# rabbitmq/ra

Hardware: AMD Instinct MI355X
Metric: append_entries decisions/sec across N Raft groups; achieved HBM GB/s vs peak (higher is better)
Workload: dtype u64

## Files before the change

### include/ra_gpu_batch.h

```cpp
#ifndef RA_GPU_BATCH_H
#define RA_GPU_BATCH_H

#include <stddef.h>
#include <stdint.h>

#ifdef __cplusplus
extern "C" {
#endif

#define RGB_ABI_VERSION   10u
#define RGB_UNDEF         UINT64_MAX
#define RGB_NONE          0xFFu
#define RGB_MAX_MEMBERS   8u
#define RGB_MAX_PENDING_RANGES 3u
#define RGB_MAX_RUNS      16u

#define RGB_AER_CHUNK_SIZE              128u
#define RGB_DEFAULT_MAX_PIPELINE_COUNT  4096u

enum {
  RGB_ROLE_FOLLOWER        = 0,
  RGB_ROLE_CANDIDATE       = 1,
  RGB_ROLE_LEADER          = 2,
  RGB_ROLE_PRE_VOTE        = 3,
// ... 273 lines not shown
int  rgb_collect(rgb_ctx *ctx, rgb_decision *out, uint32_t cap, uint32_t *n_out,
                 rgb_rpc *rpc_out, uint32_t rpc_cap, uint32_t *n_rpc_out, uint64_t *tick_out);
typedef struct rgb_view {
  const rgb_decision *decisions;
  const rgb_rpc *rpcs;
  uint64_t tick;
  uint32_t n;
  uint32_t n_rpcs;
  uint32_t slot;
  uint32_t _pad;
} rgb_view;
int  rgb_collect_view(rgb_ctx *ctx, rgb_view *view);
int  rgb_release(rgb_ctx *ctx, uint32_t slot);
uint32_t rgb_submit_trains(const rgb_ctx *ctx);
int      rgb_peek(rgb_ctx *ctx, uint32_t *n_out, uint32_t *n_rpc_out);
int      rgb_wait(rgb_ctx *ctx, uint32_t timeout_ms);
void     rgb_wake(rgb_ctx *ctx);
uint32_t rgb_in_flight(const rgb_ctx *ctx);

#define RGB_SUBMIT_RAW_MAX_ROUNDS 8u
typedef struct rgb_fill {
  rgb_msg *msgs;
  uint32_t cap;
  uint32_t slot;
  uint32_t max_rounds;
} rgb_fill;
uint32_t rgb_submit_raw_capacity(const rgb_ctx *ctx, uint32_t max_rounds);
int      rgb_submit_begin(rgb_ctx *ctx, uint32_t max_rounds, rgb_fill *out);
int      rgb_submit_commit(rgb_ctx *ctx, uint32_t slot, uint32_t n, uint64_t tick);
int      rgb_submit_raw(rgb_ctx *ctx, const rgb_msg *msgs, uint32_t n, uint32_t max_rounds, uint64_t tick);

uint32_t rgb_route(uint64_t group_uid, uint32_t n_contexts);

#define RGB_COMM_ID_BYTES 128u
typedef struct rgb_comm rgb_comm;
int  rgb_comm_unique_id(void *id_out );
int  rgb_comm_init_rank(rgb_ctx *ctx, const void *id, uint32_t n_ranks, uint32_t rank, rgb_comm **out);
void rgb_comm_destroy(rgb_comm *comm);
uint32_t rgb_comm_n_ranks(const rgb_comm *comm);
uint32_t rgb_comm_rank(const rgb_comm *comm);
int  rgb_leaderboard_allgather(rgb_ctx *ctx, rgb_comm *comm, const void *d_rows_local, uint32_t n_rows,
                               void *d_rows_all , void *stream);
int  rgb_leaderboard_allgather_host(rgb_ctx *ctx, rgb_comm *comm, uint32_t n_rows, rgb_leaderboard_row *rows_all);
const char *rgb_comm_last_error(void);

int  rgb_run_ticks_device(rgb_ctx *ctx, const void *d_msgs, uint32_t tick_stride,
                          const uint32_t *tick_counts, const void *d_tick_counts,
                          const uint32_t *kind_counts, uint32_t n_ticks, void *d_decisions,
                          void *d_rpcs, void *stream);

#define RGB_TRAIN_BUCKETS 256u
#define RGB_TRAIN_ERR_PLACEMENT 1u
#define RGB_TRAIN_ERR_SPIN      2u
#define RGB_TRAIN_ERR_ORDER     4u
#define RGB_TRAIN_ERR_PLAN      8u
#define RGB_TRAIN_FORM_NONE       0u
#define RGB_TRAIN_FORM_DEALT      1u
#define RGB_TRAIN_FORM_PERSISTENT 2u
typedef struct rgb_train_plan rgb_train_plan;
uint32_t rgb_train_bucket(uint32_t kind, uint32_t flags, uint32_t server, uint32_t n_members);
int  rgb_train_plan_create(rgb_ctx *ctx, const uint32_t *bucket_counts, uint32_t n_ticks, rgb_train_plan **out);
void rgb_train_plan_destroy(rgb_train_plan *plan);
uint32_t rgb_train_plan_blocks_per_tick(const rgb_train_plan *plan);
int  rgb_train_stamp_device(rgb_ctx *ctx, const void *d_msgs, void *d_stamps, uint32_t tick_stride,
                            const uint32_t *tick_counts, uint32_t n_ticks, void *stream);
int  rgb_train_run_device(rgb_ctx *ctx, const rgb_train_plan *plan, uint32_t first_tick, uint32_t n_ticks,
                          const void *d_msgs, const void *d_stamps, uint32_t tick_stride, void *d_decisions,
                          void *d_rpcs, uint32_t rpc_ring, void *stream);
int  rgb_train_plan_create_snap(rgb_ctx *ctx, const uint32_t *bucket_counts, uint32_t n_ticks, uint32_t snapshot_every,
                                rgb_train_plan **out);
int  rgb_train_run_snap_device(rgb_ctx *ctx, const rgb_train_plan *plan, uint32_t first_tick, uint32_t n_ticks,
                               const void *d_msgs, const void *d_stamps, uint32_t tick_stride, void *d_decisions,
                               void *d_rpcs, uint32_t rpc_ring, const void *d_snap_stamps, void *d_snap_rows,
                               void *stream);
int  rgb_snapshot_train_device(rgb_ctx *ctx, void *d_rows, void *stream);
int  rgb_train_plan_create_device(rgb_ctx *ctx, uint32_t n_ticks, uint32_t snapshot_every, rgb_train_plan **out);
int  rgb_train_plan_build_device(rgb_ctx *ctx, rgb_train_plan *plan, uint32_t first_tick, uint32_t n_ticks,
                                 const void *d_bucket_counts, void *stream);
int  rgb_train_plan_fit(rgb_ctx *ctx, rgb_train_plan *plan, uint32_t first_tick, uint32_t n_ticks, void *stream);
int  rgb_train_plan_download(rgb_ctx *ctx, const rgb_train_plan *plan, uint32_t tick, void *out_tick, uint32_t *out_rows,
                             uint32_t rows_cap);
uint32_t rgb_train_seq_bytes(const rgb_ctx *ctx);
int  rgb_train_status(rgb_ctx *ctx, uint32_t *flags_out, uint32_t *xcc_of_shard );
uint32_t rgb_train_form(const rgb_ctx *ctx);
uint32_t rgb_train_recoveries(const rgb_ctx *ctx);

int  rgb_snapshot(rgb_ctx *ctx, rgb_leaderboard_row *out);
int  rgb_snapshot_device(rgb_ctx *ctx, void *d_rows, void *stream);

int  rgb_state_checksum(rgb_ctx *ctx, uint32_t first, uint32_t n, uint64_t *out);

int  rgb_synchronize(rgb_ctx *ctx);

#ifdef __cplusplus
}
#endif
#endif
```

### ra_amd/csrc/rgb_api.hip

```cpp
#include <hip/hip_runtime.h>

#include <atomic>
#include <chrono>
#include <condition_variable>
#include <cstdio>
#include <cstdlib>
#include <cstring>
#include <memory>
#include <mutex>
#include <thread>
#include <new>
#include <vector>

#if defined(__x86_64__)
#include <emmintrin.h>
#endif

#include "rgb_internal.h"
#include "../../include/ra_gpu_batch_synth.h"

#define RGB_STREAM_COPY_MIN (1u << 20)
#ifndef RGB_COPY_STREAM_MIN
#define RGB_COPY_STREAM_MIN (2u << 20)
#endif
static inline void copy_msg(rgb_msg *dst, const rgb_msg *src, bool stream) {
#if defined(__x86_64__)
  if (stream) {
    const __m128i *q = reinterpret_cast<const __m128i *>(src);
    __m128i *d = reinterpret_cast<__m128i *>(dst);
    const __m128i a = _mm_loadu_si128(q), b = _mm_loadu_si128(q + 1), c = _mm_loadu_si128(q + 2), e = _mm_loadu_si128(q + 3);
    _mm_stream_si128(d, a); _mm_stream_si128(d + 1, b); _mm_stream_si128(d + 2, c); _mm_stream_si128(d + 3, e);
    return;
  }
#endif
  (void)stream;
  *dst = *src;
}
static inline void copy_out(void *dst, const void *src, size_t bytes) {
#if defined(__x86_64__)
  if (bytes >= RGB_STREAM_COPY_MIN && ((uintptr_t)dst & 15u) == 0 && (bytes & 63u) == 0) {
    const __m128i *q = reinterpret_cast<const __m128i *>(src);
    __m128i *d = reinterpret_cast<__m128i *>(dst);
    for (size_t k = 0; k < bytes / 16u; k += 4) {
      const __m128i a = _mm_loadu_si128(q + k), b = _mm_loadu_si128(q + k + 1), c = _mm_loadu_si128(q + k + 2), e = _mm_loadu_si128(q + k + 3);
      _mm_stream_si128(d + k, a); _mm_stream_si128(d + k + 1, b); _mm_stream_si128(d + k + 2, c); _mm_stream_si128(d + k + 3, e);
    }
    _mm_sfence();
    return;
  }
#endif
  memcpy(dst, src, bytes);
}

#define HIPCHK(ctx, expr)                          \
  do {                                             \
    hipError_t e__ = (expr);                       \
    if (e__ != hipSuccess) {                       \
      (ctx)->last_hip.store((int)e__, std::memory_order_relaxed); \
      return RGB_E_HIP;                            \
    }                                              \
  } while (0)
#define LAUNCHCHK(ctx, expr)                       \
  do {                                             \
    int lr__ = (expr);                             \
    if (lr__) {                                    \
      (ctx)->last_hip.store(lr__, std::memory_order_relaxed); \
      return RGB_E_HIP;                            \
    }                                              \
  } while (0)

struct rgb_slot {
  rgb_msg *h_msgs = nullptr;
  rgb_decision *h_dec = nullptr;
  rgb_msg *d_msgs = nullptr;
  rgb_decision *d_dec = nullptr;
  u32 *h_pos = nullptr, *d_pos = nullptr;
  rgb_rpc *d_rpcs = nullptr;
  rgb_rpc *h_rpcs = nullptr;
  u32 *h_nrpc = nullptr;
  u32 *d_res = nullptr;
  unsigned char *h_stamps = nullptr, *d_stamps = nullptr;
  rgb_train_tick *h_plan = nullptr, *d_plan = nullptr;
  u32 *h_rows = nullptr, *d_rows = nullptr;
  u32 rows_cap = 0;
  u32 *d_ctl = nullptr;
  u64 *h_ranges = nullptr, *d_ranges = nullptr;
  u32 ranges_cap = 0, n_ranges = 0;
  bool has_seqx = false;
  u32 *h_touched = nullptr, *d_touched = nullptr;
  u32 n_touched = 0;
  void *d_undo = nullptr;
  bool has_undo = false;
  u32 n_rounds = 0;
  std::vector<u32> round_start;
  std::vector<u32> round_cc;
// ... 109 lines not shown
    case RGB_E_NOMEM: return "out of memory";
    case RGB_E_HIP: return "HIP runtime error (see rgb_last_hip_error)";
    case RGB_E_STATE: return "call out of order";
    case RGB_E_FULL: return "staging ring full";
    case RGB_E_EMPTY: return "nothing submitted";
    case RGB_E_UNSUPPORTED: return "unsupported";
    case RGB_E_NODEVICE: return "no HIP device (there is no CPU fallback)";
    case RGB_E_COMM: return "RCCL error (see rgb_comm_last_error)";
    default: return "unknown error";
  }
}

void rgb_default_config(rgb_config *cfg) {
  if (!cfg) return;
  memset(cfg, 0, sizeof *cfg);
  cfg->abi_version = RGB_ABI_VERSION;
  cfg->device = 0;
  cfg->max_runs = 8;
  cfg->ring_slots = 4;
  cfg->ring_capacity = 65536;
  cfg->max_pipeline_count = RGB_DEFAULT_MAX_PIPELINE_COUNT;
  cfg->max_aer_batch = RGB_AER_CHUNK_SIZE;
  cfg->flags = 0;
}

int rgb_last_hip_error(const rgb_ctx *ctx) { return ctx ? ctx->last_hip.load(std::memory_order_relaxed) : 0; }

static int settle_trains(rgb_ctx *ctx);
struct rgb_stream_turn {
  std::lock_guard<std::mutex> a, c, b;
  int rc;
  explicit rgb_stream_turn(rgb_ctx *ctx) : a(ctx->state_mu), c(ctx->collect_mu), b(ctx->enqueue_mu), rc(settle_trains(ctx)) {}
};

static void free_slot(rgb_slot &s) {
  if (s.h_msgs) (void)hipHostFree(s.h_msgs);
  if (s.h_dec) (void)hipHostFree(s.h_dec);
  if (s.d_msgs) (void)hipFree(s.d_msgs);
  if (s.d_dec) (void)hipFree(s.d_dec);
  if (s.d_rpcs) (void)hipFree(s.d_rpcs);
  if (s.h_rpcs) (void)hipHostFree(s.h_rpcs);
  if (s.h_nrpc) (void)hipHostFree(s.h_nrpc);
  if (s.d_res) (void)hipFree(s.d_res);
  if (s.h_stamps) (void)hipHostFree(s.h_stamps);
  if (s.d_stamps) (void)hipFree(s.d_stamps);
  if (s.h_plan) (void)hipHostFree(s.h_plan);
  if (s.d_plan) (void)hipFree(s.d_plan);
  if (s.h_rows) (void)hipHostFree(s.h_rows);
  if (s.d_rows) (void)hipFree(s.d_rows);
  if (s.d_ctl) (void)hipFree(s.d_ctl);
  if (s.h_ranges) (void)hipHostFree(s.h_ranges);
  if (s.d_ranges) (void)hipFree(s.d_ranges);
  s.h_ranges = s.d_ranges = nullptr; s.ranges_cap = 0;
  if (s.h_touched) (void)hipHostFree(s.h_touched);
  if (s.d_touched) (void)hipFree(s.d_touched);
  if (s.d_undo) (void)hipFree(s.d_undo);
  if (s.done) (void)hipEventDestroy(s.done);
  if (s.copied) (void)hipEventDestroy(s.copied);
  s.copied = nullptr;
  if (s.d_raw) (void)hipFree(s.d_raw);
  if (s.d_key) (void)hipFree(s.d_key);
  free(s.h_stage);
  s.d_raw = nullptr; s.d_key = nullptr; s.h_stage = nullptr;
  s.h_msgs = nullptr; s.h_dec = nullptr; s.d_msgs = nullptr; s.d_dec = nullptr; s.d_rpcs = nullptr; s.h_rpcs = nullptr;
  s.h_nrpc = nullptr; s.d_res = nullptr;
  s.h_stamps = s.d_stamps = nullptr; s.h_plan = s.d_plan = nullptr; s.h_rows = s.d_rows = nullptr; s.done = nullptr;
  s.d_ctl = nullptr; s.h_touched = s.d_touched = nullptr; s.d_undo = nullptr;
  s.h_pos = s.d_pos = nullptr;
}

void rgb_close(rgb_ctx *ctx) {
  if (!ctx) return;
  if (ctx->stream) (void)hipStreamSynchronize(ctx->stream);
  rgb_wal_release(ctx);
  rgb_seg_release(ctx);
  for (u32 k = 0; k < ctx->ring_size; ++k) free_slot(ctx->ring_mem[k]);
  if (ctx->dev.dbg_buf) (void)hipFree(ctx->dev.dbg_buf);
  if (ctx->dev.hot) (void)hipFree(ctx->dev.hot);
  if (ctx->dev.peers) (void)hipFree(ctx->dev.peers);
  if (ctx->dev.runs) (void)hipFree(ctx->dev.runs);
  if (ctx->dev.cond) (void)hipFree(ctx->dev.cond);
  if (ctx->dev.qry) (void)hipFree(ctx->dev.qry);
  if (ctx->dev.seq) (void)hipFree(ctx->dev.seq);
  if (ctx->d_stage) (void)hipFree(ctx->d_stage);
  if (ctx->h_stage) (void)hipHostFree(ctx->h_stage);
  if (ctx->d_rows) (void)hipFree(ctx->d_rows);
  if (ctx->d_sums) (void)hipFree(ctx->d_sums);
  if (ctx->lb_stream) { (void)hipStreamSynchronize(ctx->lb_stream); (void)hipStreamDestroy(ctx->lb_stream); }
  if (ctx->copy_stream) { (void)hipStreamSynchronize(ctx->copy_stream); (void)hipStreamDestroy(ctx->copy_stream); }
  if (ctx->d_lb_gather) (void)hipFree(ctx->d_lb_gather);
  if (ctx->h_lb_pinned) (void)hipHostFree(ctx->h_lb_pinned);
  if (ctx->lb_event) (void)hipEventDestroy(ctx->lb_event);
  if (ctx->d_synth) (void)hipFree(ctx->d_synth);
  if (ctx->d_synth_sent) (void)hipFree(ctx->d_synth_sent);
  if (ctx->d_train_ctl) (void)hipFree(ctx->d_train_ctl);
  if (ctx->d_seq_cnt) (void)hipFree(ctx->d_seq_cnt);
  if (ctx->d_srv_cnt) (void)hipFree(ctx->d_srv_cnt);
  if (ctx->d_srv_list) (void)hipFree(ctx->d_srv_list);
  if (ctx->d_prep) (void)hipFree(ctx->d_prep);

  if (ctx->stream) (void)hipStreamDestroy(ctx->stream);
  delete ctx;
}

int rgb_open(const rgb_config *cfg_in, rgb_ctx **out) {
  if (!out) return RGB_E_INVAL;
  *out = nullptr;
  rgb_config cfg;
  if (cfg_in) cfg = *cfg_in; else rgb_default_config(&cfg);
  if (cfg.abi_version != RGB_ABI_VERSION) return RGB_E_INVAL;
  if (cfg.max_runs < 2 || cfg.max_runs > RGB_MAX_RUNS) return RGB_E_INVAL;
  if (cfg.ring_slots < 1 || cfg.ring_slots > 64 || cfg.ring_capacity < 1) return RGB_E_INVAL;
  if (cfg.max_pipeline_count == 0) cfg.max_pipeline_count = RGB_DEFAULT_MAX_PIPELINE_COUNT;
  if (cfg.max_aer_batch == 0) cfg.max_aer_batch = RGB_AER_CHUNK_SIZE;
  if (cfg.max_aer_batch > 65535) return RGB_E_INVAL;
  int ndev = 0;
  hipError_t e = hipGetDeviceCount(&ndev);
  if (e != hipSuccess || ndev <= 0) return RGB_E_NODEVICE;
  if (cfg.device < 0 || cfg.device >= ndev) return RGB_E_INVAL;
  rgb_ctx *ctx = new (std::nothrow) rgb_ctx();
  if (!ctx) return RGB_E_NOMEM;
  ctx->cfg = cfg;
  memset(&ctx->dev, 0, sizeof ctx->dev);
  e = hipSetDevice(cfg.device);
  if (e == hipSuccess) e = hipStreamCreateWithFlags(&ctx->stream, hipStreamNonBlocking);
  if (e == hipSuccess) e = hipStreamCreateWithFlags(&ctx->copy_stream, hipStreamNonBlocking);

  if (e != hipSuccess) { delete ctx; return RGB_E_HIP; }
  *out = ctx;
  return RGB_OK;
}

uint32_t rgb_n_servers(const rgb_ctx *ctx) { return ctx ? ctx->dev.n_servers : 0; }

static int alloc_slot(rgb_ctx *ctx, rgb_slot &s) {
  const u32 cap = ctx->cfg.ring_capacity;
  HIPCHK(ctx, hipHostMalloc((void **)&s.h_msgs, (size_t)cap * (sizeof(rgb_msg) + sizeof(u32)), hipHostMallocDefault));
  HIPCHK(ctx, hipHostMalloc((void **)&s.h_dec, (size_t)cap * sizeof(rgb_decision), hipHostMallocDefault));
  HIPCHK(ctx, hipMalloc((void **)&s.d_msgs, (size_t)cap * (sizeof(rgb_msg) + sizeof(u32))));
  HIPCHK(ctx, hipMalloc((void **)&s.d_dec, (size_t)cap * sizeof(rgb_decision)));
  s.h_pos = reinterpret_cast<u32 *>(s.h_msgs + cap); s.d_pos = reinterpret_cast<u32 *>(s.d_msgs + cap);
  HIPCHK(ctx, hipMalloc((void **)&s.d_rpcs, (size_t)ctx->rpc_cap * sizeof(rgb_rpc)));
  HIPCHK(ctx, hipHostMalloc((void **)&s.h_rpcs, (size_t)ctx->rpc_cap * sizeof(rgb_rpc), hipHostMallocDefault));
  HIPCHK(ctx, hipEventCreateWithFlags(&s.done, hipEventDisableTiming));
  HIPCHK(ctx, hipEventCreateWithFlags(&s.copied, hipEventDisableTiming));
  HIPCHK(ctx, hipHostMalloc((void **)&s.h_nrpc, 64, hipHostMallocDefault));
  HIPCHK(ctx, hipMalloc((void **)&s.d_res, ((size_t)rgb_results_blocks(cap) + 1u) * sizeof(u32)));
  HIPCHK(ctx, hipMemsetAsync(s.d_res, 0, ((size_t)rgb_results_blocks(cap) + 1u) * sizeof(u32), ctx->stream));
  HIPCHK(ctx, hipHostMalloc((void **)&s.h_stamps, cap, hipHostMallocDefault));
  HIPCHK(ctx, hipMalloc((void **)&s.d_stamps, cap));
  HIPCHK(ctx, hipHostMalloc((void **)&s.h_plan, RGB_SUBMIT_TRAIN_ROUNDS * sizeof(rgb_train_tick), hipHostMallocDefault));
  HIPCHK(ctx, hipMalloc((void **)&s.d_plan, RGB_SUBMIT_TRAIN_ROUNDS * sizeof(rgb_train_tick)));
  s.rows_cap = (cap / 32u + 2u * RGB_N_CLASSES * RGB_SUBMIT_TRAIN_ROUNDS + 64u);
  HIPCHK(ctx, hipHostMalloc((void **)&s.h_rows, (size_t)s.rows_cap * RGB_SUBMIT_TRAIN_ROUNDS * sizeof(u32), hipHostMallocDefault));
  HIPCHK(ctx, hipMalloc((void **)&s.d_rows, (size_t)s.rows_cap * RGB_SUBMIT_TRAIN_ROUNDS * sizeof(u32)));
  HIPCHK(ctx, hipMalloc((void **)&s.d_ctl, RGB_TRAIN_CTL_WORDS * sizeof(u32)));
  HIPCHK(ctx, hipMemsetAsync(s.d_ctl, 0, RGB_TRAIN_CTL_WORDS * sizeof(u32), ctx->stream));
  HIPCHK(ctx, hipHostMalloc((void **)&s.h_touched, (size_t)cap * sizeof(u32), hipHostMallocDefault));
  HIPCHK(ctx, hipMalloc((void **)&s.d_touched, (size_t)cap * sizeof(u32)));
  return RGB_OK;
}

int rgb_upload_state(rgb_ctx *ctx, uint32_t first, uint32_t n, const rgb_server_state *in);

int rgb_register_groups(rgb_ctx *ctx, uint32_t n_groups, uint32_t n_members) {
  if (!ctx) return RGB_E_INVAL;
  if (ctx->registered) return RGB_E_STATE;
  if (n_members < 1 || n_members > RGB_MAX_MEMBERS || n_groups < 1) return RGB_E_INVAL;
  const uint64_t S64 = (uint64_t)n_groups * n_members;
  if (S64 > 0x7FFFFFFFull) return RGB_E_INVAL;
  const u32 S = (u32)S64;
  HIPCHK(ctx, hipSetDevice(ctx->cfg.device));
  rgb_dev &d = ctx->dev;
  d.n_servers = S; d.n_members = n_members; d.max_runs = ctx->cfg.max_runs;
  d.peer_stride = rgb_peer_stride(n_members);
  d.max_pipeline_count = ctx->cfg.max_pipeline_count;
  d.max_aer_batch = ctx->cfg.max_aer_batch;
  d.dbg = 0; d.dbg_buf = nullptr;
  d.synth_hint = ctx->synth_hint;
  d.fuse_pipeline = (ctx->cfg.flags & RGB_CFG_FUSE_PIPELINE) ? 1u : 0u;
  d.seq_ranges = nullptr; d.n_seq_ranges = 0;
#ifdef RGB_PROFILE
  { const char *e = getenv("RGB_DEBUG"); d.dbg = e ? (u32)atoi(e) : 0u; }
  if (d.dbg & 16u) {
    HIPCHK(ctx, hipMalloc((void **)&d.dbg_buf, (size_t)(S / 64 + 16) * 8 * sizeof(u64)));
    HIPCHK(ctx, hipMemsetAsync(d.dbg_buf, 0, (size_t)(S / 64 + 16) * 8 * sizeof(u64), ctx->stream));
  }
#endif
#ifdef RGB_X_DECLINE_HIST
  HIPCHK(ctx, hipMalloc((void **)&d.dbg_buf, 128 * sizeof(u64)));
  HIPCHK(ctx, hipMemsetAsync(d.dbg_buf, 0, 128 * sizeof(u64), ctx->stream));
#endif
#ifdef RGB_X_TRAIN_TIMELINE
  HIPCHK(ctx, hipMalloc((void **)&d.dbg_buf, (size_t)(1u << 20) * 8 * sizeof(u64)));
  HIPCHK(ctx, hipMemsetAsync(d.dbg_buf, 0, (size_t)(1u << 20) * 8 * sizeof(u64), ctx->stream));
#endif
  HIPCHK(ctx, hipMalloc((void **)&d.hot, (size_t)S * RGB_HOT_WORDS * sizeof(u64)));
  HIPCHK(ctx, hipMalloc((void **)&d.peers, (size_t)S * d.peer_stride * sizeof(u64)));
  HIPCHK(ctx, hipMalloc((void **)&d.runs, (size_t)S * d.max_runs * 2 * sizeof(u64)));
  HIPCHK(ctx, hipMalloc((void **)&d.cond, (size_t)S * 4 * sizeof(u64)));
  HIPCHK(ctx, hipMalloc((void **)&d.qry, (size_t)S * RGB_QRY_WORDS * sizeof(u64)));
  HIPCHK(ctx, hipMemsetAsync(d.runs, 0, (size_t)S * d.max_runs * 2 * sizeof(u64), ctx->stream));
  d.seq_stride = (((n_groups + RGB_TRAIN_SHARDS - 1u) / RGB_TRAIN_SHARDS) * n_members + 255u) & ~255u;
  HIPCHK(ctx, hipMalloc((void **)&d.seq, (size_t)d.seq_stride * RGB_TRAIN_SHARDS));
  HIPCHK(ctx, hipMemsetAsync(d.seq, 0, (size_t)d.seq_stride * RGB_TRAIN_SHARDS, ctx->stream));
  ctx->stage_cap = S < 16384u ? S : 16384u;
  HIPCHK(ctx, hipMalloc((void **)&ctx->d_stage, (size_t)ctx->stage_cap * sizeof(rgb_server_state)));
  HIPCHK(ctx, hipHostMalloc((void **)&ctx->h_stage, (size_t)ctx->stage_cap * sizeof(rgb_server_state),
                            hipHostMallocDefault));
  HIPCHK(ctx, hipMalloc((void **)&ctx->d_rows, (size_t)n_groups * sizeof(rgb_leaderboard_row)));
  HIPCHK(ctx, hipMalloc((void **)&ctx->d_sums, (size_t)S * sizeof(u64)));
  ctx->rpc_stride = n_members > 1 ? n_members - 1 : 1;
  ctx->rpc_cap = ctx->cfg.ring_capacity * ctx->rpc_stride;
  ctx->ring_mem.reset(new (std::nothrow) rgb_slot[ctx->cfg.ring_slots]);
  if (!ctx->ring_mem) return RGB_E_NOMEM;
  ctx->ring_size = ctx->cfg.ring_slots;
  for (u32 k = 0; k < ctx->ring_size; ++k) {
    rgb_slot &s = ctx->ring_mem[k];
    int rc = alloc_slot(ctx, s);
    if (rc) return rc;
  }
  ctx->registered = true;
  std::vector<rgb_server_state> init(ctx->stage_cap);
  for (u32 base = 0; base < S; base += ctx->stage_cap) {
    u32 cnt = S - base < ctx->stage_cap ? S - base : ctx->stage_cap;
    for (u32 k = 0; k < cnt; ++k) {
      rgb_server_state &h = init[k];
      memset(&h, 0, sizeof h);
      h.snapshot_index = RGB_UNDEF; h.snapshot_term = RGB_UNDEF;
      h.pending_first = 1;
      for (unsigned i = 0; i < n_members; ++i) h.next_index[i] = 1;
      h.role = RGB_ROLE_FOLLOWER; h.self = (uint8_t)((base + k) % n_members);
      h.n_members = (uint8_t)n_members; h.voted_for = RGB_NONE; h.leader_id = RGB_NONE;
      h.cond_leader = RGB_NONE; h.n_runs = 1;
      h.present_mask = (uint8_t)((1u << n_members) - 1u); h.voter_mask = h.present_mask;
      h.status_mask = 0xFF;
    }
    int rc = rgb_upload_state(ctx, base, cnt, init.data());
    if (rc) return rc;
  }
  return RGB_OK;
}

static int validate_state(const rgb_ctx *ctx, const rgb_server_state &h) {
  if (h.n_members != ctx->dev.n_members) return RGB_E_INVAL;
  if (h.self >= RGB_MAX_MEMBERS) return RGB_E_INVAL;
  if (h.role > RGB_ROLE_AWAIT_CONDITION || h.cond_reason > RGB_COND_TRANSFER_LEADERSHIP) return RGB_E_INVAL;
  if (h.n_runs > RGB_MAX_RUNS || h.votes > 15) return RGB_E_INVAL;
  if (h.voted_for != RGB_NONE && h.voted_for >= RGB_MAX_MEMBERS) return RGB_E_INVAL;
  if (h.leader_id != RGB_NONE && h.leader_id >= RGB_MAX_MEMBERS) return RGB_E_INVAL;
  if (h.cond_leader != RGB_NONE && h.cond_leader >= RGB_MAX_MEMBERS) return RGB_E_INVAL;
  if (h.first_index <= h.last_index) {
    if (h.n_runs == 0 || h.run_start[0] != h.first_index) return RGB_E_INVAL;
    for (unsigned r = 1; r < h.n_runs; ++r)
      if (!(h.run_start[r] > h.run_start[r - 1] && h.run_start[r] <= h.last_index)) return RGB_E_INVAL;
    if (h.run_term[h.n_runs - 1] != h.last_term) return RGB_E_INVAL;
  }
  if (h.n_pending_old > 2) return RGB_E_INVAL;
  uint64_t above = h.pending_first;
  for (int k = (int)h.n_pending_old - 1; k >= 0; --k) {
    const uint64_t s = h.pending_old[k][0], e = h.pending_old[k][1];
    if (s > e || e == RGB_UNDEF || !(e + 1 < above)) return RGB_E_INVAL;
    above = s;
  }
  return RGB_OK;
}

int rgb_upload_state(rgb_ctx *ctx, uint32_t first, uint32_t n, const rgb_server_state *in) {
  if (!ctx || (!in && n)) return RGB_E_INVAL;
  if (!ctx->registered) return RGB_E_STATE;
  if ((uint64_t)first + n > ctx->dev.n_servers) return RGB_E_INVAL;
  for (u32 k = 0; k < n; ++k) {
    int rc = validate_state(ctx, in[k]);
    if (rc) return rc;
  }
  HIPCHK(ctx, hipSetDevice(ctx->cfg.device));
  rgb_stream_turn turn(ctx);
  if (turn.rc) return turn.rc;
  for (u32 base = 0; base < n; base += ctx->stage_cap) {
    u32 cnt = n - base < ctx->stage_cap ? n - base : ctx->stage_cap;
    memcpy(ctx->h_stage, in + base, (size_t)cnt * sizeof(rgb_server_state));
    HIPCHK(ctx, hipMemcpyAsync(ctx->d_stage, ctx->h_stage, (size_t)cnt * sizeof(rgb_server_state),
                               hipMemcpyHostToDevice, ctx->stream));
    LAUNCHCHK(ctx, rgb_launch_pack(ctx->dev, ctx->d_stage, first + base, cnt, ctx->stream));
    HIPCHK(ctx, hipStreamSynchronize(ctx->stream));
  }
  return RGB_OK;
}

int rgb_download_state(rgb_ctx *ctx, uint32_t first, uint32_t n, rgb_server_state *out) {
  if (!ctx || (!out && n)) return RGB_E_INVAL;
  if (!ctx->registered) return RGB_E_STATE;
  if ((uint64_t)first + n > ctx->dev.n_servers) return RGB_E_INVAL;
  HIPCHK(ctx, hipSetDevice(ctx->cfg.device));
  rgb_stream_turn turn(ctx);
  if (turn.rc) return turn.rc;
  for (u32 base = 0; base < n; base += ctx->stage_cap) {
    u32 cnt = n - base < ctx->stage_cap ? n - base : ctx->stage_cap;
    LAUNCHCHK(ctx, rgb_launch_unpack(ctx->dev, ctx->d_stage, first + base, cnt, ctx->stream));
    HIPCHK(ctx, hipMemcpyAsync(ctx->h_stage, ctx->d_stage, (size_t)cnt * sizeof(rgb_server_state),
                               hipMemcpyDeviceToHost, ctx->stream));
    HIPCHK(ctx, hipStreamSynchronize(ctx->stream));
    memcpy(out + base, ctx->h_stage, (size_t)cnt * sizeof(rgb_server_state));
  }
  return RGB_OK;
}

static int validate_msg(const rgb_ctx *ctx, const rgb_msg &m) {
  if (m.kind > RGB_MSG_KIND_MAX) return RGB_E_INVAL;
  if (m.kind == RGB_MSG_NOP) return RGB_OK;
  if (m.server >= ctx->dev.n_servers) return RGB_E_INVAL;
  if (m.from != RGB_NONE && m.from >= RGB_MAX_MEMBERS) return RGB_E_INVAL;
  if (m.kind == RGB_MSG_AER && m.n_run0 > m.n_entries) return RGB_E_INVAL;
  if (m.kind == RGB_MSG_WRITTEN && m.a > m.b) return RGB_E_INVAL;
  if (m.kind == RGB_MSG_WRITTEN && (m.flags & RGB_MF_SEQ2) &&
      !(m.run0_term <= m.run1_term && m.run1_term != RGB_UNDEF && m.run1_term + 1 < m.a)) return RGB_E_INVAL;
  if (m.kind == RGB_MSG_WRITTEN && (m.flags & RGB_MF_SEQX) && !(m.flags & RGB_MF_SEQ2)) return RGB_E_INVAL;
  return RGB_OK;
}
static int validate_seqx(const rgb_msg &m, const uint64_t *ranges, uint32_t n_ranges) {
  if (m.kind != RGB_MSG_WRITTEN || !(m.flags & RGB_MF_SEQX)) return RGB_OK;
  if (!ranges || m.n_entries == 0 || m.c > n_ranges || (uint64_t)m.c + m.n_entries > n_ranges) return RGB_E_INVAL;
  uint64_t prev_last = 0; bool have = false;
  for (uint32_t k = 0; k < m.n_entries; ++k) {
    const uint64_t f = ranges[2 * (m.c + k)], l = ranges[2 * (m.c + k) + 1];
    if (f > l || l == RGB_UNDEF || (have && !(prev_last + 1 < f))) return RGB_E_INVAL;
    prev_last = l; have = true;
  }
  return prev_last + 1 < m.run0_term ? RGB_OK : RGB_E_INVAL;
}

static int train_scratch(rgb_ctx *ctx);

#define RGB_FAULT_STAMP 1u
#define RGB_FAULT_SHARD 2u

static rgb_dev slot_dev(const rgb_ctx *ctx, const rgb_slot &s) {
  rgb_dev d = ctx->dev;
  d.seq_ranges = s.n_ranges ? s.d_ranges : nullptr;
  d.n_seq_ranges = s.n_ranges;
  return d;
}

static int enqueue_rounds(rgb_ctx *ctx, rgb_slot &s) {
  const rgb_dev dv = slot_dev(ctx, s);
  auto classes = [&](const u32 counts[RGB_N_CLASSES], u32 at) {
    return rgb_launch_tick_classes(dv, s.d_msgs + at, counts, nullptr, 0, s.d_dec + at, s.d_rpcs, at, at, ctx->stream);
  };
  for (u32 r = 0; r < s.n_rounds; ++r) {
    const u32 off = s.round_start[r], cnt = s.round_start[r + 1] - s.round_start[r];
    u32 cc[RGB_N_CLASSES], real = 0, before_written = 0;
    for (int c = 0; c < RGB_N_CLASSES; ++c) {
      cc[c] = s.round_cc[(size_t)r * RGB_N_CLASSES + c];
      real += cc[c];
      if (c < 2) before_written += cc[c];
    }
    if (!s.has_seqx || cc[2] == 0) {
      LAUNCHCHK(ctx, classes(cc, off));
    } else {
      u32 head[RGB_N_CLASSES] = {0}, tail[RGB_N_CLASSES] = {0};
      head[0] = cc[0]; head[1] = cc[1];
// ... 851 lines not shown
  void *st = stream ? stream : (void *)ctx->stream;
  LAUNCHCHK(ctx, rgb_launch_train_plan((const u32 *)d_bucket_counts, plan->d_ticks, plan->d_rows, plan->bpt / RGB_TRAIN_SHARDS,
                                       first_tick, n_ticks, plan->snap_every, ctx->dev.n_servers / ctx->dev.n_members,
                                       ctx->dev.n_members, ctx->d_train_ctl, st));
  for (u32 t = first_tick; t < first_tick + n_ticks; ++t) plan->rows_fit[t] = 0xFFFFFFFFu;
  return RGB_OK;
}

int rgb_train_plan_fit(rgb_ctx *ctx, rgb_train_plan *plan, uint32_t first_tick, uint32_t n_ticks, void *stream) {
  if (!ctx || !plan) return RGB_E_INVAL;
  if (!plan->on_device || (uint64_t)first_tick + n_ticks > plan->n_ticks) return RGB_E_INVAL;
  if (n_ticks == 0) return RGB_OK;
  HIPCHK(ctx, hipSetDevice(ctx->cfg.device));
  hipStream_t st = stream ? (hipStream_t)stream : ctx->stream;
  std::vector<u32> rows(n_ticks);
  HIPCHK(ctx, hipStreamSynchronize(st));
  HIPCHK(ctx, hipMemcpy2D(rows.data(), sizeof(u32), &plan->d_ticks[first_tick].n_rows, sizeof(rgb_train_tick), sizeof(u32),
                          n_ticks, hipMemcpyDeviceToHost));
  for (u32 t = 0; t < n_ticks; ++t) plan->rows_fit[first_tick + t] = rows[t];
  return RGB_OK;
}

int rgb_train_plan_download(rgb_ctx *ctx, const rgb_train_plan *plan, uint32_t tick, void *out_tick, uint32_t *out_rows,
                            uint32_t rows_cap) {
  if (!ctx || !plan || !out_tick || tick >= plan->n_ticks) return RGB_E_INVAL;
  HIPCHK(ctx, hipSetDevice(ctx->cfg.device));
  HIPCHK(ctx, hipStreamSynchronize(ctx->stream));
  rgb_train_tick h;
  HIPCHK(ctx, hipMemcpy(&h, plan->d_ticks + tick, sizeof h, hipMemcpyDeviceToHost));
  memcpy(out_tick, &h, sizeof h);
  const u32 rpt = plan->bpt / RGB_TRAIN_SHARDS;
  const u32 n = h.n_rows < rows_cap ? h.n_rows : rows_cap;
  if (out_rows && n && h.n_rows <= rpt)
    HIPCHK(ctx, hipMemcpy(out_rows, plan->d_rows + (size_t)tick * rpt, (size_t)n * sizeof(u32), hipMemcpyDeviceToHost));
  return (int)h.n_rows;
}

void rgb_train_plan_destroy(rgb_train_plan *plan) {
  if (!plan) return;
  if (plan->d_ticks) (void)hipFree(plan->d_ticks);
  if (plan->d_rows) (void)hipFree(plan->d_rows);
  delete plan;
}

uint32_t rgb_train_plan_blocks_per_tick(const rgb_train_plan *plan) {
  if (!plan) return 0;
  if (plan->on_device && !plan->rows_fit.empty()) {
    u32 mx = 0;
    for (u32 r : plan->rows_fit) { if (r == 0xFFFFFFFFu) return plan->bpt; if (r > mx) mx = r; }
    if (mx * RGB_TRAIN_SHARDS <= plan->bpt) return (mx ? mx : 1u) * RGB_TRAIN_SHARDS;
  }
  return plan->bpt;
}

int rgb_train_stamp_device(rgb_ctx *ctx, const void *d_msgs, void *d_stamps, uint32_t tick_stride,
                           const uint32_t *tick_counts, uint32_t n_ticks, void *stream) {
  if (!ctx || !d_msgs || !d_stamps || (!tick_counts && n_ticks)) return RGB_E_INVAL;
  if (!ctx->registered) return RGB_E_STATE;
  if (!ctx->d_seq_cnt || ctx->xcc_state != 1) return RGB_E_STATE;
  hipStream_t st = stream ? (hipStream_t)stream : ctx->stream;
  const rgb_msg *m = (const rgb_msg *)d_msgs;
  unsigned char *sp = (unsigned char *)d_stamps;
  HIPCHK(ctx, hipMemcpyAsync(ctx->d_seq_cnt, ctx->dev.seq, (size_t)ctx->dev.seq_stride * RGB_TRAIN_SHARDS,
                             hipMemcpyDeviceToDevice, st));
  for (u32 t = 0; t < n_ticks; ++t) {
    if (tick_counts[t] > tick_stride) return RGB_E_INVAL;
    LAUNCHCHK(ctx, rgb_launch_train_seq(ctx->dev, m + (size_t)t * tick_stride, tick_counts[t], ctx->d_seq_cnt,
                                        sp + (size_t)t * tick_stride, st));
  }
  return RGB_OK;
}

int rgb_train_run_device(rgb_ctx *ctx, const rgb_train_plan *plan, uint32_t first_tick, uint32_t n_ticks,
                         const void *d_msgs, const void *d_stamps, uint32_t tick_stride, void *d_decisions,
                         void *d_rpcs, uint32_t rpc_ring, void *stream) {
  return rgb_train_run_snap_device(ctx, plan, first_tick, n_ticks, d_msgs, d_stamps, tick_stride, d_decisions, d_rpcs,
                                   rpc_ring, nullptr, nullptr, stream);
}

uint32_t rgb_train_seq_bytes(const rgb_ctx *ctx) {
  return (ctx && ctx->registered) ? ctx->dev.seq_stride * RGB_TRAIN_SHARDS : 0u;
}

int rgb_snapshot_train_device(rgb_ctx *ctx, void *d_rows, void *stream) {
  int rc = rgb_snapshot_device(ctx, d_rows, stream);
  if (rc) return rc;
  void *st = stream ? stream : (void *)ctx->stream;
  LAUNCHCHK(ctx, rgb_launch_seq_bump(ctx->dev.seq, nullptr, ctx->dev.seq_stride * RGB_TRAIN_SHARDS, st));
  return RGB_OK;
}

int rgb_train_run_snap_device(rgb_ctx *ctx, const rgb_train_plan *plan, uint32_t first_tick, uint32_t n_ticks,
                              const void *d_msgs, const void *d_stamps, uint32_t tick_stride, void *d_decisions,
                              void *d_rpcs, uint32_t rpc_ring, const void *d_snap_stamps, void *d_snap_rows,
                              void *stream) {
  if (!ctx || !plan || !d_msgs || !d_stamps || !d_decisions) return RGB_E_INVAL;
  if (plan->snap_every && (!d_snap_stamps || !d_snap_rows)) return RGB_E_INVAL;
  if (!plan->snap_every && (d_snap_stamps || d_snap_rows)) return RGB_E_INVAL;
  if (!ctx->registered || ctx->xcc_state != 1) return RGB_E_STATE;
  if ((uint64_t)first_tick + n_ticks > plan->n_ticks) return RGB_E_INVAL;
  if (n_ticks == 0 || plan->bpt == 0) return RGB_OK;
  void *st = stream ? stream : (void *)ctx->stream;
  u32 per = RGB_TRAIN_MAX_TICKS;
  if ((uint64_t)per * plan->bpt > 0x7FFFFFFFull) per = (u32)(0x7FFFFFFFull / plan->bpt);
  if (per == 0) return RGB_E_INVAL;
  if (plan->snap_every) {
    if (n_ticks > per) return RGB_E_INVAL;
    const u32 last = first_tick + n_ticks - 1u;
    const u32 inside = last / plan->snap_every - first_tick / plan->snap_every;
    if (n_ticks + inside > RGB_TRAIN_MAX_TICKS) return RGB_E_INVAL;
  }
  for (u32 t = first_tick; t < first_tick + n_ticks; t += per) {
    const u32 n = first_tick + n_ticks - t < per ? first_tick + n_ticks - t : per;
    const size_t off = (size_t)t * tick_stride;
    u32 grid_bpt = plan->bpt;
    if (plan->on_device) {
      u32 mx = 0; bool known = true;
      for (u32 k = t; k < t + n && known; ++k) { known = plan->rows_fit[k] != 0xFFFFFFFFu; if (known && plan->rows_fit[k] > mx) mx = plan->rows_fit[k]; }
      if (known && mx * RGB_TRAIN_SHARDS <= plan->bpt) grid_bpt = (mx ? mx : 1u) * RGB_TRAIN_SHARDS;
    }
    LAUNCHCHK(ctx, rgb_launch_train(ctx->dev, (const rgb_msg *)d_msgs + off, (const unsigned char *)d_stamps + off,
                                    tick_stride, plan->d_ticks + t, plan->d_rows + (size_t)t * (plan->bpt / RGB_TRAIN_SHARDS), n,
                                    grid_bpt, (rgb_decision *)d_decisions + off,
                                    (rgb_rpc *)d_rpcs, rpc_ring, (u32)off, ctx->d_train_ctl, ctx->n_xcc,
                                    ctx->train_dealt.load(std::memory_order_relaxed) ? 0u : ctx->train_blocks, st,
                                    (const unsigned char *)d_snap_stamps, (rgb_leaderboard_row *)d_snap_rows,
                                    plan->bpt / RGB_TRAIN_SHARDS));
  }
  return RGB_OK;
}

int rgb_train_status(rgb_ctx *ctx, uint32_t *flags_out, uint32_t *xcc_of_shard) {
  if (!ctx) return RGB_E_INVAL;
  if (flags_out) *flags_out = 0;
  if (xcc_of_shard)
    for (u32 x = 0; x < RGB_TRAIN_SHARDS; ++x)
      xcc_of_shard[x] = ctx->xcc_state == 1 ? x % ctx->n_xcc : 0xFFFFFFFFu;
  if (!ctx->d_train_ctl) return RGB_OK;
  HIPCHK(ctx, hipSetDevice(ctx->cfg.device));
  HIPCHK(ctx, hipStreamSynchronize(ctx->stream));
  u32 w = 0;
  HIPCHK(ctx, hipMemcpy(&w, ctx->d_train_ctl, sizeof w, hipMemcpyDeviceToHost));
  if (flags_out) *flags_out = w;
  if (w & RGB_TRAIN_ERR_PLACEMENT) ctx->train_dealt.store(false, std::memory_order_relaxed);
  if (w) {
    HIPCHK(ctx, hipMemsetAsync(ctx->d_train_ctl, 0, sizeof(u32), ctx->stream));
    HIPCHK(ctx, hipStreamSynchronize(ctx->stream));
    return RGB_E_STATE;
  }
  return RGB_OK;
}

int rgb_synth_apply_tick_device(rgb_ctx *ctx, const void *d_msgs, uint32_t max_msgs, void *d_decisions,
                                void *d_rpcs, void *stream) {
  if (!ctx || !d_msgs || !d_decisions) return RGB_E_INVAL;
  if (!ctx->registered || !ctx->d_synth) return RGB_E_STATE;
  void *st = stream ? stream : (void *)ctx->stream;
  LAUNCHCHK(ctx, rgb_launch_tick_classes(ctx->dev, (const rgb_msg *)d_msgs, nullptr, ctx->d_synth, max_msgs,
                                         (rgb_decision *)d_decisions, (rgb_rpc *)d_rpcs, 0, 0, st));
  return RGB_OK;
}

int rgb_snapshot_device(rgb_ctx *ctx, void *d_rows, void *stream) {
  if (!ctx || !d_rows) return RGB_E_INVAL;
  if (!ctx->registered) return RGB_E_STATE;
  void *st = stream ? stream : (void *)ctx->stream;
// ... 164 lines not shown
```

### ra_amd/csrc/rgb_internal.h

```cpp
#ifndef RGB_INTERNAL_H
#define RGB_INTERNAL_H

#include <stdint.h>
#include "../../include/ra_gpu_batch.h"

typedef unsigned long long u64;
typedef uint32_t u32;

#define RGB_HOT_WORDS 16
#define RGB_QRY_WORDS 16

#define HOT_CT    0
#define HOT_PK    1
#define HOT_LRT   2
#define HOT_PRS   3
#define HOT_CI    4
#define HOT_LA    5
#define HOT_LI    6
#define HOT_LT    7
#define HOT_SI    8
#define HOT_ST    9
#define HOT_FIRST 10
#define HOT_LRS   11
#define HOT_LWI   12
// ... 11 lines not shown
#define PEER_MI(i, N) (2u * (unsigned)(i))
#define PEER_NI(i, N) (2u * (unsigned)(i) + 1u)
#define PEER_CS(i, N) (2u * (unsigned)(N) + (unsigned)(i))

#define PK_ROLE_SH      0
#define PK_COND_SH      3
#define PK_SELF_SH      5
#define PK_VOTES_SH     9
#define PK_NRUNS_SH     13
#define PK_NONVOTER_SH  18
#define PK_CONDTO_SH    19
#define PK_VOTED_SH     20
#define PK_LEADER_SH    24
#define PK_CONDLDR_SH   28
#define PK_PRESENT_SH   32
#define PK_VOTER_SH     40
#define PK_STATUS_SH    48
#define PK_QSELF_SH     56
#define PK_QPEER_SH     57
#define PK_BACKOFF_SH   58
#define PK_PENDX_SH     59
static inline __host__ __device__ unsigned pk_cond_reason(u64 pk) {
  const unsigned c = (unsigned)((pk >> PK_COND_SH) & 3ull), to = (unsigned)((pk >> PK_CONDTO_SH) & 1ull);
  return to == 0u ? c : c == RGB_COND_WAL_DOWN ? (unsigned)RGB_COND_WAL_DOWN_LEADER : (unsigned)RGB_COND_TRANSFER_LEADERSHIP;
}
static inline __host__ __device__ u64 pk_with_cond_reason(u64 pk, unsigned reason) {
  const u64 c = reason == RGB_COND_WAL_DOWN_LEADER ? (u64)RGB_COND_WAL_DOWN : reason == RGB_COND_TRANSFER_LEADERSHIP ? 0ull : (u64)reason;
  const u64 to = (reason == RGB_COND_WAL_DOWN_LEADER || reason == RGB_COND_TRANSFER_LEADERSHIP) ? 1ull : 0ull;
  return (pk & ~((3ull << PK_COND_SH) | (1ull << PK_CONDTO_SH))) | (c << PK_COND_SH) | (to << PK_CONDTO_SH);
}
#define QRY_PEND_LO     12
#define QRY_PEND_HI     14
#define QRY_BACKOFF     9
#define QRY_TOKEN       10
#define QRY_MACVER      11

#define RGB_N_CLASSES 15
static inline __host__ __device__ unsigned rgb_kind_rank(unsigned kind) {
  switch (kind) {
    case RGB_MSG_AER: return 0;
    case RGB_MSG_AER_REPLY: return 1;
    case RGB_MSG_WRITTEN: return 2;
    case RGB_MSG_APPEND: return 3;
    case RGB_MSG_PIPELINE_RPCS: return 4;
    case RGB_MSG_REQUEST_VOTE: return 5;
    case RGB_MSG_VOTE_RESULT: return 6;
    case RGB_MSG_AWAIT_TIMEOUT: return 7;
    case RGB_MSG_ELECTION_TIMEOUT: return 8;
    case RGB_MSG_PRE_VOTE_RPC: return 9;
    case RGB_MSG_PRE_VOTE_RESULT: return 10;
    case RGB_MSG_SNAPSHOT_WRITTEN: return 11;
    case RGB_MSG_HEARTBEAT_RPC: return 12;
    case RGB_MSG_HEARTBEAT_REPLY: return 13;
    case RGB_MSG_CONSISTENT_QUERY: return 14;
    case RGB_MSG_TRANSFER_LEADERSHIP: return 14;
    default: return 15;
  }
}
#define RGB_N_FAMILIES 32
static inline __host__ __device__ unsigned rgb_family(unsigned kind, unsigned flags) {
  return 2u * rgb_kind_rank(kind) + ((flags & RGB_MF_SUCCESS) ? 1u : 0u);
}
static inline unsigned rgb_class_of_kind(unsigned kind) { return rgb_kind_rank(kind); }

#define RGB_TRAIN_SHARDS 8u
#define RGB_N_BUCKETS ((RGB_N_CLASSES + 1u) * RGB_TRAIN_SHARDS * 2u)
#define RGB_TRAIN_CTL_WORDS (320u + 32u * 64u)
static inline __host__ __device__ unsigned rgb_shard_of_server(unsigned server, unsigned n_members) {
  return (server / n_members) & (RGB_TRAIN_SHARDS - 1u);
}
static inline __host__ __device__ unsigned rgb_bucket(unsigned kind, unsigned flags, unsigned server, unsigned n_members) {
  return (rgb_kind_rank(kind) * RGB_TRAIN_SHARDS + rgb_shard_of_server(server, n_members)) * 2u +
         ((flags & RGB_MF_SUCCESS) ? 1u : 0u);
}
static inline __host__ __device__ unsigned rgb_bucket_hinted(unsigned kind, unsigned flags, unsigned server,
                                                             unsigned n_members, bool off_steady) {
  const bool hinted_kind = kind == RGB_MSG_WRITTEN || kind == RGB_MSG_AER;
  return rgb_bucket(kind, flags, server, n_members) | ((hinted_kind && off_steady) ? 1u : 0u);
}
static inline __host__ __device__ unsigned rgb_seq_index(unsigned server, unsigned n_members, unsigned seq_stride) {
  const unsigned g = server / n_members, m = server - g * n_members;
  return (g & (RGB_TRAIN_SHARDS - 1u)) * seq_stride + (g / RGB_TRAIN_SHARDS) * n_members + m;
}
#define RGB_TRAIN_MAX_TICKS 255u
#define RGB_N_PCLASSES (2u * RGB_N_CLASSES)
#define RGB_PC_SNAP RGB_N_PCLASSES
#define RGB_SNAP_LEAD 0.5f
struct rgb_train_tick {
  u32 n_rows;
  u32 msg_base;
  u32 snap;
  u32 pad[13];
  u32 off[RGB_N_PCLASSES][RGB_TRAIN_SHARDS];
  u32 cnt[RGB_N_PCLASSES][RGB_TRAIN_SHARDS];
};
#define RGB_SYNTH_FIXED_WORDS (RGB_N_FAMILIES + 2u * RGB_N_BUCKETS)
u32 rgb_synth_scratch_words(u32 n_groups);

static inline __host__ __device__ unsigned rgb_peer_stride(unsigned n_members) {
  return (3u * n_members + 7u) & ~7u;
}

struct rgb_dev {
  u64 *hot;
  u64 *peers;
  u64 *runs;
  u64 *cond;
  u64 *qry;
  u32 n_servers;
  u32 n_members;
  u32 max_runs;
  u32 peer_stride;
  u32 max_pipeline_count;
  u32 max_aer_batch;
  unsigned char *seq;
  u32 seq_stride;
  const u64 *seq_ranges;
  u32 n_seq_ranges;
  u32 fuse_pipeline;
  u32 synth_hint;
  u32 dbg;
  u64 *dbg_buf;
};

#define RGB_TICK_CLS_WRITTEN_SEQX 32
#define RGB_TICK_CLS_NOP 33
int rgb_launch_tick(const rgb_dev &dev, int cls, const rgb_msg *d_msgs, u32 n, const u32 *d_n,
                    rgb_decision *d_dec, rgb_rpc *d_rpcs, u32 rpc_slot_base, u32 msg_index_base, void *stream);
int rgb_launch_tick_classes(const rgb_dev &dev, const rgb_msg *d_msgs, const u32 counts[RGB_N_CLASSES],
                            const u32 *d_family_totals, u32 max_msgs, rgb_decision *d_dec, rgb_rpc *d_rpcs,
                            u32 rpc_slot_base, u32 msg_index_base, void *stream);
int rgb_launch_synth(const rgb_dev &dev, u64 seed, u64 tick, rgb_msg *d_msgs, u32 *d_scratch,
                     u32 *d_kind_counts, u32 *d_n, u32 *d_bucket_counts, unsigned char *d_stamps, unsigned char *d_sent,
                     void *stream);
int rgb_launch_train(const rgb_dev &dev, const rgb_msg *d_msgs, const unsigned char *d_stamps, u32 tick_stride,
                     const rgb_train_tick *d_plan, const u32 *d_row_tab, u32 n_ticks, u32 bpt, rgb_decision *d_dec,
                     rgb_rpc *d_rpcs, u32 rpc_ring, u32 index_base, u32 *d_ctl, u32 n_xcc, u32 n_blocks, void *stream,
                     const unsigned char *d_snap_stamps = nullptr, rgb_leaderboard_row *d_snap_rows = nullptr,
                     u32 tab_rpt = 0 );
u32 rgb_train_resident_blocks(unsigned n_members);
int rgb_launch_train_verify(u32 *d_ctl, void *stream);
int rgb_launch_train_seq(const rgb_dev &dev, const rgb_msg *d_msgs, u32 n, unsigned char *d_seq_cnt,
                         unsigned char *d_stamps, void *stream);
int rgb_launch_train_calibrate(u32 *d_out, void *stream);
u32 rgb_train_make_tick(const u32 *bucket_counts, unsigned n_members, rgb_train_tick *out, u32 *row_tab, u32 row_cap,
                        u32 snap_rows = 0);
int rgb_launch_train_plan(const u32 *d_bucket_counts, rgb_train_tick *d_ticks, u32 *d_rows, u32 rpt, u32 first_tick,
                          u32 n_ticks, u32 snapshot_every, u32 n_groups, u32 n_members, u32 *d_err, void *stream);
u32 rgb_train_rows_bound(u32 n_servers, u32 n_members, bool with_snapshot);
static inline u32 rgb_train_snap_rows(u32 n_groups) {
  return ((n_groups + RGB_TRAIN_SHARDS - 1u) / RGB_TRAIN_SHARDS + 63u) / 64u;
}
int rgb_launch_seq_bump(unsigned char *d_seq, unsigned char *d_out, u32 n_bytes, void *stream);
int rgb_launch_pack(const rgb_dev &dev, const rgb_server_state *d_in, u32 first, u32 n, void *stream);
int rgb_launch_unpack(const rgb_dev &dev, rgb_server_state *d_out, u32 first, u32 n, void *stream);
int rgb_launch_leaderboard(const rgb_dev &dev, rgb_leaderboard_row *d_rows, void *stream);
int rgb_launch_checksum(const rgb_dev &dev, u32 first, u32 n, u64 *d_out, void *stream);
int rgb_launch_stamp_rounds(const rgb_dev &dev, const rgb_msg *d_msgs, u32 n, unsigned char *d_stamps, void *stream);
u32 rgb_results_blocks(u32 n);
int rgb_launch_results(const rgb_decision *d_dec, const u32 *d_pos, u32 n, u32 cap, const rgb_rpc *d_rpcs, u32 rpc_stride, u32 *d_scratch,
                       const u32 *d_ctl, rgb_decision *out_dec, rgb_rpc *out_rpcs, u32 *out_hdr, void *stream);
u32 rgb_undo_pieces(const rgb_dev &dev);
int rgb_launch_undo(const rgb_dev &dev, const u32 *d_ids, u32 n, void *d_undo, u32 restore, void *stream);

#define RGB_PREP_MAX_ROUNDS 8u
static_assert(RGB_PREP_MAX_ROUNDS == RGB_SUBMIT_RAW_MAX_ROUNDS, "a server's message list holds the public bound");
static inline __host__ __device__ u32 rgb_raw_round_base(u32 n, u32 r) {
  u32 b = 0;
  for (u32 q = 0; q < r; ++q) b += n / (q + 1u);
  return b;
}
#define RGB_PREP_ERR        0u
#define RGB_PREP_ERR_INVAL  1u
#define RGB_PREP_ERR_ROUNDS 2u
#define RGB_PREP_COUNTS     32u
#define RGB_PREP_CURSORS    (RGB_PREP_COUNTS + RGB_PREP_MAX_ROUNDS * RGB_N_FAMILIES)
#define RGB_PREP_WORDS      (RGB_PREP_CURSORS + RGB_PREP_MAX_ROUNDS * RGB_N_FAMILIES)
int rgb_launch_prepare(const rgb_dev &dev, const rgb_msg *d_raw, u32 n, u32 max_rounds, u32 *d_srv_cnt, u32 *d_srv_list,
                       u32 *d_prep, unsigned char *d_key, rgb_msg *d_msgs, rgb_decision *d_dec, u32 *d_pos,
                       u32 *code_out, void *stream);

#endif
```

### ra_amd/csrc/rgb_kernels.hip

```cpp
#include <hip/hip_runtime.h>
#include "rgb_internal.h"

#define UNDEF 0xFFFFFFFFFFFFFFFFull
#define SLOT_NONE4 0xFu

#ifdef RGB_PROFILE
#define RGB_KNOB(dev, bit) (((dev).dbg & (bit)) != 0)
#else
#define RGB_KNOB(dev, bit) false
#endif

#ifndef RGB_TICK_BLOCK
#define RGB_TICK_BLOCK 64
#endif
#ifndef RGB_CLASS_MIN_WAVES
#define RGB_CLASS_MIN_WAVES(N) ((N) <= 5 ? 4 : 3)
#endif
#ifndef RGB_MIN_WAVES
#define RGB_MIN_WAVES(N) 2
#endif

namespace {

__host__ __device__ constexpr bool rgb_lead_class(int c) { return c == 1 || c == 3 || c == 4; }
// ... 52 lines not shown

enum { GLDS_DEFAULT = 0, GLDS_NT = 2, GLDS_SC1 = 16 };
template <int POLICY>
__device__ __forceinline__ void glds16(const void *g, void *lds_base) {
#ifdef RGB_HOST_EMULATION
  memcpy(static_cast<char *>(lds_base) + 16 * emu::lane(), g, 16);
#else
  __builtin_amdgcn_global_load_lds((const __attribute__((address_space(1))) void *)g,
                                   (__attribute__((address_space(3))) void *)lds_base, 16, 0, POLICY);
#endif
}
__device__ __forceinline__ void glds_wait() {
#ifndef RGB_HOST_EMULATION
  __builtin_amdgcn_s_waitcnt(0x0F70);
  asm volatile("" ::: "memory");
#endif
}

__device__ __forceinline__ void lds_barrier() {
#ifdef RGB_HOST_EMULATION
  __syncthreads();
#else
  __builtin_amdgcn_fence(__ATOMIC_RELEASE, "workgroup", "local");
  __builtin_amdgcn_s_barrier();
  __builtin_amdgcn_fence(__ATOMIC_ACQUIRE, "workgroup", "local");
#endif
}

typedef unsigned long long v2u64 __attribute__((ext_vector_type(2)));
template <bool NT>
__device__ __forceinline__ ulonglong2 ld16(const ulonglong2 *p) {
  if (NT) {
    v2u64 v = __builtin_nontemporal_load(reinterpret_cast<const v2u64 *>(p));
    return make_ulonglong2(v.x, v.y);
  }
  return *p;
}

__device__ __forceinline__ u64 ldg8(bool coh, const u64 *p) {
#ifndef RGB_HOST_EMULATION
  if (coh) return __hip_atomic_load(p, __ATOMIC_RELAXED, __HIP_MEMORY_SCOPE_AGENT);
#endif
  return *p;
}
__device__ __forceinline__ ulonglong2 ldg16(bool coh, const ulonglong2 *p) {
#ifndef RGB_HOST_EMULATION
  if (coh) {
    const u64 *q = reinterpret_cast<const u64 *>(p);
    const u64 x = __hip_atomic_load(q, __ATOMIC_RELAXED, __HIP_MEMORY_SCOPE_AGENT);
    const u64 y = __hip_atomic_load(q + 1, __ATOMIC_RELAXED, __HIP_MEMORY_SCOPE_AGENT);
    return make_ulonglong2(x, y);
  }
#endif
  return *p;
}

__device__ __forceinline__ u64 pk_get(u64 pk, int sh, int w) { return (pk >> sh) & ((1ull << w) - 1ull); }
__device__ __forceinline__ u64 pk_set(u64 pk, int sh, int w, u64 v) {
  const u64 m = ((1ull << w) - 1ull) << sh;
  return (pk & ~m) | ((v << sh) & m);
}
__device__ __forceinline__ unsigned slot8to4(unsigned s) { return s >= 8u ? SLOT_NONE4 : s; }
__device__ __forceinline__ unsigned slot4to8(unsigned s) { return s >= 8u ? (unsigned)RGB_NONE : s; }

template <bool COH, bool WC = false, bool SEQX = false>
struct LaneT {
  static constexpr bool coh = COH;
  static constexpr bool seqx_ok = SEQX;
  static constexpr bool walk_cache = WC;
  int wc_k;
  u64 wc_start, wc_term, wc_next;
  u64 ct, ci, la, li, lt, lwi, lwt, pk, si, st, first, lrs, lrt, prs, prt, pend;
  u64 token, macver;
  u32 server, n_entries, n_run0;
  unsigned kind, from, mflags, gap;
  u64 term, a, b, c, run0_term, run1_term;
  const u64 *seqx;
  u32 n_seqx;
  const u64 *runs;
  u64 *peers;
  const ulonglong2 *peers_lds;
  unsigned peers_swz;
  const ulonglong2 *runs_lds;
  ulonglong2 *rpc_stash;
  u32 max_runs;
  u32 flags;
  u32 inv;
  bool has_reply;
  unsigned reply_to;
  u64 r_term, r_next, r_last, r_lterm;
  u64 w_first, w_last;
  bool vote_reqs;
  unsigned n_runs;
  unsigned push_cnt;
  bool cond_dirty;
  u64 cr0, cr1, cr2, cr3;
  u64 po_floor, po_cut;
  u64 pmi[8], pni[8], pcs[8];
  unsigned dmi, dni, dcs;
  unsigned pdirty;
  unsigned dcs_ci;
  bool peers_loaded;
  u64 *qry_base;
  u64 qself, qp[8];
  bool q_loaded;
  unsigned q_dirty;
  unsigned hb_mask;
  unsigned cancel_mask;
#ifdef RGB_X_DECLINE_HIST
  const u64 *dbg_hist;
#endif
#ifdef RGB_PROFILE
  unsigned prof_nloads;
  bool prof_noprobe;
#endif
  u64 hb_term, hb_qi, q_consensus;
};

template <int N, class Lane>
__device__ __forceinline__ void load_peers(Lane &L) {
  if (L.peers_loaded) return;
  constexpr int PS = (3 * N + 7) & ~7;
  u64 w[PS];
  if ((PS == 16 || PS == 24) && L.peers_lds != nullptr) {
    const unsigned sw = PS == 24 ? L.peers_swz << 1 : L.peers_swz;
#pragma unroll
    for (int k = 0; k < PS / 2; ++k) {
      if (2 * k < 3 * N) { ulonglong2 v = L.peers_lds[(unsigned)k ^ sw]; w[2 * k] = v.x; w[2 * k + 1] = v.y; }
    }
  } else {
    const ulonglong2 *pp = reinterpret_cast<const ulonglong2 *>(L.peers);
#pragma unroll
    for (int k = 0; k < PS / 2; ++k) {
      if (2 * k < 3 * N) { ulonglong2 v = ldg16(L.coh, pp + k); w[2 * k] = v.x; w[2 * k + 1] = v.y; }
    }
  }
#pragma unroll
  for (int i = 0; i < N; ++i) { L.pmi[i] = w[PEER_MI(i, N)]; L.pni[i] = w[PEER_NI(i, N)]; L.pcs[i] = w[PEER_CS(i, N)]; }
  L.peers_loaded = true;
}

template <int N>
__device__ __forceinline__ u64 peer_get(const u64 (&a)[8], unsigned p) {
  u64 r = 0;
#pragma unroll
  for (int i = 0; i < N; ++i) r = ((unsigned)i == p) ? a[i] : r;
  return r;
}
template <int N>
__device__ __forceinline__ void peer_set(u64 (&a)[8], unsigned &dirty, unsigned p, u64 v) {
#pragma unroll
  for (int i = 0; i < N; ++i)
    if ((unsigned)i == p) { a[i] = v; dirty |= 1u << i; }
}

template <class Lane>
__device__ __forceinline__ unsigned prow_at(const Lane &L, unsigned w) { return (((w >> 1) ^ L.peers_swz) << 1) | (w & 1u); }
template <class Lane>
__device__ __forceinline__ u64 prow_get(const Lane &L, unsigned w) {
  return reinterpret_cast<const u64 *>(L.peers_lds)[prow_at(L, w)];
}
template <class Lane>
__device__ __forceinline__ void prow_set(Lane &L, unsigned w, u64 v) {
  const_cast<u64 *>(reinterpret_cast<const u64 *>(L.peers_lds))[prow_at(L, w)] = v;
  L.pdirty |= 1u << w;
}
template <int N, bool PL, class Lane> __device__ __forceinline__ u64 mi_get(const Lane &L, int i) { return PL ? prow_get(L, PEER_MI(i, N)) : L.pmi[i]; }
template <int N, bool PL, class Lane> __device__ __forceinline__ u64 ni_get(const Lane &L, int i) { return PL ? prow_get(L, PEER_NI(i, N)) : L.pni[i]; }
template <int N, bool PL, class Lane> __device__ __forceinline__ u64 cs_get(const Lane &L, int i) { return PL ? prow_get(L, PEER_CS(i, N)) : L.pcs[i]; }
template <int N, bool PL, class Lane> __device__ __forceinline__ void ni_set(Lane &L, int i, u64 v) {
  if (PL) prow_set(L, PEER_NI(i, N), v); else { L.pni[i] = v; L.dni |= 1u << i; }
}
template <int N, bool PL, class Lane> __device__ __forceinline__ u64 mi_of(const Lane &L, unsigned p) { return PL ? (p < (unsigned)N ? prow_get(L, PEER_MI(p, N)) : 0) : peer_get<N>(L.pmi, p); }
template <int N, bool PL, class Lane> __device__ __forceinline__ u64 ni_of(const Lane &L, unsigned p) { return PL ? (p < (unsigned)N ? prow_get(L, PEER_NI(p, N)) : 0) : peer_get<N>(L.pni, p); }
template <int N, bool PL, class Lane> __device__ __forceinline__ void mi_put(Lane &L, unsigned p, u64 v) {
  if (PL) { if (p < (unsigned)N) prow_set(L, PEER_MI(p, N), v); } else peer_set<N>(L.pmi, L.dmi, p, v);
}
template <int N, bool PL, class Lane> __device__ __forceinline__ void ni_put(Lane &L, unsigned p, u64 v) {
  if (PL) { if (p < (unsigned)N) prow_set(L, PEER_NI(p, N), v); } else peer_set<N>(L.pni, L.dni, p, v);
}

template <class Lane>
__device__ __forceinline__ bool range_nonempty(const Lane &L) { return L.first <= L.li; }

#define RGB_RUNS_LDS 8
template <class Lane>
__device__ __forceinline__ ulonglong2 run_pair(const Lane &L, int k) {
  if (L.runs_lds != nullptr && k < RGB_RUNS_LDS) return L.runs_lds[(unsigned)k ^ L.peers_swz];
  return ldg16(L.coh, reinterpret_cast<const ulonglong2 *>(L.runs) + k);
}
template <class Lane>
__device__ __forceinline__ u64 run_word(const Lane &L, int i) {
#ifdef RGB_PROFILE
  const_cast<Lane &>(L).prof_nloads += 1;
#endif
  if (L.runs_lds != nullptr && i < 2 * RGB_RUNS_LDS) {
    const ulonglong2 v = L.runs_lds[(unsigned)(i >> 1) ^ L.peers_swz];
    return (i & 1) ? v.y : v.x;
  }
  return ldg8(L.coh, L.runs + i);
}

template <class Lane>
__device__ __forceinline__ int run_search(const Lane &L, u64 idx, u64 &term) {
  int k = (int)L.n_runs - 3;
  if (k < 0) return -1;
  if (Lane::walk_cache && L.wc_k >= 0 && L.wc_k <= k && idx >= L.wc_start && idx < L.wc_next) {
    term = L.wc_term;
    return L.wc_k;
  }
  ulonglong2 cur = run_pair(L, k);
  u64 upper = L.prs;
#pragma unroll 1
  for (; k >= 0; --k) {
    const ulonglong2 nxt = run_pair(L, k > 0 ? k - 1 : 0);
#ifdef RGB_PROFILE
    const_cast<Lane &>(L).prof_nloads += 2u;
#endif
    if (idx >= cur.x) {
      term = cur.y;
      if (Lane::walk_cache) {
        Lane &M = const_cast<Lane &>(L);
        M.wc_k = k; M.wc_start = cur.x; M.wc_term = cur.y; M.wc_next = upper;
      }
      return k;
    }
    upper = cur.x;
    cur = nxt;
  }
  return -1;
}

template <class Lane>
__device__ __forceinline__ u64 fetch_term(const Lane &L, u64 idx) {
  if (!(range_nonempty(L) && idx >= L.first && idx <= L.li)) return UNDEF;
  if (idx >= L.lrs) return L.lrt;
#ifdef RGB_PROFILE
  if (L.prof_noprobe) return L.lrt;
#endif
  if (L.n_runs >= 2 && idx >= L.prs) return L.prt;
  u64 term = UNDEF;
  run_search(L, idx, term);
  return term;
}

template <class Lane>
__device__ __forceinline__ u64 srv_fetch_term(const Lane &L, u64 idx) {
  u64 t = fetch_term(L, idx);
  if (t == UNDEF && L.si != UNDEF && L.si == idx) return L.st;
  return t;
}

template <class Lane>
__device__ __forceinline__ int find_run(const Lane &L, u64 idx) {
  if (L.n_runs == 0) return -1;
  if (idx >= L.lrs) return (int)L.n_runs - 1;
#ifdef RGB_PROFILE
  if (L.prof_noprobe) return (int)L.n_runs - 1;
#endif
  if (L.n_runs >= 2 && idx >= L.prs) return (int)L.n_runs - 2;
  u64 term;
  return run_search(L, idx, term);
}


template <class Lane>
__device__ __forceinline__ u64 next_log_index(const Lane &L) {
  if (range_nonempty(L)) return L.li + 1;
  if (L.si != UNDEF) return L.si + 1;
  return 0;
}

enum { HLE_OK = 0, HLE_MISMATCH = 1, HLE_MISSING = 2 };
template <class Lane>
__device__ __forceinline__ int has_log_entry_or_snapshot(const Lane &L, u64 idx, u64 term) {
  u64 t = fetch_term(L, idx);
  if (t == UNDEF) {
    if (L.si != UNDEF && L.si == idx) return L.st == term ? HLE_OK : HLE_MISMATCH;
    return HLE_MISSING;
// ... 267 lines not shown
  u64 lwt;
  if (lwi == L.lwi) lwt = L.lwt;
  else if (L.si != UNDEF && L.si == lwi) lwt = L.st;
  else if (lwi == 0) lwt = 0;
  else {
    lwt = fetch_term(L, lwi);
    if (lwt == UNDEF) return RGB_INV_LAST_WRITTEN_TERM;
  }
  if (!had_range) {
    L.first = fst; L.n_runs = 0;
  } else if (fst <= L.li) {
    if (fst == 0 || fst <= L.first) L.n_runs = 0;
    else truncate_runs_to(L, fst - 1);
  }
  const u64 lo = (had_range && L.first > fst) ? L.first : fst;
  if (range_lost) {
    L.n_runs = 0; L.push_cnt = 0;
    L.li = L.si; L.lt = L.st; L.first = L.si + 1;
  } else {
    if (k0 < L.n_run0) {
      const u64 s1 = base + L.n_run0;
      if (L.n_run0 == L.n_entries || lo < s1) push_segment(L, lo, L.run0_term);
      if (L.n_run0 < L.n_entries) push_segment(L, s1 > lo ? s1 : lo, L.run1_term);
    } else {
      push_segment(L, lo, L.run1_term);
    }
    L.li = lst;
    L.lt = (L.n_entries - 1) < L.n_run0 ? L.run0_term : L.run1_term;
  }
  L.lwi = lwi; L.lwt = lwt;
  if (fst < L.pend) L.pend = fst;
  pend_old_limit(L, fst);
  return 0;
}

template <class Lane>
__device__ __forceinline__ int log_set_last_index(Lane &L, u64 idx) {
  u64 t = fetch_term(L, idx);
  bool snap_is_idx = (L.si != UNDEF && L.si == idx);
  if (t == UNDEF && !snap_is_idx) return RGB_INV_SET_LAST_INDEX_NOT_FOUND;
  if (snap_is_idx) {
    if (range_nonempty(L)) {
      if (idx + 1 <= L.first) { L.n_runs = 0; L.li = idx; L.first = idx + 1; }
      else if (idx + 1 <= L.li) { truncate_runs_to(L, idx); L.li = idx; }
    }
    if (!range_nonempty(L)) L.li = L.si;
    L.lt = L.st;
    L.lwi = L.si; L.lwt = L.st;
    if (idx + 1 < L.pend) L.pend = idx + 1;
    pend_old_limit(L, idx + 1);
    pend_canon(L);
    return 0;
  }
  u64 lwi = idx < L.lwi ? idx : L.lwi;
  u64 lwt;
  if (L.si != UNDEF && L.si == lwi) lwt = L.st;
  else lwt = fetch_term(L, lwi);
  if (lwt == UNDEF) return RGB_INV_LAST_WRITTEN_TERM;
  if (idx + 1 <= L.li) { truncate_runs_to(L, idx); L.li = idx; }
  L.lt = t;
  L.lwi = lwi; L.lwt = lwt;
  if (idx + 1 < L.pend) L.pend = idx + 1;
  pend_old_limit(L, idx + 1);
  pend_canon(L);
  return 0;
}


template <class Lane>
__device__ __forceinline__ bool written_c1(const Lane &L, u64 term, u64 from, u64 to, u64 &c1) {
  const u64 hi = to < L.li ? to : L.li;
  const u64 lo = from > L.first ? from : L.first;
  if (hi < lo) return false;
  u64 end = L.li;
  for (int k = (int)L.n_runs - 1; k >= 0; --k) {
    u64 s, t;
    if ((unsigned)k == L.n_runs - 1) { s = L.lrs; t = L.lrt; }
    else if ((unsigned)k == L.n_runs - 2) { s = L.prs; t = L.prt; }
    else {
#ifdef RGB_PROFILE
      if (L.prof_noprobe) break;
#endif
      const ulonglong2 r = ldg16(L.coh, reinterpret_cast<const ulonglong2 *>(L.runs) + k);
#ifdef RGB_PROFILE
      const_cast<Lane &>(L).prof_nloads += 2;
#endif
      s = r.x; t = r.y;
    }
    const u64 rs = s < L.first ? L.first : s;
    if (rs <= hi && end >= lo && t == term) {
      const u64 idx = end < hi ? end : hi;
      if (idx >= lo && idx >= rs) { c1 = idx; return true; }
    }
    if (s <= lo) break;
    end = s - 1;
  }
  return false;
}
template <class Lane>
__device__ __forceinline__ bool written_c2(const Lane &L, bool in_range, u64 from, u64 to, u64 &c2) {
  if (L.si == UNDEF) return false;
  u64 u = to < L.si ? to : L.si;
  bool ok = u >= from;
  if (ok && in_range && u >= L.first && u <= L.li) {
    ok = L.first > 0 && L.first - 1 >= from;
    u = L.first - 1;
  }
  if (ok) c2 = u;
  return ok;
}
template <class Lane>
__device__ __forceinline__ void written_range(const Lane &L, u32 r, u64 from, u64 to, u64 &f, u64 &t) {
  if (r == 0) { f = from; t = to; }
  else if (r == 1) { f = L.run0_term; t = L.run1_term; }
  else {
    const u64 *e = L.seqx + 2u * ((u64)L.c + (u64)(L.n_entries - 1u - (r - 2u)));
    f = e[0]; t = e[1];
  }
}
template <class Lane>
__device__ __forceinline__ bool pend_range_written_many(const Lane &L, u64 ps, u64 pe, u64 c, u32 n_w, u64 from, u64 to) {
  if (ps > pe || ps > c) return true;
  const u64 e = pe < c ? pe : c;
#pragma unroll 1
  for (u32 r = 0; r < n_w; ++r) {
    u64 f, t;
    written_range(L, r, from, to, f, t);
    const u64 te = t < c ? t : c;
    if (f <= c && ps >= f && e <= te) return true;
  }
  return false;
}

template <class Lane>
__device__ __forceinline__ int log_written_many(Lane &L, u64 term, u64 from, u64 to, bool &changed) {
  changed = false;
  const bool in_range = range_nonempty(L);
  const bool two = (L.mflags & (RGB_MF_SEQ2 | RGB_MF_SEQX)) != 0;
  u32 n_w = two ? 2u : 1u;
  if (L.mflags & RGB_MF_SEQX) {
    if (L.seqx == nullptr || L.n_entries == 0u || (u64)L.c + (u64)L.n_entries > (u64)L.n_seqx) return RGB_INV_WRITTEN_SEQ_LIST;
    n_w += L.n_entries;
  }
  bool have1 = false; u64 c1 = 0;
  bool have2 = false; u64 c2 = 0;
#pragma unroll 1
  for (u32 r = 0; r < n_w; ++r) {
    u64 f, t;
    written_range(L, r, from, to, f, t);
    if (in_range && !have1) have1 = written_c1(L, term, f, t, c1);
    if (!have2) have2 = written_c2(L, in_range, f, t, c2);
  }
  const bool first_clause = have1 && (!have2 || c1 > c2);
  if (!first_clause && !have2) return 0;
  const u64 c = first_clause ? c1 : c2;
  bool prefix = true;
  const bool sparse = pk_get(L.pk, PK_PENDX_SH, 1) != 0;
  if (pend_nonempty(L)) prefix = pend_range_written_many(L, L.pend, L.li, c, n_w, from, to);
  if (sparse && prefix) {
    const u64 *q = qry_row(L);
#pragma unroll 1
    for (int k = 0; k < 2 && prefix; ++k) {
      u64 ps = ldg8(L.coh, q + QRY_PEND_LO + 2 * k), pe = ldg8(L.coh, q + QRY_PEND_LO + 2 * k + 1);
      if (ps < L.po_floor) ps = L.po_floor;
      if (L.po_cut != UNDEF && pe >= L.po_cut) pe = L.po_cut - 1;
      if (L.po_cut == 0) continue;
// ... 882 lines not shown
      return 0;
    }
    case RGB_MSG_WRITTEN:
      { bool changed; return log_written(L, L.term, L.a, L.b, changed); }
    case RGB_MSG_SNAPSHOT_WRITTEN:
      log_snapshot_written(L, L.a, L.b);
      return 0;
    case RGB_MSG_PRE_VOTE_RPC: return process_pre_vote(L);
    case RGB_MSG_ELECTION_TIMEOUT:
      if (pk_get(L.pk, PK_NONVOTER_SH, 1)) return 0;
      call_for_election_pre_vote<N>(L, L.c);
      return 0;
    case RGB_MSG_AER: {
      bool pred = false;
      if (wal_down) {
        pred = can_write;
      } else if (transfer) {
        pred = L.term > L.ct;
      } else if (L.term >= L.ct) {
        int h = has_log_entry_or_snapshot(L, L.a, L.b);
        if (h == HLE_OK) pred = true;
        else if (h == HLE_MISMATCH) pred = pk_get(L.pk, PK_COND_SH, 2) == RGB_COND_MISSING;
      }
      if (pred) { set_role(L, wal_down ? back : (unsigned)RGB_ROLE_FOLLOWER); reprocess = true; }
      return 0;
    }
    default:
      if (wal_down && can_write) { set_role(L, back); reprocess = true; }
      return 0;
  }
}

struct Dec { u64 w[8]; };

__device__ __forceinline__ void make_decision(Dec &d, u32 server, unsigned role, unsigned reply_to,
                                              unsigned n_rpcs, unsigned kind, u32 flags, u32 inv, u64 w2,
                                              u64 w3, u64 w4, u64 w5, u64 ci, u64 la, unsigned hb_mask = 0,
                                              unsigned cancel_mask = 0) {
  d.w[0] = (u64)server | ((u64)(role & 0xFF) << 32) | ((u64)(reply_to & 0xFF) << 40) |
           ((u64)(n_rpcs & 0xFF) << 48) | ((u64)(kind & 0xFF) << 56);
  d.w[1] = (u64)flags | ((u64)(inv & 0xFFFFu) << 32) | ((u64)(hb_mask & 0xFFu) << 48) |
           ((u64)(cancel_mask & 0xFFu) << 56);
  d.w[2] = w2; d.w[3] = w3; d.w[4] = w4; d.w[5] = w5; d.w[6] = ci; d.w[7] = la;
}

__device__ __forceinline__ bool compact_decision(Dec &d) {
  const u32 flags = (u32)d.w[1];
  const unsigned kind = (unsigned)(d.w[0] >> 56);
  if ((d.w[1] >> 32) != 0ull || (flags & RGB_F_COMPACT)) return false;
  const u32 plain = RGB_F_LEADER_MSG | RGB_F_APPLIED | RGB_F_AUX_EVAL | RGB_F_PIPELINE;
  u64 A, B; u32 aux = 0;
  if ((flags & ~plain) == 0u && (kind == RGB_MSG_AER_REPLY || kind == RGB_MSG_WRITTEN)) {
    if ((d.w[2] | d.w[3] | d.w[4] | d.w[5]) != 0ull) return false;
    A = d.w[6]; B = d.w[7];
  } else if ((flags & ~plain) == RGB_F_WROTE && kind == RGB_MSG_AER) {
    const u64 fst = d.w[3], lst = d.w[4], la = d.w[7];
    if ((d.w[2] | d.w[5]) != 0ull || fst > lst || lst - fst > 0xFFFFull || la > lst || lst - la > 0xFFFFull) return false;
    A = lst; B = d.w[6];
    aux = (u32)(lst - fst) | ((u32)(lst - la) << 16);
  } else if ((flags & ~plain) == (RGB_F_REPLY | RGB_F_REPLY_SUCCESS) && (kind == RGB_MSG_AER || kind == RGB_MSG_WRITTEN)) {
    const u64 term = d.w[2], next = d.w[3], last = d.w[4], lterm = d.w[5], ci = d.w[6], la = d.w[7];
    if (next == 0ull) return false;
    A = next - 1ull; B = term;
    const u64 d1 = A - last, d2 = term - lterm, d3 = ci + 512ull - A, d4 = A + 1ull - la;
    if (last > A || d1 > 0xFFull || lterm > term || d2 > 0xFull || ci + 512ull < A || d3 > 0x3FFull || la > A + 1ull ||
        d4 > 0x3FFull)
      return false;
    aux = (u32)d1 | ((u32)d2 << 8) | ((u32)d3 << 12) | ((u32)d4 << 22);
  } else {
    return false;
  }
  d.w[1] = (u64)(flags | RGB_F_COMPACT) | ((u64)aux << 32);
  d.w[2] = A; d.w[3] = B;
  return true;
}

template <int N, int KIND, bool PRE = false, bool TR = false, bool SEQXP = (KIND < 0)>
__device__ __forceinline__ void process_message(const rgb_dev &dev, const ulonglong2 m0, const ulonglong2 m1,
                                                const ulonglong2 m2, const ulonglong2 m3, u32 i,
                                                rgb_rpc *__restrict__ rpcs, u32 rpc_slot_base,
                                                u32 msg_index_base, Dec &out, u64 *t_loaded = nullptr,
                                                const ulonglong2 *pre = nullptr, unsigned swz = 0,
                                                const ulonglong2 *prepeers = nullptr,
                                                const ulonglong2 *preruns = nullptr, ulonglong2 *rpc_stash = nullptr) {
  LaneT<TR, (N >= 6 && KIND == RGB_MSG_AER), SEQXP> L;
  L.rpc_stash = rpc_stash;
  L.wc_k = -1; L.wc_start = L.wc_term = L.wc_next = 0;
  L.server = (u32)(m0.x & 0xFFFFFFFFull);
  const unsigned wire_kind = (unsigned)((m0.x >> 32) & 0xFF);
  L.kind = KIND >= 0 ? (unsigned)KIND : wire_kind;
  L.from = (unsigned)((m0.x >> 40) & 0xFF);
  L.mflags = (unsigned)((m0.x >> 48) & 0xFF);
  L.gap = (unsigned)((m0.x >> 56) & 0xFF);
  L.term = m0.y; L.a = m1.x; L.b = m1.y; L.c = m2.x;
  L.n_entries = (u32)(m2.y & 0xFFFFFFFFull);
  L.n_run0 = (u32)(m2.y >> 32);
  L.run0_term = m3.x; L.run1_term = m3.y;
  if (L.n_run0 > L.n_entries) L.n_run0 = L.n_entries;

  if (L.kind == RGB_MSG_NOP) {
    make_decision(out, L.server, 0, RGB_NONE, 0, 0, 0, 0, 0, 0, 0, 0, 0, 0);
    return;
  }
  if (L.server >= dev.n_servers || wire_kind != L.kind) {
    make_decision(out, L.server, 0xFF, RGB_NONE, 0, wire_kind, RGB_F_UNHANDLED, 0, 0, 0, 0, 0, 0, 0);
    return;
  }
  u64 *hot = dev.hot + (size_t)L.server * RGB_HOT_WORDS;
  const ulonglong2 *hp = reinterpret_cast<const ulonglong2 *>(hot);
  ulonglong2 h0, h1, h2, h3, h4, h5, h6, h7;
  if (RGB_KNOB(dev, 8u)) { h0 = h1 = h2 = h3 = h4 = h5 = h6 = h7 = make_ulonglong2(0, 0); h0.y = 0x1Full << PK_PRESENT_SH; }
  else if (PRE) {
    h0 = pre[HOT_P_TERM ^ swz]; h1 = pre[HOT_P_CI ^ swz]; h2 = pre[HOT_P_LI ^ swz]; h3 = pre[HOT_P_LW ^ swz];
    h4 = pre[HOT_P_SI ^ swz]; h5 = pre[HOT_P_FIRST ^ swz]; h6 = pre[HOT_P_LRT ^ swz]; h7 = pre[HOT_P_PEND ^ swz];
  } else {
    h0 = ldg16(TR, hp + HOT_P_TERM); h1 = ldg16(TR, hp + HOT_P_CI); h2 = ldg16(TR, hp + HOT_P_LI); h3 = ldg16(TR, hp + HOT_P_LW);
    h4 = ldg16(TR, hp + HOT_P_SI); h5 = ldg16(TR, hp + HOT_P_FIRST); h6 = ldg16(TR, hp + HOT_P_LRT); h7 = ldg16(TR, hp + HOT_P_PEND);
  }
#ifdef RGB_PROFILE
  L.prof_noprobe = RGB_KNOB(dev, 32u); L.prof_nloads = 0;
#endif
#ifdef RGB_X_DECLINE_HIST
  L.dbg_hist = dev.dbg_buf;
#endif
  if (decltype(L)::seqx_ok) { L.seqx = dev.seq_ranges; L.n_seqx = dev.n_seq_ranges; } else { L.seqx = nullptr; L.n_seqx = 0; }
  L.qry_base = dev.qry;
  L.q_loaded = false; L.q_dirty = 0; L.hb_mask = 0;
  L.qself = 0; L.hb_term = L.hb_qi = L.q_consensus = 0; L.cancel_mask = 0;
#pragma unroll
  for (int i = 0; i < 8; ++i) L.qp[i] = 0;
  L.runs = dev.runs + (size_t)L.server * dev.max_runs * 2;
  L.peers = dev.peers + (size_t)L.server * dev.peer_stride;
  L.max_runs = dev.max_runs;
  L.peers_loaded = false; L.dmi = L.dni = L.dcs = 0; L.dcs_ci = 0;
  L.peers_lds = prepeers; L.peers_swz = swz; L.pdirty = 0;
  L.runs_lds = preruns;
  constexpr bool PL = !TR && PRE && rgb_class_slice(1, (unsigned)N) == 32u &&
                      (KIND == RGB_MSG_AER_REPLY || KIND == RGB_MSG_APPEND || KIND == RGB_MSG_PIPELINE_RPCS);
  if (!PL && (L.kind == RGB_MSG_AER_REPLY || L.kind == RGB_MSG_APPEND || L.kind == RGB_MSG_PIPELINE_RPCS ||
              L.kind == RGB_MSG_TRANSFER_LEADERSHIP) &&
      !RGB_KNOB(dev, 64u)) {
    load_peers<N>(L);
  }
#ifdef RGB_PROFILE
  if (RGB_KNOB(dev, 64u)) {
#pragma unroll
    for (int i = 0; i < 8; ++i) { L.pmi[i] = 0; L.pni[i] = 1; L.pcs[i] = 0; }
    L.peers_loaded = true;
  }
#endif
  if (t_loaded && RGB_KNOB(dev, 16u)) {
#ifndef RGB_HOST_EMULATION
    asm volatile("s_waitcnt vmcnt(0)" ::"v"(h0.x), "v"(h6.y) : "memory");
#endif
    *t_loaded = wall_clock64();
  }
  L.ct = h0.x; L.pk = h0.y; L.ci = h1.x; L.la = h1.y; L.li = h2.x; L.lt = h2.y; L.lwi = h3.x;
  L.lwt = h3.y; L.si = h4.x; L.st = h4.y; L.first = h5.x; L.lrs = h5.y; L.lrt = h6.x;
  L.prs = h6.y; L.prt = h7.x; L.pend = h7.y; L.vote_reqs = false;
  constexpr bool TM = KIND < 0 || KIND == RGB_MSG_ELECTION_TIMEOUT || KIND == RGB_MSG_PRE_VOTE_RPC ||
                      KIND == RGB_MSG_PRE_VOTE_RESULT;
  u64 token0 = 0;
  L.token = 0; L.macver = 0;
  if (TM && (L.kind == RGB_MSG_ELECTION_TIMEOUT || L.kind == RGB_MSG_PRE_VOTE_RPC || L.kind == RGB_MSG_PRE_VOTE_RESULT)) {
    const ulonglong2 tm = ldg16(TR, reinterpret_cast<const ulonglong2 *>(qry_row(L) + QRY_TOKEN));
    L.token = token0 = tm.x; L.macver = tm.y;
  }
  L.flags = 0; L.inv = 0; L.has_reply = false; L.reply_to = RGB_NONE;
  L.r_term = L.r_next = L.r_last = L.r_lterm = 0; L.w_first = L.w_last = 0;
  L.n_runs = (unsigned)pk_get(L.pk, PK_NRUNS_SH, 5);
  L.push_cnt = 0;
  L.cond_dirty = false; L.cr0 = L.cr1 = L.cr2 = L.cr3 = 0;
  L.po_floor = 0; L.po_cut = UNDEF;

  const unsigned role0 = role_of(L);
  const unsigned pkhi0 = (unsigned)(L.pk >> 56);
  const u64 ci0 = L.ci, la0 = L.la;
  const unsigned n_runs0 = L.n_runs;
  unsigned n_rpcs = 0;
  int rc = 0;
  unsigned role1 = role0;
  bool go = true;
  if (role0 == RGB_ROLE_AWAIT_CONDITION) {
    bool reprocess = false;
    rc = handle_await_condition<N>(L, reprocess, dev.cond + (size_t)L.server * 4);
    go = !rc && reprocess;
    if (go) { L.flags |= RGB_F_REPROCESSED; role1 = role_of(L); }
  }
  if (go && role1 != RGB_ROLE_FOLLOWER) {
    bool reprocess = false;
    switch (role1) {
      case RGB_ROLE_LEADER:          rc = handle_leader<N, PL>(L, reprocess, dev, rpcs,
                                                           (rpc_slot_base + i) * (N > 1 ? N - 1 : 1),
                                                           msg_index_base + i, n_rpcs); break;
      case RGB_ROLE_CANDIDATE:       rc = handle_candidate<N>(L, reprocess); break;
      case RGB_ROLE_PRE_VOTE:        rc = handle_pre_vote<N>(L, reprocess); break;
      default: L.flags |= RGB_F_UNHANDLED; break;
    }
    go = !rc && reprocess;
    if (go) L.flags |= RGB_F_REPROCESSED;
  }
  if (go) rc = handle_follower<N>(L);
#ifdef RGB_PROFILE
  if (t_loaded && RGB_KNOB(dev, 16u)) t_loaded[2] = wall_clock64();
#endif
  if (rc) {
    make_decision(out, L.server, role0, RGB_NONE, 0, L.kind, RGB_F_INVARIANT, (u32)rc, 0, 0, 0, 0, ci0, la0);
    return;
  }

#ifndef RGB_HOST_EMULATION
  __builtin_amdgcn_s_waitcnt(0x0F70);
#endif
  if (RGB_KNOB(dev, 1u)) { L.n_runs = n_runs0; L.push_cnt = 0; L.cond_dirty = false; L.dmi = L.dni = L.dcs = 0; L.dcs_ci = 0; L.pdirty = 0; }
  if (L.n_runs != n_runs0 || L.push_cnt) {
    u64 *runs = const_cast<u64 *>(L.runs);
    unsigned nr = L.n_runs;
    if (nr > L.max_runs) {
      unsigned shift = nr - L.max_runs;
      unsigned in_mem = nr - L.push_cnt;
      for (unsigned k = shift; k < in_mem; ++k) {
        const u64 rs = ldg8(TR, runs + 2 * k), rt = ldg8(TR, runs + 2 * k + 1);
        runs[2 * (k - shift)] = rs;
        runs[2 * (k - shift) + 1] = rt;
      }
      nr = L.max_runs;
      L.flags |= RGB_F_RUNS_OVERFLOW;
      u64 nf;
      if (L.push_cnt >= nr) nf = (L.push_cnt == 2 && nr == 2) ? L.prs : L.lrs;
      else nf = ldg8(TR, runs);
      L.first = nf;
      L.n_runs = nr;
    }
    if (L.push_cnt == 2) { runs[2 * (nr - 2)] = L.prs; runs[2 * (nr - 2) + 1] = L.prt; }
    if (L.push_cnt >= 1) { runs[2 * (nr - 1)] = L.lrs; runs[2 * (nr - 1) + 1] = L.lrt; }
  }
  L.pk = pk_set(L.pk, PK_NRUNS_SH, 5, L.n_runs);
  if (L.cond_dirty) {
    ulonglong2 *cp = reinterpret_cast<ulonglong2 *>(dev.cond + (size_t)L.server * 4);
    ST16(cp, make_ulonglong2(L.cr0, L.cr1));
    ST16(cp + 1, make_ulonglong2(L.cr2, L.cr3));
  }
  const bool q_reset = ((pkhi0 >> (PK_QPEER_SH - 56)) & 1u) && !pk_get(L.pk, PK_QPEER_SH, 1);
  if ((L.q_dirty || q_reset) && !RGB_KNOB(dev, 1u)) {
    u64 *q = qry_row(L);
    if (L.q_dirty & 1u) q[0] = L.qself;
#pragma unroll
    for (int i = 0; i < N; ++i)
      if (q_reset || (L.q_dirty & (2u << i))) q[1 + i] = L.qp[i];
  }
  if (PL) {
    if (L.pdirty | L.dcs_ci) {
#pragma unroll
      for (int w = 0; w < 2 * N; ++w)
        if (L.pdirty & (1u << w)) ST8(L.peers + w, prow_get(L, (unsigned)w));
#pragma unroll
      for (int k = 0; k < N; ++k)
        if (L.dcs_ci & (1u << k)) ST8(L.peers + PEER_CS(k, N), L.ci);
    }
  } else if (L.dmi | L.dni | L.dcs | L.dcs_ci) {
#pragma unroll
    for (int k = 0; k < N; ++k) {
      if (L.dmi & (1u << k)) ST8(L.peers + PEER_MI(k, N), L.pmi[k]);
      if (L.dni & (1u << k)) ST8(L.peers + PEER_NI(k, N), L.pni[k]);
      if (L.dcs & (1u << k)) ST8(L.peers + PEER_CS(k, N), L.pcs[k]);
      else if (L.dcs_ci & (1u << k)) ST8(L.peers + PEER_CS(k, N), L.ci);
    }
  }
  if (((pkhi0 >> (PK_PENDX_SH - 56)) & 1u) && !RGB_KNOB(dev, 1u)) {
    u64 *q = qry_row(L);
    u64 s0 = ldg8(TR, q + QRY_PEND_LO), e0 = ldg8(TR, q + QRY_PEND_LO + 1), s1 = ldg8(TR, q + QRY_PEND_HI),
        e1 = ldg8(TR, q + QRY_PEND_HI + 1);
    if (s0 < L.po_floor) s0 = L.po_floor;
    if (s1 < L.po_floor) s1 = L.po_floor;
    if (L.po_cut != UNDEF) {
      if (L.po_cut == 0) { s0 = 1; e0 = 0; s1 = 1; e1 = 0; }
      else { if (e0 >= L.po_cut) e0 = L.po_cut - 1; if (e1 >= L.po_cut) e1 = L.po_cut - 1; }
    }
    bool v0 = s0 <= e0, v1 = s1 <= e1;
    const bool newest = range_nonempty(L) && L.pend <= L.li;
    if (v1 && newest && e1 + 1 == L.pend) { L.pend = s1; v1 = false; }
    else if (v1 && !newest && range_nonempty(L) && e1 == L.li) { L.pend = s1; v1 = false; }
    else if (!v1 && v0 && newest && e0 + 1 == L.pend) { L.pend = s0; v0 = false; }
    else if (!v1 && v0 && !newest && range_nonempty(L) && e0 == L.li) { L.pend = s0; v0 = false; }
    if (!v1 && v0) { s1 = s0; e1 = e0; v1 = true; v0 = false; }
    q[QRY_PEND_LO] = v0 ? s0 : 1; q[QRY_PEND_LO + 1] = v0 ? e0 : 0;
    q[QRY_PEND_HI] = v1 ? s1 : 1; q[QRY_PEND_HI + 1] = v1 ? e1 : 0;
    L.pk = pk_set(L.pk, PK_PENDX_SH, 1, v1 ? 1 : 0);
  }
  ulonglong2 *ho = reinterpret_cast<ulonglong2 *>(hot);
  if (!RGB_KNOB(dev, 1u)) {
  if (L.n_runs < 2) { L.prs = 0; L.prt = 0; }
  if (!TR && PRE) {
#pragma unroll
    for (int k = 0; k < 8; ++k) {
      const ulonglong2 o = pre[(unsigned)k ^ swz];
      ulonglong2 n;
      switch (k) {
        case HOT_P_TERM: n = make_ulonglong2(L.ct, L.pk); break;
        case HOT_P_CI: n = make_ulonglong2(L.ci, L.la); break;
        case HOT_P_LI: n = make_ulonglong2(L.li, L.lt); break;
        case HOT_P_LW: n = make_ulonglong2(L.lwi, L.lwt); break;
        case HOT_P_SI: n = make_ulonglong2(L.si, L.st); break;
        case HOT_P_FIRST: n = make_ulonglong2(L.first, L.lrs); break;
        case HOT_P_LRT: n = make_ulonglong2(L.lrt, L.prs); break;
        default: n = make_ulonglong2(L.prt, L.pend); break;
      }
      if (n.x != o.x || n.y != o.y) ST16(ho + k, n);
    }
  } else {
  if (L.ct != h0.x || L.pk != h0.y) ST16(ho + HOT_P_TERM, make_ulonglong2(L.ct, L.pk));
  if (L.ci != h1.x || L.la != h1.y) ST16(ho + HOT_P_CI, make_ulonglong2(L.ci, L.la));
  if (L.li != h2.x || L.lt != h2.y) ST16(ho + HOT_P_LI, make_ulonglong2(L.li, L.lt));
  if (L.lwi != h3.x || L.lwt != h3.y) ST16(ho + HOT_P_LW, make_ulonglong2(L.lwi, L.lwt));
  if (L.si != h4.x || L.st != h4.y) ST16(ho + HOT_P_SI, make_ulonglong2(L.si, L.st));
  if (L.first != h5.x || L.lrs != h5.y) ST16(ho + HOT_P_FIRST, make_ulonglong2(L.first, L.lrs));
  if (L.lrt != h6.x || L.prs != h6.y) ST16(ho + HOT_P_LRT, make_ulonglong2(L.lrt, L.prs));
  if (L.prt != h7.x || L.pend != h7.y) ST16(ho + HOT_P_PEND, make_ulonglong2(L.prt, L.pend));
  }
  if (TM && L.token != token0) ST8(qry_row(L) + QRY_TOKEN, L.token);
  }

  u64 w2 = 0, w3 = 0, w4 = 0, w5 = 0;
  if (L.has_reply || L.vote_reqs) { w2 = L.r_term; w3 = L.r_next; w4 = L.r_last; w5 = L.r_lterm; }
  else if (L.flags & RGB_F_WROTE) { w3 = L.w_first; w4 = L.w_last; }
  if ((L.flags & RGB_F_SEND_HEARTBEATS) || L.kind == RGB_MSG_CONSISTENT_QUERY) { w2 = L.hb_term; w5 = L.hb_qi; }
  if (L.flags & RGB_F_QUERY_QUORUM) w3 = L.q_consensus;
  make_decision(out, L.server, role_of(L), L.has_reply ? L.reply_to : (unsigned)RGB_NONE, n_rpcs, L.kind,
                L.flags, 0, w2, w3, w4, w5, L.ci, L.la, L.hb_mask, L.cancel_mask);
#ifdef RGB_PROFILE
  if (t_loaded) { t_loaded[1] = L.prof_nloads; if (RGB_KNOB(dev, 16u)) t_loaded[3] = wall_clock64(); }
#endif
}

template <int N, bool TR>
__device__ __forceinline__ void fuse_pipeline_step(const rgb_dev &dev, Dec &d, u32 i, rgb_rpc *__restrict__ rpcs,
                                                   u32 rpc_slot_base, u32 msg_index_base) {
#ifndef RGB_HOST_EMULATION
  __builtin_amdgcn_s_waitcnt(0x0F70);
  asm volatile("" ::: "memory");
#endif
  const u64 m0x = (d.w[0] & 0xFFFFFFFFull) | ((u64)RGB_MSG_PIPELINE_RPCS << 32) | ((u64)RGB_NONE << 40);
  Dec e;
  process_message<N, RGB_MSG_PIPELINE_RPCS, false, TR>(dev, make_ulonglong2(m0x, 0), make_ulonglong2(0, 0), make_ulonglong2(0, 0),
                                                        make_ulonglong2(0, 0), i, rpcs, rpc_slot_base, msg_index_base, e);
  const u32 ef = (u32)e.w[1];
  if (ef & (RGB_F_INVARIANT | RGB_F_UNHANDLED)) return;
  d.w[0] = (d.w[0] & ~(0xFFull << 48)) | (e.w[0] & (0xFFull << 48));
  d.w[1] = (d.w[1] & ~(u64)RGB_F_PIPELINE) | (u64)ef;
}
__device__ __forceinline__ bool fuse_wanted(const rgb_dev &dev, const Dec &d) {
  const unsigned kind = (unsigned)(d.w[0] >> 56), role = (unsigned)((d.w[0] >> 32) & 0xFF);
  return dev.fuse_pipeline && ((u32)d.w[1] & RGB_F_PIPELINE) && !((u32)d.w[1] & RGB_F_INVARIANT) && role == RGB_ROLE_LEADER &&
         (kind == RGB_MSG_AER_REPLY || kind == RGB_MSG_WRITTEN);
}

#if defined(RGB_X_DECLINE_HIST) && !defined(RGB_HOST_EMULATION)
#define FP_DECLINE(cls, code) do { atomicAdd(dev.dbg_buf + (cls) * 32 + (code), 1ull); return false; } while (0)
#define FP_TAKEN(cls) atomicAdd(dev.dbg_buf + (cls) * 32, 1ull)
#else
#define FP_DECLINE(cls, code) return false
#define FP_TAKEN(cls) do { } while (0)
#endif

struct PairSt {
  ulonglong2 *p;
  ulonglong2 a, b;
  unsigned m;
};
__device__ __forceinline__ void pair_record(PairSt *ps, ulonglong2 *p, bool sa, const ulonglong2 a, bool sb, const ulonglong2 b) {
  if (ps != nullptr) {
    ps->p = p; ps->a = a; ps->b = b; ps->m = (sa ? 1u : 0u) | (sb ? 2u : 0u);
  }
}
__device__ __forceinline__ u64 shfl64(u64 v, int src) {
  return (u64)(u32)__shfl((int)(u32)v, src, 64) | ((u64)(u32)__shfl((int)(u32)(v >> 32), src, 64) << 32);
}
__device__ __forceinline__ void pair_store(const PairSt &st, u32 lane) {
  const int t = (int)(threadIdx.x & ~63u) + (int)(lane & ~1u);
#pragma unroll
  for (int k = 0; k < 2; ++k) {
    const int src = t + k;
    const u64 pp = shfl64((u64)(uintptr_t)st.p, src);
    const unsigned m = (unsigned)__shfl((int)st.m, src, 64);
    const bool second = (lane & 1u) != 0u;
    const u64 ax = shfl64(st.a.x, src), ay = shfl64(st.a.y, src), bx = shfl64(st.b.x, src), by = shfl64(st.b.y, src);
    if (m & (second ? 2u : 1u))
      ST16(reinterpret_cast<ulonglong2 *>((uintptr_t)pp) + (second ? 1 : 0), second ? make_ulonglong2(bx, by) : make_ulonglong2(ax, ay));
  }
}

__device__ __forceinline__ bool fast_aer(const rgb_dev &dev, const ulonglong2 m0, const ulonglong2 m1, const ulonglong2 m2,
                                         const ulonglong2 m3, const ulonglong2 *pre, unsigned swz, Dec &out,
                                         PairSt *pst) {
  const u32 server = (u32)(m0.x & 0xFFFFFFFFull);
  const unsigned wire_kind = (unsigned)((m0.x >> 32) & 0xFF), from = (unsigned)((m0.x >> 40) & 0xFF);
  const unsigned mflags = (unsigned)((m0.x >> 48) & 0xFF), gap = (unsigned)((m0.x >> 56) & 0xFF);
  const u32 n_entries = (u32)(m2.y & 0xFFFFFFFFull), n_run0 = (u32)(m2.y >> 32);
  if (wire_kind != RGB_MSG_AER || server >= dev.n_servers || from >= 8u || mflags != 0) FP_DECLINE(0, 1);
  if (gap != 0) FP_DECLINE(0, 2);
  if (n_run0 < n_entries) FP_DECLINE(0, 4);
  const ulonglong2 h0 = pre[HOT_P_TERM ^ swz], h1 = pre[HOT_P_CI ^ swz], h2 = pre[HOT_P_LI ^ swz], h3 = pre[HOT_P_LW ^ swz],
                   h5 = pre[HOT_P_FIRST ^ swz], h6 = pre[HOT_P_LRT ^ swz], h7 = pre[HOT_P_PEND ^ swz];
  const u64 ct = h0.x, pk = h0.y, la = h1.y, li = h2.x, lt = h2.y, lwi = h3.x, first = h5.x, lrs = h5.y, lrt = h6.x,
            pend = h7.y;
  if (pk_get(pk, PK_ROLE_SH, 3) != RGB_ROLE_FOLLOWER) FP_DECLINE(0, 5);
  if (pk_get(pk, PK_LEADER_SH, 4) != from) FP_DECLINE(0, 6);
  if (pk_get(pk, PK_PENDX_SH, 1) || pk_get(pk, PK_NRUNS_SH, 5) == 0) FP_DECLINE(0, 7);
  const u64 term = m0.y, pli = m1.x, plt = m1.y, leader_commit = m2.x, eterm = m3.x;
  if (term != ct) FP_DECLINE(0, 8);
  if (!(first <= li) || li == UNDEF) FP_DECLINE(0, 9);
  if (pli != li) FP_DECLINE(0, 10);
  if (li < lrs) FP_DECLINE(0, 11);
  if (plt != lrt) FP_DECLINE(0, 12);
  if (lt != lrt) FP_DECLINE(0, 13);
  if (n_entries != 0 && eterm != lrt) FP_DECLINE(0, 14);
  if (la > li + 1 || lwi > li || pend > li + 1) FP_DECLINE(0, 15);
  if (pk_get(pk, PK_NRUNS_SH, 5) < 2 && (h6.y | h7.x) != 0) FP_DECLINE(0, 16);
  FP_TAKEN(0);
  const u64 fst = li + 1, lst = li + n_entries;
  u32 flags = RGB_F_LEADER_MSG;
  const u64 ci = leader_commit;
  u64 nla = la;
  const u64 at = lst < ci ? lst : ci;
  if (at > la) { nla = at; flags |= RGB_F_APPLIED | RGB_F_AUX_EVAL; }
  ulonglong2 *ho = reinterpret_cast<ulonglong2 *>(dev.hot + (size_t)server * RGB_HOT_WORDS);
  static_assert(HOT_P_LI == HOT_P_CI + 1 && (HOT_P_CI & 1) == 0, "commit and last_index pieces: one aligned 32-byte unit");
  pair_record(pst, ho + HOT_P_CI, ci != h1.x || nla != la, make_ulonglong2(ci, nla), n_entries != 0, make_ulonglong2(li + n_entries, lt));
  if (n_entries == 0) {
    make_decision(out, server, RGB_ROLE_FOLLOWER, from, 0, RGB_MSG_AER, flags | RGB_F_REPLY | RGB_F_REPLY_SUCCESS, 0, term,
                  li + 1, lwi, h3.y, ci, nla);
    return true;
  }
  flags |= RGB_F_WROTE;
  make_decision(out, server, RGB_ROLE_FOLLOWER, RGB_NONE, 0, RGB_MSG_AER, flags, 0, 0, fst, lst, 0, ci, nla);
  return true;
}

__device__ __forceinline__ bool fast_written(const rgb_dev &dev, const ulonglong2 m0, const ulonglong2 m1,
                                             const ulonglong2 *pre, unsigned swz, Dec &out, PairSt *pst) {
  const u32 server = (u32)(m0.x & 0xFFFFFFFFull);
  const unsigned wire_kind = (unsigned)((m0.x >> 32) & 0xFF), mflags = (unsigned)((m0.x >> 48) & 0xFF);
  if (wire_kind != RGB_MSG_WRITTEN || server >= dev.n_servers || mflags != 0) FP_DECLINE(2, 1);
  const ulonglong2 h0 = pre[HOT_P_TERM ^ swz], h1 = pre[HOT_P_CI ^ swz], h2 = pre[HOT_P_LI ^ swz], h3 = pre[HOT_P_LW ^ swz],
                   h4 = pre[HOT_P_SI ^ swz], h5 = pre[HOT_P_FIRST ^ swz], h6 = pre[HOT_P_LRT ^ swz], h7 = pre[HOT_P_PEND ^ swz];
  const u64 ct = h0.x, pk = h0.y, li = h2.x, si = h4.x, first = h5.x, lrs = h5.y, lrt = h6.x, pend = h7.y;
  const unsigned l4 = (unsigned)pk_get(pk, PK_LEADER_SH, 4);
  if (pk_get(pk, PK_ROLE_SH, 3) != RGB_ROLE_FOLLOWER) FP_DECLINE(2, 2);
  if (l4 == SLOT_NONE4) FP_DECLINE(2, 3);
  if (pk_get(pk, PK_PENDX_SH, 1) || pk_get(pk, PK_NRUNS_SH, 5) == 0) FP_DECLINE(2, 4);
  const u64 term = m0.y, from = m1.x, to = m1.y;
  if (!(first <= li) || li == UNDEF || from > to) FP_DECLINE(2, 5);
  if (to > li) FP_DECLINE(2, 6);
  if (to < lrs) FP_DECLINE(2, 7);
  if (to < first) FP_DECLINE(2, 8);
  if (lrt != term) FP_DECLINE(2, 9);
  if (si != UNDEF && si >= first) FP_DECLINE(2, 10);
  if (pend > li + 1) FP_DECLINE(2, 11);
  if (pk_get(pk, PK_NRUNS_SH, 5) < 2 && (h6.y | h7.x) != 0) FP_DECLINE(2, 12);
  if (pend <= li && pend <= to && pend < from) FP_DECLINE(2, 13);
  FP_TAKEN(2);
  u64 npend = pend;
  if (pend <= li && to + 1 > pend) npend = to + 1;
  const bool changed = !(h3.x == to && h3.y == term);
  ulonglong2 *ho = reinterpret_cast<ulonglong2 *>(dev.hot + (size_t)server * RGB_HOT_WORDS);
  static_assert(HOT_P_PEND == HOT_P_LW + 1 && (HOT_P_LW & 1) == 0, "last_written and pending pieces: one aligned 32-byte unit");
  pair_record(pst, ho + HOT_P_LW, changed, make_ulonglong2(to, term), npend != pend, make_ulonglong2(h7.x, npend));
  u32 flags = 0;
  u64 w2 = 0, w3 = 0, w4 = 0, w5 = 0;
  unsigned reply_to = RGB_NONE;
  if (changed) {
    flags = RGB_F_REPLY | RGB_F_REPLY_SUCCESS;
    w2 = ct; w3 = li + 1; w4 = to; w5 = term; reply_to = slot4to8(l4);
  }
  make_decision(out, server, RGB_ROLE_FOLLOWER, reply_to, 0, RGB_MSG_WRITTEN, flags, 0, w2, w3, w4, w5, h1.x, h1.y);
  return true;
}

template <int N, bool TR = false, bool PROW = false>
__device__ __forceinline__ bool fast_aer_reply(const rgb_dev &dev, const ulonglong2 m0, const ulonglong2 m1,
                                               const ulonglong2 *pre, unsigned swz, Dec &out,
                                               const ulonglong2 *prow = nullptr,
                                               const ulonglong2 *rrow = nullptr) {
  const u32 server = (u32)(m0.x & 0xFFFFFFFFull);
  const unsigned wire_kind = (unsigned)((m0.x >> 32) & 0xFF), peer = (unsigned)((m0.x >> 40) & 0xFF);
  const unsigned mflags = (unsigned)((m0.x >> 48) & 0xFF);
  const ulonglong2 h0 = pre[HOT_P_TERM ^ swz], h1 = pre[HOT_P_CI ^ swz], h2 = pre[HOT_P_LI ^ swz], h3 = pre[HOT_P_LW ^ swz],
                   h4 = pre[HOT_P_SI ^ swz], h5 = pre[HOT_P_FIRST ^ swz], h6 = pre[HOT_P_LRT ^ swz], h7 = pre[HOT_P_PEND ^ swz];
  const u64 ct = h0.x, pk = h0.y, ci0 = h1.x, la = h1.y, li = h2.x, lwi = h3.x, si = h4.x, st = h4.y, first = h5.x,
            lrs = h5.y, lrt = h6.x, prs = h6.y, prt = h7.x;
  const unsigned present = (unsigned)pk_get(pk, PK_PRESENT_SH, 8), voters = (unsigned)pk_get(pk, PK_VOTER_SH, 8);
  const unsigned self = (unsigned)pk_get(pk, PK_SELF_SH, 4), n_runs = (unsigned)pk_get(pk, PK_NRUNS_SH, 5);
#if defined(RGB_X_DECLINE_HIST) && !defined(RGB_HOST_EMULATION)
  if (wire_kind != RGB_MSG_AER_REPLY || server >= dev.n_servers || peer >= (unsigned)N) FP_DECLINE(1, 1);
  if (mflags != RGB_MF_SUCCESS) FP_DECLINE(1, 2);
  if (dev.fuse_pipeline) FP_DECLINE(1, 9);
  if (pk_get(pk, PK_ROLE_SH, 3) != RGB_ROLE_LEADER) FP_DECLINE(1, 3);
  if (m0.y != ct) FP_DECLINE(1, 4);
  if (!((present >> peer) & 1u)) FP_DECLINE(1, 5);
  if (n_runs < 2 && (h6.y | h7.x) != 0) FP_DECLINE(1, 6);
#else
  const bool ok = (wire_kind == RGB_MSG_AER_REPLY) & (server < dev.n_servers) & (peer < (unsigned)N) &
                  (mflags == RGB_MF_SUCCESS) & (dev.fuse_pipeline == 0u) &
                  (pk_get(pk, PK_ROLE_SH, 3) == RGB_ROLE_LEADER) & (m0.y == ct) & (((present >> (peer & 7u)) & 1u) != 0u) &
                  !((n_runs < 2) & ((h6.y | h7.x) != 0));
  if (!ok) return false;
#endif
  u64 *peers = dev.peers + (size_t)server * dev.peer_stride;
  u64 wm[N], wn[N];
  if (PROW || prow != nullptr) {
    const unsigned psw = rgb_wide_peers((unsigned)N) ? swz << 1 : swz;
#pragma unroll
    for (int k = 0; k < N; ++k) { const ulonglong2 v = prow[(unsigned)k ^ psw]; wm[k] = v.x; wn[k] = v.y; }
  } else {
    const ulonglong2 *pp = reinterpret_cast<const ulonglong2 *>(peers);
#pragma unroll
    for (int k = 0; k < N; ++k) { const ulonglong2 v = ldg16(TR, pp + k); wm[k] = v.x; wn[k] = v.y; }
  }
  u64 mi_new = 0, ni_new = 0; bool mi_dirty = false, ni_dirty = false;
  if (PROW) {
    const unsigned psw = rgb_wide_peers((unsigned)N) ? swz << 1 : swz;
    const ulonglong2 pv = prow[peer ^ psw];
    mi_dirty = m1.y > pv.x; ni_dirty = m1.x > pv.y;
    mi_new = mi_dirty ? m1.y : pv.x; ni_new = ni_dirty ? m1.x : pv.y;
#pragma unroll
    for (int i = 0; i < N; ++i) wm[i] = ((unsigned)i == peer) ? mi_new : wm[i];
  } else {
#pragma unroll
    for (int i = 0; i < N; ++i) {
      if ((unsigned)i != peer) continue;
      mi_new = wm[i]; ni_new = wn[i];
      if (m1.y > wm[i]) { mi_new = m1.y; mi_dirty = true; wm[i] = m1.y; }
      if (m1.x > wn[i]) { ni_new = m1.x; ni_dirty = true; }
    }
  }
  u64 v[N + 1]; bool use[N + 1]; int n = 1;
  v[N] = lwi; use[N] = true;
#pragma unroll
  for (int i = 0; i < N; ++i) {
    const bool u = ((unsigned)i != self) && ((present >> i) & 1u) && ((voters >> i) & 1u);
    v[i] = wm[i]; use[i] = u; n += u ? 1 : 0;
  }
  const u64 p = agreed_commit<N + 1>(v, use, n);
  u64 t = UNDEF;
  if (first <= li && p >= first && p <= li) {
    if (p >= lrs) t = lrt;
    else if (n_runs >= 2 && p >= prs) t = prt;
    else {
      bool found = false;
      const ulonglong2 *rt = reinterpret_cast<const ulonglong2 *>(dev.runs + (size_t)server * dev.max_runs * 2u);
      const int lds_runs = rrow != nullptr ? RGB_RUNS_LDS : 0;
#pragma unroll 1
      for (int k = (int)n_runs - 3; k >= lds_runs && !found; --k) {
        const ulonglong2 r = ldg16(TR, rt + k);
        if (p >= r.x) { t = r.y; found = true; }
      }
      if (rrow != nullptr) {
#pragma unroll
        for (int k = RGB_RUNS_LDS - 1; k >= 0; --k) {
          if (!found && (unsigned)k + 3u <= n_runs) {
            const ulonglong2 r = rrow[(unsigned)k ^ swz];
            if (p >= r.x) { t = r.y; found = true; }
          }
        }
      }
      if (!found) FP_DECLINE(1, 8);
    }
  }
  FP_TAKEN(1);
  if (t == UNDEF && si != UNDEF && si == p) t = st;
  u64 ci = ci0, nla = la;
  u32 flags = RGB_F_PIPELINE;
  if (t != UNDEF && t == ct) ci = p;
  if (ci > ci0) flags |= RGB_F_AUX_EVAL;
  if (ci > la) { const u64 to = li < ci ? li : ci; if (to >= la + 1) { nla = to; flags |= RGB_F_APPLIED; } }
  if (mi_dirty | ni_dirty) ST16(reinterpret_cast<ulonglong2 *>(peers) + peer, make_ulonglong2(mi_new, ni_new));
  if (ci != ci0 || nla != la)
    ST16(reinterpret_cast<ulonglong2 *>(dev.hot + (size_t)server * RGB_HOT_WORDS) + HOT_P_CI, make_ulonglong2(ci, nla));
  make_decision(out, server, RGB_ROLE_LEADER, RGB_NONE, 0, RGB_MSG_AER_REPLY, flags, 0, 0, 0, 0, 0, ci, nla);
  return true;
}

#define RGB_IO_SLOT 5
#define RGB_HOT_SLOT 9

template <int N, int KIND, bool SEQXP = (KIND < 0)>
__global__ __launch_bounds__(RGB_TICK_BLOCK, RGB_MIN_WAVES(N)) void rgb_tick_kernel(rgb_dev dev, const rgb_msg *__restrict__ msgs,
                                                                  u32 n, const u32 *__restrict__ n_dev,
                                                                  rgb_decision *__restrict__ dec,
                                                                  rgb_rpc *__restrict__ rpcs, u32 rpc_slot_base,
                                                                  u32 msg_index_base) {
  __shared__ ulonglong2 io[RGB_TICK_BLOCK * RGB_IO_SLOT];
  const u32 lane = threadIdx.x;
  const u32 base = blockIdx.x * RGB_TICK_BLOCK;
  if (n_dev != nullptr) {
    const u32 nd = *n_dev;
    n = nd < n ? nd : n;
    if (base >= n) return;
  }
  const u32 cnt = n - base < RGB_TICK_BLOCK ? n - base : RGB_TICK_BLOCK;
  const ulonglong2 *src = reinterpret_cast<const ulonglong2 *>(msgs + base);
  {
    const u32 last = cnt * 4u - 1u;
    ulonglong2 v[4];
#pragma unroll
    for (int k = 0; k < 4; ++k) {
      const u32 piece = k * RGB_TICK_BLOCK + lane;
      v[k] = ld16<true>(src + (piece < last ? piece : last));
    }
#pragma unroll
    for (int k = 0; k < 4; ++k) {
      const u32 piece = k * RGB_TICK_BLOCK + lane;
      io[(piece >> 2) * RGB_IO_SLOT + (piece & 3u)] = v[k];
    }
  }
  lds_barrier();
  const bool active = lane < cnt;
  Dec d;
  if (active) {
    const ulonglong2 m0 = io[lane * RGB_IO_SLOT + 0], m1 = io[lane * RGB_IO_SLOT + 1],
                     m2 = io[lane * RGB_IO_SLOT + 2], m3 = io[lane * RGB_IO_SLOT + 3];
    process_message<N, KIND, false, false, SEQXP>(dev, m0, m1, m2, m3, base + lane, rpcs, rpc_slot_base, msg_index_base, d);
    if (fuse_wanted(dev, d)) fuse_pipeline_step<N, false>(dev, d, base + lane, rpcs, rpc_slot_base, msg_index_base);
    (void)compact_decision(d);
    io[lane * RGB_IO_SLOT + 0] = make_ulonglong2(d.w[0], d.w[1]);
    io[lane * RGB_IO_SLOT + 1] = make_ulonglong2(d.w[2], d.w[3]);
    io[lane * RGB_IO_SLOT + 2] = make_ulonglong2(d.w[4], d.w[5]);
    io[lane * RGB_IO_SLOT + 3] = make_ulonglong2(d.w[6], d.w[7]);
  }
  lds_barrier();
  if (RGB_KNOB(dev, 2u)) return;
  ulonglong2 *dst = reinterpret_cast<ulonglong2 *>(dec + base);
// ... 1 lines not shown
  for (int k = 0; k < 4; ++k) {
    const u32 piece = k * RGB_TICK_BLOCK + lane;
    const u32 j = piece >> 2, part = piece & 3u;
    if (j < cnt && (part < 2u || !((u32)io[j * RGB_IO_SLOT].y & RGB_F_COMPACT)))
      store16_nt((void *)(dst + piece), io[j * RGB_IO_SLOT + part]);
  }
}


struct rgb_tick_plan {
  u32 blk_end[RGB_N_CLASSES];
  u32 off[RGB_N_CLASSES];
  u32 cnt[RGB_N_CLASSES];
};

#define RGB_CLASS_ORDER 0x201CDEB756A8943ull
__host__ __device__ constexpr int rgb_class_at(unsigned q) { return (int)((RGB_CLASS_ORDER >> (4u * q)) & 0xFu); }
static_assert(rgb_class_at(0) == 3 && rgb_class_at(1) == 4 && rgb_class_at(2) == 9 && rgb_class_at(3) == 8 &&
              rgb_class_at(4) == 10 && rgb_class_at(5) == 6 && rgb_class_at(6) == 5 && rgb_class_at(7) == 7 &&
              rgb_class_at(8) == 11 && rgb_class_at(9) == 14 && rgb_class_at(10) == 13 && rgb_class_at(11) == 12 &&
              rgb_class_at(12) == 1 && rgb_class_at(13) == 0 && rgb_class_at(14) == 2, "class order");

__host__ __device__ __forceinline__ void rgb_make_plan(const u32 (&n)[RGB_N_CLASSES], rgb_tick_plan &p, unsigned n_members) {
  u32 blocks = 0;
#pragma unroll
  for (int q = 0; q < RGB_N_CLASSES; ++q) {
    const int c = rgb_class_at((unsigned)q);
    u32 off = 0, cnt = 0;
#pragma unroll
    for (int k = 0; k < RGB_N_CLASSES; ++k) { off += k < c ? n[k] : 0u; cnt = k == c ? n[k] : cnt; }
    const u32 sl = rgb_class_slice(c, n_members);
    blocks += (cnt + sl - 1) / sl;
    p.blk_end[q] = blocks; p.off[q] = off; p.cnt[q] = cnt;
  }
}

__device__ __forceinline__ u32 rgb_xcc_id() {
#ifdef RGB_HOST_EMULATION
  return 0;
#else
  u32 xcc;
  asm volatile("s_getreg_b32 %0, hwreg(HW_REG_XCC_ID, 0, 4)" : "=s"(xcc));
  return xcc;
#endif
}

#ifndef RGB_TRAIN_SPIN_LIMIT
#ifdef RGB_HOST_EMULATION
#define RGB_TRAIN_SPIN_LIMIT 16u
#else
#define RGB_TRAIN_SPIN_LIMIT 20000u
#endif
#endif
#ifndef RGB_TRAIN_SLEEP
#define RGB_TRAIN_SLEEP 4
#endif

__device__ __forceinline__ u32 rgb_take_ticket(u32 *ctr, const u32 *err) {
  u32 v = 0;
#ifdef RGB_HOST_EMULATION
  if (threadIdx.x == 0) v = atomicAdd(ctr, 1u);
  if (threadIdx.x == 1) v = *err;
#else
  if (threadIdx.x == 0) v = __hip_atomic_fetch_add(ctr, 1u, __ATOMIC_RELAXED, __HIP_MEMORY_SCOPE_AGENT);
  if (threadIdx.x == 1) v = __hip_atomic_load(err, __ATOMIC_RELAXED, __HIP_MEMORY_SCOPE_AGENT);
#endif
  return v;
}
__device__ __forceinline__ u32 rgb_ticket_value(u32 raw) {
#ifdef RGB_HOST_EMULATION
  return __shfl(raw, 0, 64);
#else
  return (u32)__builtin_amdgcn_readfirstlane((int)raw);
#endif
}
__device__ __forceinline__ u32 rgb_ticket_err(u32 raw) {
#ifdef RGB_HOST_EMULATION
  return __shfl(raw, 1, 64);
#else
  return (u32)__builtin_amdgcn_readlane((int)raw, 1);
#endif
}

template <int N, bool TR>
__device__ __forceinline__ bool rgb_tick_slice(const rgb_dev &dev, ulonglong2 *io, const int cls, const u32 base,
                                               const u32 cnt, const u32 SL, const rgb_msg *__restrict__ msgs,
                                               rgb_decision *__restrict__ dec, rgb_rpc *__restrict__ rpcs,
                                               u32 rpc_slot_base, u32 msg_index_base, u32 *__restrict__ ctl,
                                               const unsigned char *__restrict__ stamps,
                                               u32 *__restrict__ ticket_ctr = nullptr, u32 *next_ticket = nullptr,
                                               u32 shard = 0, u32 lane_in = 0, const u32 *place_word = nullptr,
                                               u32 place_bit = 0) {
  const u32 lane = TR ? lane_in : (u32)threadIdx.x;
#ifdef RGB_PROFILE
  u64 t0 = 0, t1 = 0, t2 = 0, t2b = 0, tl[4] = {0, 0, 0, 0};
  if (!TR && RGB_KNOB(dev, 16u)) t0 = wall_clock64();
#endif
  const bool lead_cls = rgb_lead_class(cls);
  constexpr bool PEERS_LDS = rgb_class_slice(1, (unsigned)N) == 32u;
  constexpr bool PEERS_WIDE = TR && rgb_train_class_slice(1, (unsigned)N) == 32u && !PEERS_LDS;
  const bool RUNS_LDS = TR && (PEERS_LDS || PEERS_WIDE) && dev.max_runs >= (u32)RGB_RUNS_LDS;
  bool AER_RUNS = false;
#if defined(RGB_X_TRAIN_TIMELINE) && !defined(RGB_HOST_EMULATION)
  u64 tt[7] = {0, 0, 0, 0, 0, 0, 0};
  unsigned tt_spins = 0;
#define RGB_TT(k) do { if (TR) tt[k] = wall_clock64(); } while (0)
#else
#define RGB_TT(k) do { } while (0)
#endif
  RGB_TT(0);
  const ulonglong2 *src = reinterpret_cast<const ulonglong2 *>(msgs + base);
  unsigned need_raw = 0;
  if (TR && lane < cnt) need_raw = (unsigned)stamps[base + lane];
  {
    const u32 last = cnt * 4u - 1u;
    const bool half = rgb_half_msg_class(cls);
#pragma unroll
    for (int k = 0; k < 4; ++k) {
      if ((u32)k * 16u >= SL) break;
      const u32 piece = k * RGB_TICK_BLOCK + lane;
      const u32 r = piece >> 2;
      const u32 sp = (r << 2) | ((piece & 3u) ^ ((r >> 2) & 3u));
      if (!half || (sp & 2u) == 0u) glds16<GLDS_NT>(src + (sp < last ? sp : last), io + k * RGB_TICK_BLOCK);
    }
    glds_wait();
  }
  lds_barrier();
#ifdef RGB_PROFILE
  if (!TR && RGB_KNOB(dev, 16u)) t1 = wall_clock64();
#endif
  const bool active = lane < cnt;
  const u32 mswz = (lane >> 2) & 3u;
  const ulonglong2 m0 = io[lane * 4 + (0 ^ mswz)], m1 = io[lane * 4 + (1 ^ mswz)];
  ulonglong2 m2 = io[lane * 4 + (2 ^ mswz)], m3 = io[lane * 4 + (3 ^ mswz)];
  if (rgb_half_msg_class(cls)) {
    m2 = make_ulonglong2(0, 0); m3 = make_ulonglong2(0, 0);
    if (cls == 2 && active && (((m0.x >> 48) & 0xFFull) & RGB_MF_SEQ2)) m3 = ld16<true>(src + lane * 4u + 3u);
  }
  RGB_TT(1);
  if (TR && !PEERS_LDS && cls == 0 && dev.max_runs >= (u32)RGB_RUNS_LDS)
    AER_RUNS = __ballot(active && m1.y != m0.y) != 0ull;
  const u32 sv = (u32)(m0.x & 0xFFFFFFFFull);
  const bool has_srv = TR && active && sv < dev.n_servers && ((m0.x >> 32) & 0xFFull) != RGB_MSG_NOP;
  unsigned char *seqp = nullptr;
  unsigned need = 0;
  if (TR) {
    if (__ballot(has_srv && rgb_shard_of_server(sv, (unsigned)N) != shard) != 0ull) {
      if (lane == 0) atomicOr(ctl, (u32)RGB_TRAIN_ERR_ORDER);
      return false;
    }
    seqp = dev.seq + rgb_seq_index(has_srv ? sv : 0u, dev.n_members, dev.seq_stride);
    need = has_srv ? need_raw : 0u;
    unsigned spins = 0;
    bool late = has_srv;
    for (;;) {
      if (late) {
#ifdef RGB_HOST_EMULATION
        const unsigned cur = *seqp;
#else
        const unsigned cur = __hip_atomic_load(seqp, __ATOMIC_RELAXED, __HIP_MEMORY_SCOPE_AGENT);
#endif
        late = cur != need;
      }
      if (__ballot(late) == 0ull) break;
      spins += 1;
#if defined(RGB_X_TRAIN_TIMELINE) && !defined(RGB_HOST_EMULATION)
      tt_spins = spins;
#endif
      bool give_up = spins > RGB_TRAIN_SPIN_LIMIT;
#ifndef RGB_HOST_EMULATION
      if ((spins & 15u) == 0u && __hip_atomic_load(ctl, __ATOMIC_RELAXED, __HIP_MEMORY_SCOPE_AGENT) != 0u) give_up = true;
      __builtin_amdgcn_s_sleep(RGB_TRAIN_SLEEP);
      if (spins > 64u) __builtin_amdgcn_s_sleep(127);
#endif
      if (give_up) {
        if (lane == 0) atomicOr(ctl, (u32)RGB_TRAIN_ERR_SPIN);
        return false;
      }
    }
  }
  RGB_TT(2);
  constexpr bool PRE = true;
  constexpr int ROWS = TR ? GLDS_SC1 : GLDS_DEFAULT;
  u64 pf0 = 0, pf1 = 0;
  lds_barrier();
  {
    const u32 srv = (active && sv < dev.n_servers) ? sv : 0u;
    if (lead_cls && !PEERS_LDS && !PEERS_WIDE) {
      const u64 *pp = dev.peers + (size_t)srv * dev.peer_stride;
      pf0 = ldg8(TR, pp);
      if (3 * N > 16) pf1 = ldg8(TR, pp + 16);
    }
#pragma unroll
    for (int k = 0; k < 8; ++k) {
      if ((u32)k * 8u >= SL) break;
      const u32 r = 8 * k + (lane >> 3);
      const u32 sj = __shfl(srv, (int)r, 64);
      glds16<ROWS>(reinterpret_cast<const ulonglong2 *>(dev.hot + (size_t)sj * RGB_HOT_WORDS) + ((lane & 7u) ^ ((r >> 1) & 7u)),
                   io + k * RGB_TICK_BLOCK);
    }
    if (!PEERS_LDS && AER_RUNS) {
#pragma unroll
      for (int k = 0; k < 8; ++k) {
        const u32 r = 8 * k + (lane >> 3);
        const u32 sj = __shfl(srv, (int)r, 64);
        glds16<ROWS>(reinterpret_cast<const ulonglong2 *>(dev.runs + (size_t)sj * dev.max_runs * 2u) + ((lane & 7u) ^ ((r >> 1) & 7u)),
                     io + (8 + k) * RGB_TICK_BLOCK);
      }
    }
    if (PEERS_WIDE && lead_cls) {
#pragma unroll
      for (int k = 0; k < 8; ++k) {
        const u32 r = 4 * k + (lane >> 4);
        const u32 sj = __shfl(srv, (int)r, 64);
        const u32 pcx = (lane & 15u) ^ (((r >> 1) & 7u) << 1);
        if (pcx < 12u)
          glds16<ROWS>(reinterpret_cast<const ulonglong2 *>(dev.peers + (size_t)sj * 24u) + pcx, io + (4 + k) * RGB_TICK_BLOCK);
      }
      if (RUNS_LDS) {
#pragma unroll
        for (int k = 0; k < 4; ++k) {
          const u32 r = 8 * k + (lane >> 3);
          const u32 sj = __shfl(srv, (int)r, 64);
          glds16<ROWS>(reinterpret_cast<const ulonglong2 *>(dev.runs + (size_t)sj * dev.max_runs * 2u) + ((lane & 7u) ^ ((r >> 1) & 7u)),
                       io + (12 + k) * RGB_TICK_BLOCK);
        }
      }
    }
    if (PEERS_LDS && lead_cls) {
#pragma unroll
      for (int k = 0; k < 4; ++k) {
        const u32 r = 8 * k + (lane >> 3);
        const u32 sj = __shfl(srv, (int)r, 64);
        glds16<ROWS>(reinterpret_cast<const ulonglong2 *>(dev.peers + (size_t)sj * 16u) + ((lane & 7u) ^ ((r >> 1) & 7u)),
                     io + (4 + k) * RGB_TICK_BLOCK);
      }
      if (RUNS_LDS) {
#pragma unroll
        for (int k = 0; k < 4; ++k) {
          const u32 r = 8 * k + (lane >> 3);
          const u32 sj = __shfl(srv, (int)r, 64);
          glds16<ROWS>(reinterpret_cast<const ulonglong2 *>(dev.runs + (size_t)sj * dev.max_runs * 2u) + ((lane & 7u) ^ ((r >> 1) & 7u)),
                       io + (8 + k) * RGB_TICK_BLOCK);
        }
      }
    }
    glds_wait();
  }
  lds_barrier();
  RGB_TT(3);
  const ulonglong2 *hrow = io + lane * 8;
  const unsigned hswz = (lane >> 1) & 7u;
  const ulonglong2 *prow = (PEERS_LDS && lead_cls) ? io + 4 * RGB_TICK_BLOCK + lane * 8
                           : (PEERS_WIDE && lead_cls) ? io + 4 * RGB_TICK_BLOCK + lane * 16 : nullptr;
  const ulonglong2 *rrow = (RUNS_LDS && PEERS_WIDE && lead_cls) ? io + 12 * RGB_TICK_BLOCK + lane * 8
                           : ((RUNS_LDS && PEERS_LDS && lead_cls) || (!PEERS_LDS && AER_RUNS)) ? io + 8 * RGB_TICK_BLOCK + lane * 8 : nullptr;
#ifndef RGB_HOST_EMULATION
  asm volatile("" ::"v"(pf0), "v"(pf1));
#endif
  Dec d;
  u64 *tlp = nullptr;
#ifdef RGB_PROFILE
  if (!TR) tlp = tl;
#endif
  const bool STASH = TR && (PEERS_LDS || PEERS_WIDE) && lead_cls && rpcs != nullptr;
  ulonglong2 *stash = STASH ? io + lane * 8 : nullptr;
  u64 ct0 = 0;
  if (STASH) ct0 = hrow[HOT_P_TERM ^ hswz].x;
  bool done = false;
  PairSt pst;
  pst.p = nullptr; pst.a = pst.b = make_ulonglong2(0, 0); pst.m = 0;
  if (active) {
    if (cls == 0) done = fast_aer(dev, m0, m1, m2, m3, hrow, hswz, d, &pst);
    else if (cls == 1) done = fast_aer_reply<N, TR, (PEERS_LDS || PEERS_WIDE)>(dev, m0, m1, hrow, hswz, d, prow, rrow);
    else if (cls == 2) done = fast_written(dev, m0, m1, hrow, hswz, d, &pst);
  }
  if (cls == 0 || cls == 2) pair_store(pst, lane);
#if defined(RGB_PROFILE) && !defined(RGB_HOST_EMULATION)
  u64 tf = 0; unsigned n_fast = 0;
  if (!TR && RGB_KNOB(dev, 16u)) { tf = wall_clock64(); n_fast = (unsigned)__popcll(__ballot(done)); }
#endif
  if (active && !done) {
#define RGB_CASE(RANK, KIND)                                                                            \
  case RANK:                                                                                            \
    RGB_MARK("begin", RANK)                                                                             \
    process_message<N, KIND, PRE, TR>(dev, m0, m1, m2, m3, base + lane, rpcs, rpc_slot_base, msg_index_base, d, tlp, \
                                      hrow, hswz, prow, rrow, stash);                                   \
    RGB_MARK("end", RANK)                                                                               \
    break;
    switch (cls) {
      RGB_CASE(0, RGB_MSG_AER) RGB_CASE(1, RGB_MSG_AER_REPLY) RGB_CASE(2, RGB_MSG_WRITTEN)
      RGB_CASE(3, RGB_MSG_APPEND) RGB_CASE(4, RGB_MSG_PIPELINE_RPCS) RGB_CASE(5, RGB_MSG_REQUEST_VOTE)
      RGB_CASE(6, RGB_MSG_VOTE_RESULT) RGB_CASE(7, RGB_MSG_AWAIT_TIMEOUT)
      RGB_CASE(8, RGB_MSG_ELECTION_TIMEOUT) RGB_CASE(9, RGB_MSG_PRE_VOTE_RPC)
      RGB_CASE(10, RGB_MSG_PRE_VOTE_RESULT) RGB_CASE(11, RGB_MSG_SNAPSHOT_WRITTEN)
      RGB_CASE(12, RGB_MSG_HEARTBEAT_RPC) RGB_CASE(13, RGB_MSG_HEARTBEAT_REPLY)
      default:
        if (((m0.x >> 32) & 0xFFull) == RGB_MSG_TRANSFER_LEADERSHIP)
          process_message<N, RGB_MSG_TRANSFER_LEADERSHIP, PRE, TR>(dev, m0, m1, m2, m3, base + lane, rpcs, rpc_slot_base,
                                                                   msg_index_base, d, tlp, hrow, hswz, prow);
        else
          process_message<N, RGB_MSG_CONSISTENT_QUERY, PRE, TR>(dev, m0, m1, m2, m3, base + lane, rpcs, rpc_slot_base,
                                                                msg_index_base, d, tlp, hrow, hswz, prow);
        break;
    }
#undef RGB_CASE
#if defined(RGB_PROFILE) && !defined(RGB_HOST_EMULATION)
    if (!TR && RGB_KNOB(dev, 16u)) { t2 = wall_clock64(); asm volatile("s_waitcnt vmcnt(0)" ::: "memory"); t2b = wall_clock64(); }
#endif
  }
  const unsigned n_parked = (STASH && active) ? (unsigned)((d.w[0] >> 48) & 0xFFull) : 0u;
  if (dev.fuse_pipeline && (cls == 1 || cls == 2)) {
    const bool want = active && fuse_wanted(dev, d);
    if (__ballot(want) != 0ull && want) fuse_pipeline_step<N, TR>(dev, d, base + lane, rpcs, rpc_slot_base, msg_index_base);
  }
  const bool is_compact = active && compact_decision(d);
  const u64 cmask = __ballot(is_compact);
  RGB_TT(4);
  if (TR) {
#ifndef RGB_HOST_EMULATION
    __builtin_amdgcn_s_waitcnt(0x0F70);
    asm volatile("" ::: "memory");
#endif
    if (has_srv && seqp != nullptr) *seqp = (unsigned char)(need + 1u);
    if (ticket_ctr != nullptr) *next_ticket = rgb_take_ticket(ticket_ctr, ctl);
    if (place_word != nullptr && lane == 0) {
#ifdef RGB_HOST_EMULATION
      *const_cast<u32 *>(place_word) |= place_bit;
#else
      (void)__hip_atomic_fetch_or(const_cast<u32 *>(place_word), place_bit, __ATOMIC_RELAXED, __HIP_MEMORY_SCOPE_AGENT);
#endif
    }
  }
  if (STASH) {
    const unsigned n_rp = n_parked;
    if (__ballot(n_rp != 0u) != 0ull) {
      rgb_rpc *slot0 = rpcs + (size_t)(rpc_slot_base + base + lane) * (N > 1 ? N - 1 : 1);
      const u64 w0 = (u64)(msg_index_base + base + lane) | ((d.w[0] & 0xFFFFFFFFull) << 32);
#pragma unroll
      for (unsigned j = 0; j < (N > 1 ? (unsigned)N - 1u : 1u) && j < 4u; ++j) {
        if (j < n_rp) {
          const ulonglong2 a = stash[2u * j], b = stash[2u * j + 1u];
          store_rpc(slot0 + j, w0, a.x, ct0, a.y, b.x, d.w[6], b.y);
        }
      }
    }
  }
  RGB_TT(5);
  lds_barrier();
  if (active) {
    io[lane * RGB_IO_SLOT + 0] = make_ulonglong2(d.w[0], d.w[1]);
    io[lane * RGB_IO_SLOT + 1] = make_ulonglong2(d.w[2], d.w[3]);
    if (!is_compact) {
      io[lane * RGB_IO_SLOT + 2] = make_ulonglong2(d.w[4], d.w[5]);
      io[lane * RGB_IO_SLOT + 3] = make_ulonglong2(d.w[6], d.w[7]);
    }
  }
  lds_barrier();
  if (!TR && RGB_KNOB(dev, 2u)) return true;
  ulonglong2 *dst = reinterpret_cast<ulonglong2 *>(dec + base);
#pragma unroll
  for (int k = 0; k < 4; ++k) {
    const u32 piece = k * RGB_TICK_BLOCK + lane;
    const u32 j = piece >> 2, part = piece & 3u;
    if (j < cnt && (part < 2u || !((cmask >> j) & 1ull)))
      store16_nt((void *)(dst + piece), io[j * RGB_IO_SLOT + part]);
  }
#if defined(RGB_X_TRAIN_TIMELINE) && !defined(RGB_HOST_EMULATION)
  if (TR && dev.dbg_buf != nullptr && lane == 0 && blockIdx.x < (1u << 20)) {
    u64 *o = dev.dbg_buf + (size_t)blockIdx.x * 8;
    tt[6] = wall_clock64();
    for (int k = 0; k < 7; ++k) o[k] = tt[k];
    o[7] = (u64)(unsigned)cls | ((u64)cnt << 8) | ((u64)tt_spins << 32) | ((u64)rgb_xcc_id() << 56);
  }
#endif
#ifdef RGB_PROFILE
  if (!TR && RGB_KNOB(dev, 16u)) {
    unsigned mx = (unsigned)tl[1], sm = (unsigned)tl[1], nz = tl[1] ? 1u : 0u;
#pragma unroll
    for (int o = 32; o >= 1; o >>= 1) {
      const unsigned a = __shfl_xor(mx, o, 64), b = __shfl_xor(sm, o, 64), c = __shfl_xor(nz, o, 64);
      mx = a > mx ? a : mx; sm += b; nz += c;
    }
    if (lane == 0) {
      u64 *o = dev.dbg_buf + (size_t)blockIdx.x * 8;
      o[0] = t0; o[1] = t1 | ((tl[0] > t1 ? tl[0] - t1 : 0) << 40);
      o[2] = t2 | ((t2b > t2 ? t2b - t2 : 0) << 40) | ((u64)cls << 60); o[3] = wall_clock64();
      o[4] = mx; o[5] = sm | ((tl[2] > t1 ? tl[2] - t1 : 0) << 24); o[6] = nz | ((tl[3] > t1 ? tl[3] - t1 : 0) << 24);
      o[7] = cnt | ((u64)n_fast << 8) | ((tf > t1 ? tf - t1 : 0) << 24);
    }
  }
#endif
  return true;
}

template <int N>
__global__ __launch_bounds__(RGB_TICK_BLOCK, RGB_CLASS_MIN_WAVES(N)) void rgb_tick_classes_kernel(
    rgb_dev dev, const rgb_msg *__restrict__ msgs, rgb_tick_plan plan, const u32 *__restrict__ fam_dev,
    rgb_decision *__restrict__ dec, rgb_rpc *__restrict__ rpcs, u32 rpc_slot_base, u32 msg_index_base) {
  __shared__ ulonglong2 io[RGB_TICK_BLOCK * RGB_HOT_SLOT];
  const u32 blk_id = blockIdx.x;
  u32 q = 0, off, ncls, blk;
  if (fam_dev != nullptr) {
    u32 n[RGB_N_CLASSES];
#pragma unroll
    for (int c = 0; c < RGB_N_CLASSES; ++c) n[c] = fam_dev[2 * c] + fam_dev[2 * c + 1];
    rgb_tick_plan p;
// ... 150 lines not shown
  (void)rgb_tick_slice<N, true>(args.dev, io, cls, off + lbase, cnt, SL, args.msgs + toff, args.dec + toff, rp, 0,
                                args.index_base + (u32)toff, args.ctl, args.stamps + toff, nullptr, &unused, x,
                                threadIdx.x, args.ctl + RGB_TRAIN_CTL_MARK + 32u * (k & (RGB_TRAIN_MARK_WORDS - 1u)),
                                1u << ((rgb_xcc_id() - x) & (RGB_TRAIN_SHARDS - 1u)));
}

__global__ void rgb_train_prolog_kernel(u32 *__restrict__ ctl, u32 clear) {
  if (threadIdx.x < RGB_TRAIN_MARK_WORDS) {
    u32 v = ctl[RGB_TRAIN_CTL_MARK + 32u * threadIdx.x];
#pragma unroll
    for (int o = 32; o >= 1; o >>= 1) v |= __shfl_xor(v, o, 64);
    if (threadIdx.x == 0 && (v & (v - 1u)) != 0u) atomicOr(ctl, (u32)RGB_TRAIN_ERR_PLACEMENT);
  }
  __syncthreads();
  if (clear)
    for (u32 w = 1u + threadIdx.x; w < RGB_TRAIN_CTL_WORDS; w += blockDim.x) ctl[w] = 0u;
}

template <int N>
__global__ __launch_bounds__(RGB_TICK_BLOCK, RGB_TRAIN_PERSIST_MIN_WAVES(N)) void rgb_train_kernel(rgb_train_args args) {
  __shared__ ulonglong2 io[rgb_class_slice(1, (unsigned)N) == 32u ? 12 * RGB_TICK_BLOCK : 16 * RGB_TICK_BLOCK];
  u32 x;
  {
    const u32 n_xcc = args.n_xcc;
    const u32 xcc = rgb_xcc_id() & (RGB_TRAIN_SHARDS - 1u);
    if (n_xcc >= RGB_TRAIN_SHARDS) x = xcc;
    else {
      u32 a = 0;
      if (threadIdx.x == 0) a = atomicAdd(args.ctl + RGB_TRAIN_CTL_ARRIVE + (xcc & (n_xcc - 1u)), 1u);
      a = rgb_ticket_value(a);
      x = (xcc & (n_xcc - 1u)) + n_xcc * (a % (RGB_TRAIN_SHARDS / n_xcc));
    }
  }
  u32 raw = rgb_take_ticket(args.ctl + RGB_TRAIN_CTL_TICKET * (1u + x), args.ctl);
  u32 t = 0, cum = 0;
  for (;;) {
#if defined(RGB_HOST_EMULATION) || !defined(__HIP_DEVICE_COMPILE__)
    const rgb_train_args *A = &args;
    u32 lane = threadIdx.x;
#else
    typedef const __attribute__((address_space(4))) rgb_train_args *args_ptr;
    args_ptr A = (args_ptr)__builtin_amdgcn_kernarg_segment_ptr();
    asm volatile("" : "+s"(A));
    u32 lane = threadIdx.x;
    asm volatile("" : "+v"(lane));
#endif
    const rgb_dev dev = A->dev;
    const u32 k = rgb_ticket_value(raw);
    if (rgb_ticket_err(raw) != 0u) break;
    const rgb_train_tick *plan = A->plan;
    const u32 n_ticks = A->n_ticks;
    u32 nr = 0;
    while (t < n_ticks) {
      nr = plan[t].n_rows;
      if (k - cum < nr) break;
      cum += nr; ++t;
    }
    if (t >= n_ticks) break;
    const rgb_train_tick *p = plan + t;
    const u32 e = A->row_tab[(size_t)t * A->tab_rpt + (k - cum)];
    const u32 pc = e >> 24;
    u32 *const tk = A->ctl + RGB_TRAIN_CTL_TICKET * (1u + x);
    if (pc == RGB_PC_SNAP) {
      if (t != 0u && p->snap != 0u && A->snap_rows != nullptr) {
        if (!rgb_train_snap_slice<N>(dev, x, e & 0xFFFFFFu, lane,
                                     A->snap_stamps + (size_t)(p->snap - 1u) * dev.seq_stride * RGB_TRAIN_SHARDS,
                                     A->snap_rows + (size_t)(p->snap - 1u) * (dev.n_servers / (u32)N), A->ctl))
          break;
      }
      raw = rgb_take_ticket(tk, A->ctl);
      continue;
    }
    const int cls = (int)(pc >> 1);
    const u32 off = p->off[pc][x], ncls = p->cnt[pc][x];
    const u32 SL = rgb_train_class_slice(cls, (unsigned)N);
    const u32 lbase = (e & 0xFFFFFFu) * SL;
    if (lbase >= ncls) { raw = rgb_take_ticket(tk, A->ctl); continue; }
    const u32 cnt = ncls - lbase < SL ? ncls - lbase : SL;
    const u32 tick_stride = A->tick_stride;
    const size_t toff = tick_stride ? (size_t)t * tick_stride : (size_t)p->msg_base;
    rgb_rpc *rp = A->rpcs ? A->rpcs + (tick_stride ? (size_t)(t % A->rpc_ring) * tick_stride : toff) * (N > 1 ? N - 1 : 1) : nullptr;
    lds_barrier();
    raw = 0;
    if (!rgb_tick_slice<N, true>(dev, io, cls, off + lbase, cnt, SL, A->msgs + toff, A->dec + toff, rp, 0,
                                 A->index_base + (u32)toff, A->ctl, A->stamps + toff, tk, &raw, x, lane))
      break;
  }
}

__global__ void rgb_train_calibrate_kernel(u32 *__restrict__ out) {
  if (threadIdx.x == 0) {
    const u32 xcc = rgb_xcc_id();
    atomicOr(out, 1u << xcc);
    atomicOr(out + 1, 1u << ((xcc - blockIdx.x) & (RGB_TRAIN_SHARDS - 1u)));
  }
}

__global__ void rgb_train_seq_kernel(rgb_dev dev, const rgb_msg *__restrict__ msgs, u32 n, unsigned char *__restrict__ seq_cnt,
                                     unsigned char *__restrict__ stamps) {
  const u32 i = blockIdx.x * blockDim.x + threadIdx.x;
  if (i >= n) return;
  const u64 w = *reinterpret_cast<const u64 *>(msgs + i);
  const u32 sv = (u32)(w & 0xFFFFFFFFull);
  if (((w >> 32) & 0xFFull) == RGB_MSG_NOP || sv >= dev.n_servers) { stamps[i] = 0; return; }
  const u32 k = rgb_seq_index(sv, dev.n_members, dev.seq_stride);
  const unsigned char c = seq_cnt[k];
  seq_cnt[k] = (unsigned char)(c + 1u);
  stamps[i] = c;
}


#define SYN_FAMILIES RGB_N_FAMILIES

__device__ __forceinline__ u64 sm64(u64 &x) {
  x += 0x9E3779B97F4A7C15ull;
  u64 z = x;
  z = (z ^ (z >> 30)) * 0xBF58476D1CE4E5B9ull;
  z = (z ^ (z >> 27)) * 0x94D049BB133111EBull;
  return z ^ (z >> 31);
}

struct SynMember { u64 ct, ci, la, li, lt, lwi, lwt, pk, first, lrs, lrt, prs, prt; };

template <class Lane>
__device__ __forceinline__ void syn_lane(Lane &T, const SynMember &x, const u64 *runs) {
  T.first = x.first; T.li = x.li; T.lrs = x.lrs; T.lrt = x.lrt; T.prs = x.prs; T.prt = x.prt;
  T.push_cnt = 0; T.n_runs = (unsigned)pk_get(x.pk, PK_NRUNS_SH, 5);
  T.runs = runs; T.runs_lds = nullptr;
#ifdef RGB_PROFILE
  T.prof_noprobe = false; T.prof_nloads = 0;
#endif
}

struct SynMsg {
  u32 server; unsigned kind, from, flags, gap; u64 term, a, b, c; u32 n_entries, n_run0; u64 run0, run1;
  bool off_steady;
};

__device__ __forceinline__ void syn_store(rgb_msg *slot, const SynMsg &m) {
  ulonglong2 *o = reinterpret_cast<ulonglong2 *>(slot);
  u64 w0 = (u64)m.server | ((u64)(m.kind & 0xFF) << 32) | ((u64)(m.from & 0xFF) << 40) |
           ((u64)(m.flags & 0xFF) << 48) | ((u64)(m.gap & 0xFF) << 56);
  o[0] = make_ulonglong2(w0, m.term);
  o[1] = make_ulonglong2(m.a, m.b);
  o[2] = make_ulonglong2(m.c, (u64)m.n_entries | ((u64)m.n_run0 << 32));
  o[3] = make_ulonglong2(m.run0, m.run1);
}

__device__ __forceinline__ SynMsg syn_msg(u32 server, unsigned kind, unsigned from, unsigned flags, u64 term,
                                          u64 a, u64 b, u64 c, u32 n_entries = 0, u32 n_run0 = 0, u64 run0 = 0) {
  SynMsg m;
  m.server = server; m.kind = kind; m.from = from; m.flags = flags; m.gap = 0; m.term = term;
  m.a = a; m.b = b; m.c = c; m.n_entries = n_entries; m.n_run0 = n_run0; m.run0 = run0; m.run1 = 0;
  m.off_steady = false;
  return m;
}

template <int N, class Emit>
__device__ __forceinline__ void synth_group(const rgb_dev &dev, u64 seed, u64 tick, u32 g, Emit &&emit) {
  u64 rs = seed ^ (tick * 0xD1B54A32D192ED03ull) ^ ((u64)g * 0x9E3779B97F4A7C15ull);
  SynMember mb[N];
  int leader = -1, cand = -1, prev = -1, hi = 0;
  u64 lead_ct = 0, maxct = 0;
#pragma unroll
  for (int m = 0; m < N; ++m) {
    const ulonglong2 *hp = reinterpret_cast<const ulonglong2 *>(dev.hot + ((size_t)g * N + m) * RGB_HOT_WORDS);
    const ulonglong2 h0 = hp[HOT_P_TERM], h1 = hp[HOT_P_CI], h2 = hp[HOT_P_LI], h3 = hp[HOT_P_LW], h5 = hp[HOT_P_FIRST],
                     h6 = hp[HOT_P_LRT], h7 = hp[HOT_P_PEND];
    mb[m].ct = h0.x; mb[m].pk = h0.y; mb[m].ci = h1.x; mb[m].la = h1.y; mb[m].li = h2.x;
    mb[m].lt = h2.y; mb[m].lwi = h3.x; mb[m].lwt = h3.y; mb[m].first = h5.x; mb[m].lrs = h5.y;
    mb[m].lrt = h6.x; mb[m].prs = h6.y; mb[m].prt = h7.x;
  }
#pragma unroll
  for (int m = 0; m < N; ++m) {
    const unsigned role = (unsigned)pk_get(mb[m].pk, PK_ROLE_SH, 3);
    if (mb[m].ct > maxct) maxct = mb[m].ct;
    if (role == RGB_ROLE_LEADER && (leader < 0 || mb[m].ct > lead_ct)) { leader = m; lead_ct = mb[m].ct; }
  }
#pragma unroll
  for (int m = 0; m < N; ++m) {
    const unsigned role = (unsigned)pk_get(mb[m].pk, PK_ROLE_SH, 3);
    if (role == RGB_ROLE_CANDIDATE && mb[m].ct == maxct && cand < 0) cand = m;
    if (role == RGB_ROLE_PRE_VOTE && mb[m].ct == maxct && prev < 0) prev = m;
    const bool better = mb[m].ct > mb[hi].ct ||
                        (mb[m].ct == mb[hi].ct && (mb[m].lt > mb[hi].lt ||
                                                   (mb[m].lt == mb[hi].lt && mb[m].li > mb[hi].li)));
    if (better) hi = m;
  }
  auto sid = [&](int m) -> u32 { return g * N + (u32)m; };
  auto other = [&](int m, u64 r) -> int { return N > 1 ? (int)((m + 1 + r % (N - 1)) % N) : m; };

  const bool healthy = leader >= 0 && lead_ct == maxct;
  if (!healthy) {
    const u64 r = sm64(rs);
    if (leader >= 0) {
      int mh = hi == leader ? other(leader, r) : hi;
      emit(syn_msg(sid(leader), RGB_MSG_AER_REPLY, mh, 0, mb[mh].ct, mb[mh].li + 1, mb[mh].lwi, mb[mh].lwt));
    } else if (cand >= 0) {
      emit(syn_msg(sid(cand), RGB_MSG_VOTE_RESULT, other(cand, r), RGB_MF_SUCCESS, mb[cand].ct, 0, 0, 0));
    } else if (prev >= 0) {
      emit(syn_msg(sid(prev), RGB_MSG_PRE_VOTE_RESULT, other(prev, r), RGB_MF_SUCCESS, mb[prev].ct, 0, 0,
                   (dev.qry + (size_t)sid(prev) * RGB_QRY_WORDS)[QRY_TOKEN]));
    } else {
      emit(syn_msg(sid(hi), RGB_MSG_ELECTION_TIMEOUT, RGB_NONE, 0, 0, 0, 0, (r | 1ull) & 0xFFFFFFFFFFFFull));
    }
    return;
  }
  const int l = leader;
  const SynMember &ld = mb[l];
  bool used[N];
#pragma unroll
// ... 993 lines not shown
```

### ra_amd/engine.py

```python
from __future__ import annotations

import ctypes as C
import os
import subprocess

import numpy as np

from . import abi

_CSRC = os.path.join(os.path.dirname(os.path.abspath(__file__)), "csrc")
LIB_PATH = os.environ.get("RGB_LIB") or os.path.join(_CSRC, "libra_gpu_batch.so")

EXPORTS = [
    "rgb_abi_version", "rgb_struct_size", "rgb_strerror", "rgb_default_config", "rgb_open",
    "rgb_close", "rgb_last_hip_error", "rgb_register_groups", "rgb_n_servers", "rgb_upload_state",
    "rgb_download_state", "rgb_submit", "rgb_collect", "rgb_run_ticks_device", "rgb_snapshot",
    "rgb_snapshot_device", "rgb_state_checksum", "rgb_synchronize", "rgb_wait", "rgb_wake", "rgb_in_flight",
    "rgb_route", "rgb_submit_trains", "rgb_peek",
    "rgb_train_bucket", "rgb_train_plan_create", "rgb_train_plan_destroy", "rgb_train_plan_blocks_per_tick",
    "rgb_train_stamp_device", "rgb_train_run_device", "rgb_train_status", "rgb_train_form", "rgb_train_recoveries",
    "rgb_train_plan_create_snap", "rgb_train_run_snap_device", "rgb_snapshot_train_device", "rgb_train_seq_bytes",
    "rgb_train_plan_create_device", "rgb_train_plan_build_device", "rgb_train_plan_download", "rgb_train_plan_fit",
    "rgb_submit_seq", "rgb_set_seq_ranges_device", "rgb_collect_view", "rgb_release",
    "rgb_submit_raw_capacity", "rgb_submit_begin", "rgb_submit_commit", "rgb_submit_raw",
]
COMM_EXPORTS = ["rgb_comm_unique_id", "rgb_comm_init_rank", "rgb_comm_destroy", "rgb_comm_n_ranks", "rgb_comm_rank",
                "rgb_leaderboard_allgather", "rgb_leaderboard_allgather_host", "rgb_comm_last_error"]
EXPORTS += COMM_EXPORTS
SYNTH_EXPORTS = ["rgb_synth_tick_device", "rgb_synth_tick_buckets_device", "rgb_synth_apply_tick_device",
                 "rgb_synth_tick_stamped_device", "rgb_synth_stamps_resync_device",
                 "rgb_synth_snapshot_mark_device", "rgb_synth_set_hint"]
OPTIONAL_IN_OLD_BUILDS = {"rgb_synth_tick_stamped_device", "rgb_synth_stamps_resync_device", "rgb_train_form",
                          "rgb_train_recoveries", "rgb_train_plan_create_snap", "rgb_train_run_snap_device",
                          "rgb_snapshot_train_device", "rgb_train_seq_bytes", "rgb_synth_snapshot_mark_device",
                          "rgb_synth_set_hint", "rgb_train_plan_create_device", "rgb_train_plan_build_device",
                          "rgb_train_plan_download", "rgb_train_plan_fit", "rgb_submit_seq", "rgb_set_seq_ranges_device",
                          "rgb_collect_view", "rgb_release", "rgb_submit_raw_capacity", "rgb_submit_begin",
                          "rgb_submit_commit", "rgb_submit_raw"} | set(COMM_EXPORTS)
WAL_EXPORTS = ["rgb_wal_adler32_device", "rgb_wal_adler32", "rgb_wal_layout", "rgb_wal_frame_device",
               "rgb_wal_frame", "rgb_wal_scan", "rgb_wal_validate",
               "rgb_crc32_device", "rgb_crc32", "rgb_crc32_stream_device", "rgb_crc32_stream", "rgb_segment_layout",
               "rgb_segment_build_device", "rgb_segment_build", "rgb_segment_scan", "rgb_segment_validate"]


class RgbError(RuntimeError):
    def __init__(self, code: int, what: str, hip: int = 0):
        self.code, self.hip = code, hip
        super().__init__(f"{what}: rc={code} ({_strerror(code)})" + (f" hipError={hip}" if hip else ""))


def build(force: bool = False) -> str:
    srcs = [os.path.join(_CSRC, f) for f in ("rgb_kernels.hip", "rgb_api.hip", "rgb_prepare.hip", "rgb_wal.hip", "rgb_wal_host.cpp", "rgb_segment.hip",
                                              "rgb_segment_host.cpp", "rgb_comm.cpp", "rgb_internal.h")]
    srcs.append(os.path.join(_CSRC, "..", "..", "include", "ra_gpu_wal.h"))
    srcs.append(os.path.join(_CSRC, "..", "..", "include", "ra_gpu_batch.h"))
    stale = (not os.path.exists(LIB_PATH)) or any(
        os.path.getmtime(s) > os.path.getmtime(LIB_PATH) for s in srcs)
    if force or stale:
        subprocess.check_call(["make", "-C", _CSRC, "libra_gpu_batch.so"])
    return LIB_PATH


_lib = None


def lib():
    global _lib
    if _lib is not None:
        return _lib
    if not os.path.exists(LIB_PATH):
        raise RuntimeError(
            f"{LIB_PATH} is missing: build it (python -c 'import __graft_entry__ as g; g.build()' "
            "or make -C ra_amd/csrc).  ra_gpu_batch has no CPU fallback.")
    try:
        import torch
    except Exception:
        pass
    L = C.CDLL(LIB_PATH)
    for name in EXPORTS + SYNTH_EXPORTS + WAL_EXPORTS:
        if not hasattr(L, name):
            if os.environ.get("RGB_LIB") and name in OPTIONAL_IN_OLD_BUILDS:
                continue
            raise RuntimeError(f"libra_gpu_batch.so does not export {name}")
    vp, u32, u64p = C.c_void_p, C.c_uint32, C.POINTER(C.c_uint64)
    L.rgb_abi_version.restype = C.c_uint32
    L.rgb_struct_size.restype = C.c_size_t
    L.rgb_struct_size.argtypes = [C.c_int]
    L.rgb_strerror.restype = C.c_char_p
    L.rgb_strerror.argtypes = [C.c_int]
    L.rgb_default_config.argtypes = [vp]
    L.rgb_open.argtypes = [vp, C.POINTER(vp)]
    L.rgb_close.argtypes = [vp]
    L.rgb_last_hip_error.argtypes = [vp]
    L.rgb_register_groups.argtypes = [vp, u32, u32]
    L.rgb_n_servers.restype = C.c_uint32
    L.rgb_n_servers.argtypes = [vp]
    L.rgb_upload_state.argtypes = [vp, u32, u32, vp]
    L.rgb_download_state.argtypes = [vp, u32, u32, vp]
    L.rgb_submit.argtypes = [vp, vp, u32, C.c_uint64]
    if hasattr(L, "rgb_submit_seq"):
        L.rgb_submit_seq.argtypes = [vp, vp, u32, C.c_uint64, vp, u32]
        L.rgb_set_seq_ranges_device.argtypes = [vp, vp, u32]
    L.rgb_collect.argtypes = [vp, vp, u32, C.POINTER(u32), vp, u32, C.POINTER(u32), u64p]
    if hasattr(L, "rgb_collect_view"):
        L.rgb_collect_view.argtypes = [vp, vp]
        L.rgb_release.argtypes = [vp, u32]
    if hasattr(L, "rgb_submit_raw"):
        L.rgb_submit_raw_capacity.restype = C.c_uint32
        L.rgb_submit_raw_capacity.argtypes = [vp, u32]
        L.rgb_submit_begin.argtypes = [vp, u32, vp]
        L.rgb_submit_commit.argtypes = [vp, u32, u32, C.c_uint64]
        L.rgb_submit_raw.argtypes = [vp, vp, u32, u32, C.c_uint64]
    L.rgb_run_ticks_device.argtypes = [vp, vp, u32, vp, vp, vp, u32, vp, vp, vp]
    L.rgb_snapshot.argtypes = [vp, vp]
    L.rgb_snapshot_device.argtypes = [vp, vp, vp]
    L.rgb_state_checksum.argtypes = [vp, u32, u32, u64p]
    L.rgb_synchronize.argtypes = [vp]
    L.rgb_wait.argtypes = [vp, u32]
    L.rgb_wake.argtypes = [vp]
    L.rgb_wake.restype = None
    L.rgb_in_flight.argtypes = [vp]
    L.rgb_peek.argtypes = [vp, C.POINTER(u32), C.POINTER(u32)]
    L.rgb_submit_trains.restype = C.c_uint32
    L.rgb_submit_trains.argtypes = [vp]
    L.rgb_in_flight.restype = C.c_uint32
    L.rgb_route.argtypes = [C.c_uint64, u32]
    L.rgb_route.restype = C.c_uint32
    L.rgb_synth_tick_device.argtypes = [vp, C.c_uint64, C.c_uint64, vp, vp, vp, vp]
    L.rgb_synth_tick_buckets_device.argtypes = [vp, C.c_uint64, C.c_uint64, vp, vp, vp, vp, vp]
    if hasattr(L, "rgb_synth_tick_stamped_device"):
        L.rgb_synth_tick_stamped_device.argtypes = [vp, C.c_uint64, C.c_uint64, vp, vp, vp, vp, vp, vp]
        L.rgb_synth_stamps_resync_device.argtypes = [vp, vp]
    if hasattr(L, "rgb_comm_init_rank"):
        L.rgb_comm_unique_id.argtypes = [vp]
        L.rgb_comm_init_rank.argtypes = [vp, vp, u32, u32, C.POINTER(vp)]
        L.rgb_comm_destroy.argtypes = [vp]
        L.rgb_comm_destroy.restype = None
        L.rgb_comm_n_ranks.argtypes = [vp]
        L.rgb_comm_n_ranks.restype = C.c_uint32
        L.rgb_comm_rank.argtypes = [vp]
        L.rgb_comm_rank.restype = C.c_uint32
        L.rgb_leaderboard_allgather.argtypes = [vp, vp, vp, u32, vp, vp]
        L.rgb_comm_last_error.restype = C.c_char_p
    if hasattr(L, "rgb_debug_inject_train_fault"):
        L.rgb_debug_inject_train_fault.argtypes = [vp, u32]
        L.rgb_debug_inject_train_fault.restype = None
        L.rgb_train_recoveries.argtypes = [vp]
        L.rgb_train_recoveries.restype = C.c_uint32
        L.rgb_train_form.argtypes = [vp]
        L.rgb_train_form.restype = C.c_uint32
    L.rgb_train_bucket.restype = C.c_uint32
    L.rgb_train_bucket.argtypes = [u32, u32, u32, u32]
    L.rgb_train_plan_create.argtypes = [vp, vp, u32, C.POINTER(vp)]
    L.rgb_train_plan_destroy.argtypes = [vp]
    L.rgb_train_plan_destroy.restype = None
    L.rgb_train_plan_blocks_per_tick.restype = C.c_uint32
    L.rgb_train_plan_blocks_per_tick.argtypes = [vp]
    L.rgb_train_stamp_device.argtypes = [vp, vp, vp, u32, vp, u32, vp]
    L.rgb_train_run_device.argtypes = [vp, vp, u32, u32, vp, vp, u32, vp, vp, u32, vp]
    if hasattr(L, "rgb_train_run_snap_device"):
        L.rgb_train_plan_create_snap.argtypes = [vp, vp, u32, u32, C.POINTER(vp)]
        L.rgb_train_run_snap_device.argtypes = [vp, vp, u32, u32, vp, vp, u32, vp, vp, u32, vp, vp, vp]
        L.rgb_snapshot_train_device.argtypes = [vp, vp, vp]
        L.rgb_train_seq_bytes.restype = C.c_uint32
        L.rgb_train_seq_bytes.argtypes = [vp]
        L.rgb_synth_snapshot_mark_device.argtypes = [vp, vp, vp]
    if hasattr(L, "rgb_train_plan_create_device"):
        L.rgb_train_plan_create_device.argtypes = [vp, u32, u32, C.POINTER(vp)]
        L.rgb_train_plan_build_device.argtypes = [vp, vp, u32, u32, vp, vp]
        L.rgb_train_plan_download.argtypes = [vp, vp, u32, vp, vp, u32]
    if hasattr(L, "rgb_train_plan_fit"):
        L.rgb_train_plan_fit.argtypes = [vp, vp, u32, u32, vp]
    L.rgb_train_status.argtypes = [vp, C.POINTER(u32), vp]
    L.rgb_synth_apply_tick_device.argtypes = [vp, vp, u32, vp, vp, vp]
    if hasattr(L, "rgb_synth_set_hint"):
        L.rgb_synth_set_hint.argtypes = [vp, u32]
    L.rgb_wal_adler32_device.argtypes = [vp, vp, u32, vp, C.c_uint64, vp, vp]
    L.rgb_wal_adler32.argtypes = [vp, vp, u32, vp, C.c_uint64, vp]
    L.rgb_wal_layout.restype = C.c_uint64
    L.rgb_wal_layout.argtypes = [vp, u32, C.c_uint64]
    L.rgb_wal_frame_device.argtypes = [vp, vp, u32, vp, C.c_uint64, vp, C.c_uint64, vp, u32, vp]
    L.rgb_wal_frame.argtypes = [vp, vp, u32, vp, C.c_uint64, vp, C.c_uint64, u32]
    L.rgb_wal_scan.argtypes = [vp, C.c_uint64, vp, u32, C.POINTER(C.c_uint32), u64p, C.POINTER(C.c_uint32)]
    L.rgb_wal_validate.argtypes = [vp, vp, C.c_uint64, vp, u32, C.POINTER(C.c_uint32), C.POINTER(C.c_uint32)]
    u32p = C.POINTER(C.c_uint32)
    L.rgb_crc32_device.argtypes = [vp, vp, u32, vp, C.c_uint64, vp, vp]
    L.rgb_crc32.argtypes = [vp, vp, u32, vp, C.c_uint64, vp]
    L.rgb_crc32_stream_device.argtypes = [vp, vp, C.c_uint64, u32, vp, vp]
    L.rgb_crc32_stream.argtypes = [vp, vp, C.c_uint64, u32, u32p]
    L.rgb_segment_layout.restype = C.c_uint64
    L.rgb_segment_layout.argtypes = [vp, u32, u32, vp]
    L.rgb_segment_build_device.argtypes = [vp, vp, u32, u32, vp, vp, C.c_uint64, vp, C.c_uint64, u32, vp]
    L.rgb_segment_build.argtypes = [vp, vp, u32, u32, vp, C.c_uint64, vp, C.c_uint64, u32]
    L.rgb_segment_scan.argtypes = [vp, C.c_uint64, vp, u32, u32p, u32p, u32p, u32p]
    L.rgb_segment_validate.argtypes = [vp, vp, C.c_uint64, vp, u32, u32p]
    if L.rgb_abi_version() != abi.ABI_VERSION and not (os.environ.get("RGB_LIB") and L.rgb_abi_version() == abi.ABI_VERSION - 1):
        raise RuntimeError("ABI version mismatch")
    for i, dt in enumerate(abi.STRUCT_DTYPES):
        if os.environ.get("RGB_LIB") and i >= 6 and L.rgb_abi_version() < abi.ABI_VERSION:
            continue
        if os.environ.get("RGB_LIB") and i >= 7 and not hasattr(L, "rgb_submit_raw"):
            continue
        if L.rgb_struct_size(i) != dt.itemsize:
            raise RuntimeError(f"struct {i}: C size {L.rgb_struct_size(i)} != numpy {dt.itemsize}")
    _lib = L
    return L


def _strerror(code: int) -> str:
    try:
        return lib().rgb_strerror(code).decode()
    except Exception:
        return "?"


def default_config() -> np.ndarray:
    cfg = np.zeros(1, dtype=abi.CONFIG_DTYPE)
    lib().rgb_default_config(cfg.ctypes.data)
    return cfg


class RaGpuBatch:

    def __init__(self, n_groups: int, n_members: int, device: int = 0, max_runs: int = 8,
                 ring_slots: int = 4, ring_capacity: int = 65536, max_pipeline_count: int = 0,
                 max_aer_batch: int = 0, flags: int = 0):
        self._L = lib()
        cfg = default_config()
        cfg["device"] = device
        cfg["max_runs"] = max_runs
        cfg["ring_slots"] = ring_slots
        cfg["ring_capacity"] = ring_capacity
        if max_pipeline_count:
            cfg["max_pipeline_count"] = max_pipeline_count
        if max_aer_batch:
            cfg["max_aer_batch"] = max_aer_batch
        cfg["flags"] = flags
        h = C.c_void_p()
        rc = self._L.rgb_open(cfg.ctypes.data, C.byref(h))
        if rc:
            raise RgbError(rc, "rgb_open")
        self._h = h
        self.n_groups, self.n_members = n_groups, n_members
        self.n_servers = n_groups * n_members
        self.ring_capacity = ring_capacity
        self._check(self._L.rgb_register_groups(self._h, n_groups, n_members), "rgb_register_groups")

    def _check(self, rc: int, what: str):
        if rc:
            raise RgbError(rc, what, self._L.rgb_last_hip_error(self._h) if self._h else 0)

    def close(self):
        if getattr(self, "_h", None):
# ... 105 lines not shown

    def submit_trains(self) -> int:
        return int(self._L.rgb_submit_trains(self._h))

    @property
    def in_flight(self) -> int:
        return int(self._L.rgb_in_flight(self._h))

    def step(self, msgs: np.ndarray, seq_ranges: np.ndarray | None = None):
        m = np.ascontiguousarray(msgs, dtype=abi.MSG_DTYPE)
        out_d, out_r = [], []
        for off in range(0, max(len(m), 1), self.ring_capacity):
            chunk = m[off:off + self.ring_capacity]
            self.submit(chunk, seq_ranges=seq_ranges)
            d, r, _ = self.collect(cap=max(len(chunk), 1))
            r = r.copy()
            r["msg_index"] += off
            out_d.append(d)
            out_r.append(r)
        return np.concatenate(out_d), np.concatenate(out_r)

    def run_ticks_device(self, d_msgs: int, tick_stride: int, n_ticks: int, d_decisions: int,
                         d_rpcs: int = 0, stream: int = 0, tick_counts: np.ndarray | None = None,
                         d_tick_counts: int = 0, kind_counts: np.ndarray | None = None):
        cp = None
        if tick_counts is not None:
            tc = np.ascontiguousarray(tick_counts, dtype=np.uint32)
            assert len(tc) >= n_ticks
            cp = tc.ctypes.data
        kp = None
        if kind_counts is not None:
            kcs = np.ascontiguousarray(kind_counts, dtype=np.uint32)
            assert kcs.shape == (n_ticks, abi.N_KINDS), kcs.shape
            kp = kcs.ctypes.data
        self._check(self._L.rgb_run_ticks_device(self._h, d_msgs, tick_stride, cp, d_tick_counts or None, kp,
                                                 n_ticks, d_decisions, d_rpcs or None, stream or None),
                    "rgb_run_ticks_device")

    def synth_tick_device(self, seed: int, tick: int, d_msgs: int, d_kind_counts: int = 0, d_n: int = 0,
                          stream: int = 0):
        self._check(self._L.rgb_synth_tick_device(self._h, seed, tick, d_msgs, d_kind_counts or None,
                                                  d_n or None, stream or None), "rgb_synth_tick_device")

    def synth_tick_buckets_device(self, seed: int, tick: int, d_msgs: int, d_kind_counts: int = 0, d_n: int = 0,
                                  d_bucket_counts: int = 0, stream: int = 0):
        self._check(self._L.rgb_synth_tick_buckets_device(self._h, seed & (2**64 - 1), tick, d_msgs, d_kind_counts,
                                                         d_n, d_bucket_counts, stream), "rgb_synth_tick_buckets_device")

    def synth_tick_stamped_device(self, seed: int, tick: int, d_msgs: int, d_kind_counts: int = 0, d_n: int = 0,
                                  d_bucket_counts: int = 0, d_stamps: int = 0, stream: int = 0):
        self._check(self._L.rgb_synth_tick_stamped_device(self._h, seed & (2**64 - 1), tick, d_msgs, d_kind_counts,
                                                         d_n, d_bucket_counts, d_stamps, stream),
                    "rgb_synth_tick_stamped_device")

    def synth_stamps_resync_device(self, stream: int = 0):
        self._check(self._L.rgb_synth_stamps_resync_device(self._h, stream), "rgb_synth_stamps_resync_device")

    def train_plan(self, bucket_counts: np.ndarray) -> "TrainPlan":
        return TrainPlan(self, bucket_counts)

    def train_stamp_device(self, d_msgs: int, d_stamps: int, tick_stride: int, tick_counts: np.ndarray, stream: int = 0):
        tc = np.ascontiguousarray(tick_counts, dtype=np.uint32)
        self._check(self._L.rgb_train_stamp_device(self._h, d_msgs, d_stamps, tick_stride, tc.ctypes.data, len(tc),
                                                   stream), "rgb_train_stamp_device")

    def train_run_device(self, plan: "TrainPlan", first_tick: int, n_ticks: int, d_msgs: int, d_stamps: int,
                         tick_stride: int, d_decisions: int, d_rpcs: int = 0, rpc_ring: int = 1, stream: int = 0):
        self._check(self._L.rgb_train_run_device(self._h, plan.h, first_tick, n_ticks, d_msgs, d_stamps, tick_stride,
                                                 d_decisions, d_rpcs, rpc_ring, stream), "rgb_train_run_device")

    def train_plan_snap(self, bucket_counts: np.ndarray, snapshot_every: int) -> "TrainPlan":
        return TrainPlan(self, bucket_counts, snapshot_every)

    def train_run_snap_device(self, plan: "TrainPlan", first_tick: int, n_ticks: int, d_msgs: int, d_stamps: int,
                              tick_stride: int, d_decisions: int, d_rpcs: int, rpc_ring: int, d_snap_stamps: int,
                              d_snap_rows: int, stream: int = 0):
        self._check(self._L.rgb_train_run_snap_device(self._h, plan.h, first_tick, n_ticks, d_msgs, d_stamps, tick_stride,
                                                      d_decisions, d_rpcs, rpc_ring, d_snap_stamps, d_snap_rows, stream),
                    "rgb_train_run_snap_device")

    def snapshot_train_device(self, d_rows: int, stream: int = 0):
        self._check(self._L.rgb_snapshot_train_device(self._h, d_rows, stream or None), "rgb_snapshot_train_device")

    def train_seq_bytes(self) -> int:
        return int(self._L.rgb_train_seq_bytes(self._h))

    def synth_snapshot_mark_device(self, d_snap_stamps: int = 0, stream: int = 0):
        self._check(self._L.rgb_synth_snapshot_mark_device(self._h, d_snap_stamps or None, stream or None),
                    "rgb_synth_snapshot_mark_device")

    def train_status(self, check: bool = True):
        flags = C.c_uint32(0)
        xcc = np.zeros(8, dtype=np.uint32)
        rc = self._L.rgb_train_status(self._h, C.byref(flags), xcc.ctypes.data)
        if check and rc:
            raise RgbError(rc, f"train launch failed (flags={flags.value}: 1 = placement, 2 = spin bound)")
        return int(flags.value), xcc

    def inject_train_fault(self, fault: int):
        self._L.rgb_debug_inject_train_fault(self._h, fault)

    def train_form(self) -> str:
        return {0: "none", 1: "dealt", 2: "persistent"}[int(self._L.rgb_train_form(self._h))] if hasattr(self._L, "rgb_train_form") else "round-3 build"

    def train_recoveries(self) -> int:
        return int(self._L.rgb_train_recoveries(self._h))

    def synth_set_hint(self, level: int):
        self._check(self._L.rgb_synth_set_hint(self._h, level), "rgb_synth_set_hint")

    def synth_apply_tick_device(self, d_msgs: int, max_msgs: int, d_decisions: int, d_rpcs: int = 0,
                                stream: int = 0):
        self._check(self._L.rgb_synth_apply_tick_device(self._h, d_msgs, max_msgs, d_decisions, d_rpcs or None,
                                                        stream or None), "rgb_synth_apply_tick_device")

    def wal_adler32_device(self, d_entries: int, n: int, d_data: int, data_bytes: int, d_checksums: int,
                           stream: int = 0):
        self._check(self._L.rgb_wal_adler32_device(self._h, d_entries, n, d_data, data_bytes, d_checksums,
                                                   stream or None), "rgb_wal_adler32_device")

    def wal_adler32(self, entries: np.ndarray, data: np.ndarray) -> np.ndarray:
        entries = np.ascontiguousarray(entries, dtype=abi.WAL_ENTRY_DTYPE)
        data = np.ascontiguousarray(data, dtype=np.uint8)
        out = np.zeros(len(entries), dtype=np.uint32)
        self._check(self._L.rgb_wal_adler32(self._h, entries.ctypes.data, len(entries),
                                            data.ctypes.data if len(data) else None, len(data),
                                            out.ctypes.data), "rgb_wal_adler32")
        return out

    def wal_frame_device(self, d_records: int, n: int, d_data: int, data_bytes: int, d_out: int, out_bytes: int,
                         d_checksums: int = 0, flags: int = 0, stream: int = 0):
        self._check(self._L.rgb_wal_frame_device(self._h, d_records, n, d_data, data_bytes, d_out, out_bytes,
                                                 d_checksums or None, flags, stream or None), "rgb_wal_frame_device")

    def wal_frame(self, records: np.ndarray, data: np.ndarray, out_bytes: int, flags: int = 0) -> np.ndarray:
        records = np.ascontiguousarray(records, dtype=abi.WAL_RECORD_DTYPE)
        data = np.ascontiguousarray(data, dtype=np.uint8)
        out = np.zeros(out_bytes, dtype=np.uint8)
        self._check(self._L.rgb_wal_frame(self._h, records.ctypes.data, len(records),
                                          data.ctypes.data if len(data) else None, len(data),
                                          out.ctypes.data if out_bytes else None, out_bytes, flags), "rgb_wal_frame")
        return out

    def wal_validate(self, file_bytes: np.ndarray, scanned: np.ndarray):
        file_bytes = np.ascontiguousarray(file_bytes, dtype=np.uint8)
        scanned = np.ascontiguousarray(scanned, dtype=abi.WAL_SCANNED_DTYPE)
        n_ok, status = C.c_uint32(0), C.c_uint32(0)
        self._check(self._L.rgb_wal_validate(self._h, file_bytes.ctypes.data, len(file_bytes),
                                             scanned.ctypes.data if len(scanned) else None, len(scanned),
                                             C.byref(n_ok), C.byref(status)), "rgb_wal_validate")
        return n_ok.value, status.value

    def crc32_device(self, d_entries: int, n: int, d_data: int, data_bytes: int, d_crcs: int, stream: int = 0):
        self._check(self._L.rgb_crc32_device(self._h, d_entries, n, d_data, data_bytes, d_crcs, stream or None),
                    "rgb_crc32_device")

    def crc32(self, entries: np.ndarray, data: np.ndarray) -> np.ndarray:
        entries = np.ascontiguousarray(entries, dtype=abi.SEG_ENTRY_DTYPE)
        data = np.ascontiguousarray(data, dtype=np.uint8)
        out = np.zeros(len(entries), dtype=np.uint32)
        self._check(self._L.rgb_crc32(self._h, entries.ctypes.data, len(entries),
                                      data.ctypes.data if len(data) else None, len(data), out.ctypes.data), "rgb_crc32")
        return out

    def crc32_stream_device(self, d_data: int, n_bytes: int, init: int, d_crc: int, stream: int = 0):
        self._check(self._L.rgb_crc32_stream_device(self._h, d_data or None, n_bytes, init, d_crc, stream or None),
# ... 203 lines not shown
```

Baseline: 13.43 billion.

## Add per-server runs-table hint to skip LDS prefetch of unused run rows

Adds a per-server 16-bit countdown hint array, reset to K on state upload, that records whether deep run-table lookups happened recently. In the train tick slice, the run rows are prefetched into LDS only for lanes whose hint is nonzero; lookups refresh the hint to K and it decays otherwise. The aim is to cut HBM traffic from prefetching run tables that go unused. The cost is an extra atomic load and store per message and a possible fallback to global loads when the hint is stale.

```diff
diff --git a/include/ra_gpu_batch.h b/include/ra_gpu_batch.h
--- a/include/ra_gpu_batch.h
+++ b/include/ra_gpu_batch.h
@@ -379,6 +379,8 @@
                              uint32_t rows_cap);
 uint32_t rgb_train_seq_bytes(const rgb_ctx *ctx);
 int  rgb_train_status(rgb_ctx *ctx, uint32_t *flags_out, uint32_t *xcc_of_shard );
+#define RGB_HINT_FILL_ODD(v) (0x10000u | (((uint32_t)(v) & 0xFFu) << 8))
+int  rgb_train_fill_runs_hint(rgb_ctx *ctx, uint32_t value, void *stream);
 uint32_t rgb_train_form(const rgb_ctx *ctx);
 uint32_t rgb_train_recoveries(const rgb_ctx *ctx);
 
diff --git a/ra_amd/csrc/rgb_api.hip b/ra_amd/csrc/rgb_api.hip
--- a/ra_amd/csrc/rgb_api.hip
+++ b/ra_amd/csrc/rgb_api.hip
@@ -9,8 +9,8 @@
 #include <memory>
 #include <mutex>
 #include <thread>
+#include <vector>
 #include <new>
-#include <vector>
 
 #if defined(__x86_64__)
 #include <emmintrin.h>
@@ -286,6 +286,7 @@
   if (ctx->dev.cond) (void)hipFree(ctx->dev.cond);
   if (ctx->dev.qry) (void)hipFree(ctx->dev.qry);
   if (ctx->dev.seq) (void)hipFree(ctx->dev.seq);
+  if (ctx->dev.runs_hint) (void)hipFree(ctx->dev.runs_hint);
   if (ctx->d_stage) (void)hipFree(ctx->d_stage);
   if (ctx->h_stage) (void)hipHostFree(ctx->h_stage);
   if (ctx->d_rows) (void)hipFree(ctx->d_rows);
@@ -408,6 +409,8 @@
   d.seq_stride = (((n_groups + RGB_TRAIN_SHARDS - 1u) / RGB_TRAIN_SHARDS) * n_members + 255u) & ~255u;
   HIPCHK(ctx, hipMalloc((void **)&d.seq, (size_t)d.seq_stride * RGB_TRAIN_SHARDS));
   HIPCHK(ctx, hipMemsetAsync(d.seq, 0, (size_t)d.seq_stride * RGB_TRAIN_SHARDS, ctx->stream));
+  HIPCHK(ctx, hipMalloc((void **)&d.runs_hint, (size_t)d.seq_stride * RGB_TRAIN_SHARDS * sizeof(unsigned short)));
+  HIPCHK(ctx, hipMemsetAsync(d.runs_hint, (int)RGB_RUNS_HINT_K, (size_t)d.seq_stride * RGB_TRAIN_SHARDS * sizeof(unsigned short), ctx->stream));
   ctx->stage_cap = S < 16384u ? S : 16384u;
   HIPCHK(ctx, hipMalloc((void **)&ctx->d_stage, (size_t)ctx->stage_cap * sizeof(rgb_server_state)));
   HIPCHK(ctx, hipHostMalloc((void **)&ctx->h_stage, (size_t)ctx->stage_cap * sizeof(rgb_server_state),
@@ -481,6 +484,8 @@
   HIPCHK(ctx, hipSetDevice(ctx->cfg.device));
   rgb_stream_turn turn(ctx);
   if (turn.rc) return turn.rc;
+  HIPCHK(ctx, hipMemsetAsync(ctx->dev.runs_hint, (int)RGB_RUNS_HINT_K, (size_t)ctx->dev.seq_stride * RGB_TRAIN_SHARDS * sizeof(unsigned short),
+                             ctx->stream));
   for (u32 base = 0; base < n; base += ctx->stage_cap) {
     u32 cnt = n - base < ctx->stage_cap ? n - base : ctx->stage_cap;
     memcpy(ctx->h_stage, in + base, (size_t)cnt * sizeof(rgb_server_state));
@@ -1498,6 +1503,23 @@
   return (ctx && ctx->registered) ? ctx->dev.seq_stride * RGB_TRAIN_SHARDS : 0u;
 }
 
+int rgb_train_fill_runs_hint(rgb_ctx *ctx, uint32_t value, void *stream) {
+  if (!ctx || value > 0x1FFFFu) return RGB_E_INVAL;
+  if (!ctx->registered) return RGB_E_STATE;
+  HIPCHK(ctx, hipSetDevice(ctx->cfg.device));
+  hipStream_t st = stream ? (hipStream_t)stream : ctx->stream;
+  const size_t n = (size_t)ctx->dev.seq_stride * RGB_TRAIN_SHARDS;
+  if (value & 0x10000u) {
+    std::vector<unsigned short> h(n);
+    for (size_t i = 0; i < n; ++i) h[i] = (unsigned short)(((i & 1u) ? value >> 8 : value) & 0xFFu);
+    HIPCHK(ctx, hipStreamSynchronize(st));
+    HIPCHK(ctx, hipMemcpy(ctx->dev.runs_hint, h.data(), n * sizeof(unsigned short), hipMemcpyHostToDevice));
+    return RGB_OK;
+  }
+  HIPCHK(ctx, hipMemsetAsync(ctx->dev.runs_hint, (int)(value & 0xFFu), n * sizeof(unsigned short), st));
+  return RGB_OK;
+}
+
 int rgb_snapshot_train_device(rgb_ctx *ctx, void *d_rows, void *stream) {
   int rc = rgb_snapshot_device(ctx, d_rows, stream);
   if (rc) return rc;
diff --git a/ra_amd/csrc/rgb_internal.h b/ra_amd/csrc/rgb_internal.h
--- a/ra_amd/csrc/rgb_internal.h
+++ b/ra_amd/csrc/rgb_internal.h
@@ -117,6 +117,7 @@
   const unsigned g = server / n_members, m = server - g * n_members;
   return (g & (RGB_TRAIN_SHARDS - 1u)) * seq_stride + (g / RGB_TRAIN_SHARDS) * n_members + m;
 }
+#define RGB_RUNS_HINT_K 4u
 #define RGB_TRAIN_MAX_TICKS 255u
 #define RGB_N_PCLASSES (2u * RGB_N_CLASSES)
 #define RGB_PC_SNAP RGB_N_PCLASSES
@@ -150,6 +151,7 @@
   u32 max_aer_batch;
   unsigned char *seq;
   u32 seq_stride;
+  unsigned short *runs_hint;
   const u64 *seq_ranges;
   u32 n_seq_ranges;
   u32 fuse_pipeline;
diff --git a/ra_amd/csrc/rgb_kernels.hip b/ra_amd/csrc/rgb_kernels.hip
--- a/ra_amd/csrc/rgb_kernels.hip
+++ b/ra_amd/csrc/rgb_kernels.hip
@@ -158,6 +158,7 @@
   const ulonglong2 *peers_lds;
   unsigned peers_swz;
   const ulonglong2 *runs_lds;
+  unsigned runs_hint;
   ulonglong2 *rpc_stash;
   u32 max_runs;
   u32 flags;
@@ -260,9 +261,17 @@
 __device__ __forceinline__ bool range_nonempty(const Lane &L) { return L.first <= L.li; }
 
 #define RGB_RUNS_LDS 8
+#define RGB_HINT_VAL(w) (((w) >> 8) & 0xFFu)
+#define RGB_HINT_DEEP 0x10000u
+template <class Lane>
+__device__ __forceinline__ bool runs_line(const Lane &L) {
+  if (!Lane::coh) return L.runs_lds != nullptr;
+  const_cast<Lane &>(L).runs_hint |= RGB_HINT_DEEP;
+  return L.runs_lds != nullptr && RGB_HINT_VAL(L.runs_hint) != 0u;
+}
 template <class Lane>
 __device__ __forceinline__ ulonglong2 run_pair(const Lane &L, int k) {
-  if (L.runs_lds != nullptr && k < RGB_RUNS_LDS) return L.runs_lds[(unsigned)k ^ L.peers_swz];
+  if (runs_line(L) && k < RGB_RUNS_LDS) return L.runs_lds[(unsigned)k ^ L.peers_swz];
   return ldg16(L.coh, reinterpret_cast<const ulonglong2 *>(L.runs) + k);
 }
 template <class Lane>
@@ -270,7 +279,7 @@
 #ifdef RGB_PROFILE
   const_cast<Lane &>(L).prof_nloads += 1;
 #endif
-  if (L.runs_lds != nullptr && i < 2 * RGB_RUNS_LDS) {
+  if (runs_line(L) && i < 2 * RGB_RUNS_LDS) {
     const ulonglong2 v = L.runs_lds[(unsigned)(i >> 1) ^ L.peers_swz];
     return (i & 1) ? v.y : v.x;
   }
@@ -704,6 +713,7 @@
       if (L.prof_noprobe) break;
 #endif
       const ulonglong2 r = ldg16(L.coh, reinterpret_cast<const ulonglong2 *>(L.runs) + k);
+      (void)runs_line(L);
 #ifdef RGB_PROFILE
       const_cast<Lane &>(L).prof_nloads += 2;
 #endif
@@ -1752,7 +1762,8 @@
                                                 u32 msg_index_base, Dec &out, u64 *t_loaded = nullptr,
                                                 const ulonglong2 *pre = nullptr, unsigned swz = 0,
                                                 const ulonglong2 *prepeers = nullptr,
-                                                const ulonglong2 *preruns = nullptr, ulonglong2 *rpc_stash = nullptr) {
+                                                const ulonglong2 *preruns = nullptr, ulonglong2 *rpc_stash = nullptr,
+                                                unsigned *runs_hint = nullptr, bool hinted = false) {
   LaneT<TR, (N >= 6 && KIND == RGB_MSG_AER), SEQXP> L;
   L.rpc_stash = rpc_stash;
   L.wc_k = -1; L.wc_start = L.wc_term = L.wc_next = 0;
@@ -1805,6 +1816,7 @@
   L.peers_loaded = false; L.dmi = L.dni = L.dcs = 0; L.dcs_ci = 0;
   L.peers_lds = prepeers; L.peers_swz = swz; L.pdirty = 0;
   L.runs_lds = preruns;
+  if (TR) L.runs_hint = hinted ? *runs_hint : 1u << 8;
   constexpr bool PL = !TR && PRE && rgb_class_slice(1, (unsigned)N) == 32u &&
                       (KIND == RGB_MSG_AER_REPLY || KIND == RGB_MSG_APPEND || KIND == RGB_MSG_PIPELINE_RPCS);
   if (!PL && (L.kind == RGB_MSG_AER_REPLY || L.kind == RGB_MSG_APPEND || L.kind == RGB_MSG_PIPELINE_RPCS ||
@@ -1876,6 +1888,7 @@
 #endif
   if (rc) {
     make_decision(out, L.server, role0, RGB_NONE, 0, L.kind, RGB_F_INVARIANT, (u32)rc, 0, 0, 0, 0, ci0, la0);
+    if (TR && hinted) *runs_hint = L.runs_hint;
     return;
   }
 
@@ -1998,6 +2011,7 @@
   if (L.flags & RGB_F_QUERY_QUORUM) w3 = L.q_consensus;
   make_decision(out, L.server, role_of(L), L.has_reply ? L.reply_to : (unsigned)RGB_NONE, n_rpcs, L.kind,
                 L.flags, 0, w2, w3, w4, w5, L.ci, L.la, L.hb_mask, L.cancel_mask);
+  if (TR && hinted) *runs_hint = L.runs_hint;
 #ifdef RGB_PROFILE
   if (t_loaded) { t_loaded[1] = L.prof_nloads; if (RGB_KNOB(dev, 16u)) t_loaded[3] = wall_clock64(); }
 #endif
@@ -2151,7 +2165,8 @@
 __device__ __forceinline__ bool fast_aer_reply(const rgb_dev &dev, const ulonglong2 m0, const ulonglong2 m1,
                                                const ulonglong2 *pre, unsigned swz, Dec &out,
                                                const ulonglong2 *prow = nullptr,
-                                               const ulonglong2 *rrow = nullptr) {
+                                               const ulonglong2 *rrow = nullptr, unsigned *runs_hint = nullptr,
+                                               bool hinted = false) {
   const u32 server = (u32)(m0.x & 0xFFFFFFFFull);
   const unsigned wire_kind = (unsigned)((m0.x >> 32) & 0xFF), peer = (unsigned)((m0.x >> 40) & 0xFF);
   const unsigned mflags = (unsigned)((m0.x >> 48) & 0xFF);
@@ -2218,6 +2233,10 @@
     else if (n_runs >= 2 && p >= prs) t = prt;
     else {
       bool found = false;
+      if (TR && hinted) {
+        if (RGB_HINT_VAL(*runs_hint) == 0u) rrow = nullptr;
+        if (n_runs >= 3u) *runs_hint |= RGB_HINT_DEEP;
+      }
       const ulonglong2 *rt = reinterpret_cast<const ulonglong2 *>(dev.runs + (size_t)server * dev.max_runs * 2u);
       const int lds_runs = rrow != nullptr ? RGB_RUNS_LDS : 0;
 #pragma unroll 1
@@ -2385,7 +2404,7 @@
 #endif
 }
 
-template <int N, bool TR>
+template <int N, bool TR, bool PERSIST = false>
 __device__ __forceinline__ bool rgb_tick_slice(const rgb_dev &dev, ulonglong2 *io, const int cls, const u32 base,
                                                const u32 cnt, const u32 SL, const rgb_msg *__restrict__ msgs,
                                                rgb_decision *__restrict__ dec, rgb_rpc *__restrict__ rpcs,
@@ -2445,23 +2464,27 @@
     AER_RUNS = __ballot(active && m1.y != m0.y) != 0ull;
   const u32 sv = (u32)(m0.x & 0xFFFFFFFFull);
   const bool has_srv = TR && active && sv < dev.n_servers && ((m0.x >> 32) & 0xFFull) != RGB_MSG_NOP;
-  unsigned char *seqp = nullptr;
+  u32 sqi = 0;
   unsigned need = 0;
+  const bool HINTED = RUNS_LDS && lead_cls && (PEERS_LDS || !PERSIST);
+  unsigned hint = 0;
   if (TR) {
     if (__ballot(has_srv && rgb_shard_of_server(sv, (unsigned)N) != shard) != 0ull) {
       if (lane == 0) atomicOr(ctl, (u32)RGB_TRAIN_ERR_ORDER);
       return false;
     }
-    seqp = dev.seq + rgb_seq_index(has_srv ? sv : 0u, dev.n_members, dev.seq_stride);
+    sqi = rgb_seq_index(has_srv ? sv : 0u, dev.n_members, dev.seq_stride);
     need = has_srv ? need_raw : 0u;
     unsigned spins = 0;
     bool late = has_srv;
     for (;;) {
       if (late) {
 #ifdef RGB_HOST_EMULATION
-        const unsigned cur = *seqp;
+        const unsigned cur = dev.seq[sqi];
+        if (HINTED) hint = dev.runs_hint[sqi] & 0xFFu;
 #else
-        const unsigned cur = __hip_atomic_load(seqp, __ATOMIC_RELAXED, __HIP_MEMORY_SCOPE_AGENT);
+        const unsigned cur = __hip_atomic_load(dev.seq + sqi, __ATOMIC_RELAXED, __HIP_MEMORY_SCOPE_AGENT);
+        if (HINTED) hint = __hip_atomic_load(dev.runs_hint + sqi, __ATOMIC_RELAXED, __HIP_MEMORY_SCOPE_AGENT) & 0xFFu;
 #endif
         late = cur != need;
       }
@@ -2520,13 +2543,14 @@
         if (pcx < 12u)
           glds16<ROWS>(reinterpret_cast<const ulonglong2 *>(dev.peers + (size_t)sj * 24u) + pcx, io + (4 + k) * RGB_TICK_BLOCK);
       }
-      if (RUNS_LDS) {
+      if (RUNS_LDS && (!HINTED || __ballot(hint != 0u) != 0ull)) {
 #pragma unroll
         for (int k = 0; k < 4; ++k) {
           const u32 r = 8 * k + (lane >> 3);
           const u32 sj = __shfl(srv, (int)r, 64);
-          glds16<ROWS>(reinterpret_cast<const ulonglong2 *>(dev.runs + (size_t)sj * dev.max_runs * 2u) + ((lane & 7u) ^ ((r >> 1) & 7u)),
-                       io + (12 + k) * RGB_TICK_BLOCK);
+          if (!HINTED || __shfl(hint, (int)r, 64) != 0u)
+            glds16<ROWS>(reinterpret_cast<const ulonglong2 *>(dev.runs + (size_t)sj * dev.max_runs * 2u) + ((lane & 7u) ^ ((r >> 1) & 7u)),
+                         io + (12 + k) * RGB_TICK_BLOCK);
         }
       }
     }
@@ -2538,13 +2562,14 @@
         glds16<ROWS>(reinterpret_cast<const ulonglong2 *>(dev.peers + (size_t)sj * 16u) + ((lane & 7u) ^ ((r >> 1) & 7u)),
                      io + (4 + k) * RGB_TICK_BLOCK);
       }
-      if (RUNS_LDS) {
+      if (RUNS_LDS && __ballot(hint != 0u) != 0ull) {
 #pragma unroll
         for (int k = 0; k < 4; ++k) {
           const u32 r = 8 * k + (lane >> 3);
           const u32 sj = __shfl(srv, (int)r, 64);
-          glds16<ROWS>(reinterpret_cast<const ulonglong2 *>(dev.runs + (size_t)sj * dev.max_runs * 2u) + ((lane & 7u) ^ ((r >> 1) & 7u)),
-                       io + (8 + k) * RGB_TICK_BLOCK);
+          if (__shfl(hint, (int)r, 64) != 0u)
+            glds16<ROWS>(reinterpret_cast<const ulonglong2 *>(dev.runs + (size_t)sj * dev.max_runs * 2u) + ((lane & 7u) ^ ((r >> 1) & 7u)),
+                         io + (8 + k) * RGB_TICK_BLOCK);
         }
       }
     }
@@ -2561,6 +2586,7 @@
 #ifndef RGB_HOST_EMULATION
   asm volatile("" ::"v"(pf0), "v"(pf1));
 #endif
+  if (HINTED) need |= hint << 8;
   Dec d;
   u64 *tlp = nullptr;
 #ifdef RGB_PROFILE
@@ -2575,7 +2601,7 @@
   pst.p = nullptr; pst.a = pst.b = make_ulonglong2(0, 0); pst.m = 0;
   if (active) {
     if (cls == 0) done = fast_aer(dev, m0, m1, m2, m3, hrow, hswz, d, &pst);
-    else if (cls == 1) done = fast_aer_reply<N, TR, (PEERS_LDS || PEERS_WIDE)>(dev, m0, m1, hrow, hswz, d, prow, rrow);
+    else if (cls == 1) done = fast_aer_reply<N, TR, (PEERS_LDS || PEERS_WIDE)>(dev, m0, m1, hrow, hswz, d, prow, rrow, &need, HINTED);
     else if (cls == 2) done = fast_written(dev, m0, m1, hrow, hswz, d, &pst);
   }
   if (cls == 0 || cls == 2) pair_store(pst, lane);
@@ -2588,7 +2614,7 @@
   case RANK:                                                                                            \
     RGB_MARK("begin", RANK)                                                                             \
     process_message<N, KIND, PRE, TR>(dev, m0, m1, m2, m3, base + lane, rpcs, rpc_slot_base, msg_index_base, d, tlp, \
-                                      hrow, hswz, prow, rrow, stash);                                   \
+                                      hrow, hswz, prow, rrow, stash, &need, rgb_lead_class(RANK) && HINTED); \
     RGB_MARK("end", RANK)                                                                               \
     break;
     switch (cls) {
@@ -2620,12 +2646,17 @@
   const bool is_compact = active && compact_decision(d);
   const u64 cmask = __ballot(is_compact);
   RGB_TT(4);
+  if (TR && HINTED) {
+    const unsigned h0 = RGB_HINT_VAL(need);
+    const unsigned nh = (need & RGB_HINT_DEEP) ? RGB_RUNS_HINT_K : (h0 != 0u ? h0 - 1u : 0u);
+    if (has_srv && nh != h0) dev.runs_hint[sqi] = (unsigned short)nh;
+  }
   if (TR) {
 #ifndef RGB_HOST_EMULATION
     __builtin_amdgcn_s_waitcnt(0x0F70);
     asm volatile("" ::: "memory");
 #endif
-    if (has_srv && seqp != nullptr) *seqp = (unsigned char)(need + 1u);
+    if (has_srv) dev.seq[sqi] = (unsigned char)(need + 1u);
     if (ticket_ctr != nullptr) *next_ticket = rgb_take_ticket(ticket_ctr, ctl);
     if (place_word != nullptr && lane == 0) {
 #ifdef RGB_HOST_EMULATION
@@ -2942,7 +2973,7 @@
     rgb_rpc *rp = A->rpcs ? A->rpcs + (tick_stride ? (size_t)(t % A->rpc_ring) * tick_stride : toff) * (N > 1 ? N - 1 : 1) : nullptr;
     lds_barrier();
     raw = 0;
-    if (!rgb_tick_slice<N, true>(dev, io, cls, off + lbase, cnt, SL, A->msgs + toff, A->dec + toff, rp, 0,
+    if (!rgb_tick_slice<N, true, true>(dev, io, cls, off + lbase, cnt, SL, A->msgs + toff, A->dec + toff, rp, 0,
                                  A->index_base + (u32)toff, A->ctl, A->stamps + toff, tk, &raw, x, lane))
       break;
   }
@@ -2986,7 +3017,7 @@
 __device__ __forceinline__ void syn_lane(Lane &T, const SynMember &x, const u64 *runs) {
   T.first = x.first; T.li = x.li; T.lrs = x.lrs; T.lrt = x.lrt; T.prs = x.prs; T.prt = x.prt;
   T.push_cnt = 0; T.n_runs = (unsigned)pk_get(x.pk, PK_NRUNS_SH, 5);
-  T.runs = runs; T.runs_lds = nullptr;
+  T.runs = runs; T.runs_lds = nullptr; T.runs_hint = 0;
 #ifdef RGB_PROFILE
   T.prof_noprobe = false; T.prof_nloads = 0;
 #endif
diff --git a/ra_amd/engine.py b/ra_amd/engine.py
--- a/ra_amd/engine.py
+++ b/ra_amd/engine.py
@@ -23,6 +23,7 @@
     "rgb_train_plan_create_device", "rgb_train_plan_build_device", "rgb_train_plan_download", "rgb_train_plan_fit",
     "rgb_submit_seq", "rgb_set_seq_ranges_device", "rgb_collect_view", "rgb_release",
     "rgb_submit_raw_capacity", "rgb_submit_begin", "rgb_submit_commit", "rgb_submit_raw",
+    "rgb_train_fill_runs_hint",
 ]
 COMM_EXPORTS = ["rgb_comm_unique_id", "rgb_comm_init_rank", "rgb_comm_destroy", "rgb_comm_n_ranks", "rgb_comm_rank",
                 "rgb_leaderboard_allgather", "rgb_leaderboard_allgather_host", "rgb_comm_last_error"]
@@ -36,7 +37,7 @@
                           "rgb_synth_set_hint", "rgb_train_plan_create_device", "rgb_train_plan_build_device",
                           "rgb_train_plan_download", "rgb_train_plan_fit", "rgb_submit_seq", "rgb_set_seq_ranges_device",
                           "rgb_collect_view", "rgb_release", "rgb_submit_raw_capacity", "rgb_submit_begin",
-                          "rgb_submit_commit", "rgb_submit_raw"} | set(COMM_EXPORTS)
+                          "rgb_submit_commit", "rgb_submit_raw", "rgb_train_fill_runs_hint"} | set(COMM_EXPORTS)
 WAL_EXPORTS = ["rgb_wal_adler32_device", "rgb_wal_adler32", "rgb_wal_layout", "rgb_wal_frame_device",
                "rgb_wal_frame", "rgb_wal_scan", "rgb_wal_validate",
                "rgb_crc32_device", "rgb_crc32", "rgb_crc32_stream_device", "rgb_crc32_stream", "rgb_segment_layout",
@@ -60,6 +61,8 @@
         subprocess.check_call(["make", "-C", _CSRC, "libra_gpu_batch.so"])
     return LIB_PATH
 
+
+RUNS_HINT_K = 4
 
 _lib = None
 
@@ -169,6 +172,8 @@
         L.rgb_train_plan_create_device.argtypes = [vp, u32, u32, C.POINTER(vp)]
         L.rgb_train_plan_build_device.argtypes = [vp, vp, u32, u32, vp, vp]
         L.rgb_train_plan_download.argtypes = [vp, vp, u32, vp, vp, u32]
+    if hasattr(L, "rgb_train_fill_runs_hint"):
+        L.rgb_train_fill_runs_hint.argtypes = [vp, u32, vp]
     if hasattr(L, "rgb_train_plan_fit"):
         L.rgb_train_plan_fit.argtypes = [vp, vp, u32, u32, vp]
     L.rgb_train_status.argtypes = [vp, C.POINTER(u32), vp]
@@ -440,6 +445,11 @@
     def snapshot_train_device(self, d_rows: int, stream: int = 0):
         self._check(self._L.rgb_snapshot_train_device(self._h, d_rows, stream or None), "rgb_snapshot_train_device")
 
+    def train_fill_runs_hint(self, value: int, odd=None, stream: int = 0):
+        if odd is not None:
+            value |= 0x10000 | ((odd & 0xFF) << 8)
+        self._check(self._L.rgb_train_fill_runs_hint(self._h, value, stream or None), "rgb_train_fill_runs_hint")
+
     def train_seq_bytes(self) -> int:
         return int(self._L.rgb_train_seq_bytes(self._h))
 
```

After: 13.05 billion. 0.972x the previous value.
